# bcgsc/RNA-Bloom

Measured on AMD Instinct MI355X. Metric: k-mers/sec hashed+inserted into Bloom dBG (k=25, 50M 150bp reads), higher is better.
Workload: dtype u64

## Files before the change

### rna-bloom_amd/csrc/rb_capi.hip

```cpp
#include <math.h>
#include <stdarg.h>
#include <stdlib.h>
#include <string.h>
#include <time.h>

#include <algorithm>
#include <new>
#include <vector>

#include <functional>
#include <string>
#include <thread>

#include <fcntl.h>
#include <unistd.h>
#include <zlib.h>

#include "rb_pipeline.hpp"

using namespace rb;

namespace {

__global__ void k_popcount_bits(const uint32_t *__restrict__ w, size_t n_words, unsigned long long *out) {
// ... 594 lines not shown
            std::thread prep;
            int prep_rc = RB_OK;
            std::string prep_err;
            if (!last) {
                const size_t carry = len - cur.consumed;
                memcpy(buf[1 - w], buf[w] + cur.consumed, carry);
                prep = std::thread([&, carry] {
                    prep_rc = guarded([&] { nxt = make(1 - w, carry, &nlen); });
                    if (prep_rc != RB_OK) prep_err = rb_last_error();
                });
            }
            const int add_rc = guarded([&] { if (cur.b && cur.b->n_reads) add_range(g, cur.b, 0, cur.b->n_reads, flags, stats); });
            if (prep.joinable()) prep.join();
            if (add_rc != RB_OK) { if (nxt.b) rb_batch_destroy(nxt.b); throw HipError{add_rc}; }
            if (prep_rc != RB_OK) { set_error("%s", prep_err.c_str()); throw HipError{prep_rc}; }
            if (last) break;
            w = 1 - w; len = nlen; cur = nxt;
        }
        if (n_records) *n_records = recs;
    });
    if (st && !own_stream.s && rc != RB_OK) (void)hipStreamSynchronize(st);
    return rc;
}
}

extern "C" {
int rb_graph_add_fastq_file(rb_graph *g, const char *path, int min_base_qual, unsigned flags, rb_add_stats *stats, int64_t *n_records) {
    return add_text_file(g, path, false, min_base_qual, flags, stats, n_records);
}
int rb_graph_add_fasta_file(rb_graph *g, const char *path, unsigned flags, rb_add_stats *stats, int64_t *n_records) {
    return add_text_file(g, path, true, 0, flags, stats, n_records);
}

int rb_graph_apply(rb_graph *g, int op, const uint64_t *h0, size_t n) {
    return guarded([&] {
        RB_REQUIRE(g && (h0 || n == 0), "rb_graph_apply: null argument");
        WriteLock wl(g->rw);
        RB_REQUIRE(op >= RB_OP_ADD && op <= RB_OP_ADD_FRAG_PAIR, "rb_graph_apply: unknown op %d", op);
        RB_REQUIRE(!g->shard, "rb_graph_apply: not available on a shard handle");
        RB_HIP(hipSetDevice(g->p.device));
        hipStream_t s = g->stream;
        if (op == RB_OP_ADD_DBG_ONLY || op == RB_OP_ADD_READ_PAIR || op == RB_OP_ADD_FRAG_PAIR) {
            BitFilter *f = op == RB_OP_ADD_DBG_ONLY ? &g->dbg : op == RB_OP_ADD_READ_PAIR ? &g->rpk : &g->fpk;
            if (!f->bits) { set_error("rb_graph_apply: filter not initialised"); throw HipError{RB_ERR_STATE}; }
            if (n) {
                uint64_t *d = upload_h0(g, g->qbuf0, h0, n);
                hipLaunchKernelGGL(k_bits_add, dim3(blocks_for((int64_t)n)), dim3(TPB), 0, s, f->bits, f->mod, f->num_hash,
                                   kmul_of(g->k), d, n);
                RB_HIP(hipGetLastError());
            }
            RB_HIP(hipStreamSynchronize(s));
            return;
        }
        const int mode = op == RB_OP_ADD ? M_ADD : op == RB_OP_ADD_IF_ABSENT ? M_ADD_IF_ABSENT
                       : op == RB_OP_ADD_COUNT_IF_PRESENT ? M_COUNT_IF_PRESENT : M_COUNT_ONLY;
        size_t done = 0;
        const size_t chunk = (size_t)g->max_batch_kmers;
        while (done < n) {
            size_t m = std::min(chunk, n - done);
            g->keys0.reserve(m * 8); g->vals0.reserve(m * 4);
            RB_HIP(hipMemcpyAsync(g->keys0.p, h0 + done, m * 8, hipMemcpyHostToDevice, s));
            hipLaunchKernelGGL(k_iota, dim3(blocks_for((int64_t)m)), dim3(TPB), 0, s, g->vals0.as<uint32_t>(), m);
            run_pipeline(g, m, mode, g->ordinal, 0, nullptr);
            g->ordinal += m;
            done += m;
        }
        RB_HIP(hipStreamSynchronize(s));
    });
}

}
namespace {
__global__ void k_debug_probe(uint32_t *words, uint64_t n_words, uint32_t per_thread, int mode, uint64_t salt, unsigned long long *sink) {
    const uint64_t t = (uint64_t)blockIdx.x * blockDim.x + threadIdx.x;
    uint64_t x = (t + salt) * 0x9E3779B97F4A7C15ull + 0x632BE59BD9B4E019ull;
    uint32_t acc = 0;
    for (uint32_t i = 0; i < per_thread; ++i) {
        x ^= x >> 30; x *= 0xBF58476D1CE4E5B9ull; x ^= x >> 27; x *= 0x94D049BB133111EBull; x ^= x >> 31;
        uint32_t *w = &words[(uint64_t)(((unsigned __int128)x * n_words) >> 64)];
        acc |= mode ? atomicXor(w, 0x80808080u) : atomicOr(w, 0u);
    }
    if (acc == 0x12345678u) atomicAdd(sink, 1ull);
}
}
extern "C" {
int rb_debug_probe_cbf(rb_graph *g, int mode, float *ms_out) {
    return guarded([&] {
        RB_REQUIRE(g && g->cbf && ms_out, "rb_debug_probe_cbf: bad argument");
        rb::WriteLock wl(g->rw);
        RB_HIP(hipSetDevice(g->p.device));
        hipStream_t s = g->stream;
        g->devctr.reserve(DEVCTR_BYTES);
        rb::Event e0, e1;
        RB_HIP(hipEventCreate(&e0.e)); RB_HIP(hipEventCreate(&e1.e));
        RB_HIP(hipStreamSynchronize(s));
        RB_HIP(hipEventRecord(e0, s));
        for (int pass = 0; pass < 2; ++pass)
            hipLaunchKernelGGL(k_debug_probe, dim3(65536), dim3(256), 0, s, reinterpret_cast<uint32_t *>(g->cbf), (uint64_t)(g->cbf_alloc / 4), 16u, mode, 0ull, g->devctr.as<unsigned long long>());
        RB_HIP(hipEventRecord(e1, s));
        RB_HIP(hipEventSynchronize(e1));
        RB_HIP(hipEventElapsedTime(ms_out, e0, e1));
    });
}

int rb_debug_scan_u32(int device, const uint32_t *in, size_t n, uint32_t *out, int misalign) {
    DevBuf a, b, t;
    return guarded([&] {
        RB_REQUIRE((in && out) || n == 0, "rb_debug_scan_u32: null array");
        RB_REQUIRE(misalign >= 0 && misalign < 16, "rb_debug_scan_u32: misalign in 0..15");
        RB_HIP(hipSetDevice(device));
        a.reserve((n + 8) * 4); b.reserve((n + 8) * 4); t.reserve(scan_temp_bytes(n));
        uint32_t *di = a.as<uint32_t>() + (misalign & 3), *dout = b.as<uint32_t>() + ((misalign >> 2) & 3);
        if (n) RB_HIP(hipMemcpy(di, in, n * 4, hipMemcpyHostToDevice));
        exclusive_scan_u32(t.p, t.cap, di, dout, n, nullptr);
        RB_HIP(hipGetLastError());
        RB_HIP(hipDeviceSynchronize());
        if (n) RB_HIP(hipMemcpy(out, dout, n * 4, hipMemcpyDeviceToHost));
    });
}
int rb_debug_sort_pairs(int device, uint64_t *keys, void *vals, int vals64, size_t n, int lo_begin, int lo_end, int hi_begin, int hi_end) {
    DevBuf k0, k1, v0, v1, t;
    return guarded([&] {
        RB_REQUIRE(keys || n == 0, "rb_debug_sort_pairs: null keys");
        RB_REQUIRE(!(vals64 && hi_begin >= 0), "rb_debug_sort_pairs: two ranges with 32-bit values only");
        RB_HIP(hipSetDevice(device));
        if (n == 0) return;
        const size_t vb = vals64 ? 8 : 4;
        k0.reserve(n * 8); k1.reserve(n * 8);
        if (vals) { v0.reserve(n * vb); v1.reserve(n * vb); RB_HIP(hipMemcpy(v0.p, vals, n * vb, hipMemcpyHostToDevice)); }
        RB_HIP(hipMemcpy(k0.p, keys, n * 8, hipMemcpyHostToDevice));
        t.reserve(vals64 ? sort_pairs32_temp_bytes(n) : sort_pairs_temp_bytes(n));
        if (vals64) sort_pairs_u64_u64(t.p, t.cap, k0.as<uint64_t>(), k1.as<uint64_t>(), v0.as<uint64_t>(), v1.as<uint64_t>(), n, lo_begin, lo_end, nullptr);
        else if (hi_begin >= 0) sort_pairs_u64_u32_2r(t.p, t.cap, k0.as<uint64_t>(), k1.as<uint64_t>(), v0.as<uint32_t>(), v1.as<uint32_t>(), n, lo_begin, lo_end, hi_begin, hi_end, nullptr);
        else if (vals) sort_pairs_u64_u32(t.p, t.cap, k0.as<uint64_t>(), k1.as<uint64_t>(), v0.as<uint32_t>(), v1.as<uint32_t>(), n, lo_begin, lo_end, nullptr);
        else sort_keys_u64(t.p, t.cap, k0.as<uint64_t>(), k1.as<uint64_t>(), n, lo_begin, lo_end, nullptr);
        RB_HIP(hipGetLastError());
        RB_HIP(hipDeviceSynchronize());
        RB_HIP(hipMemcpy(keys, k1.p, n * 8, hipMemcpyDeviceToHost));
        if (vals) RB_HIP(hipMemcpy(vals, v1.p, n * vb, hipMemcpyDeviceToHost));
    });
}
int rb_debug_group(int device, const uint64_t *keys, const uint32_t *vals, size_t n, int group_bits, int bucket_target, unsigned flags,
                   uint64_t seed, uint64_t ordinal0, uint32_t pos_bits, uint64_t idx_size, uint64_t idx_lo, uint64_t idx_span,
                   uint32_t *vals_out, uint8_t *tz_out, uint64_t *uniq, uint32_t *counts, uint32_t *starts, uint32_t *brun, uint32_t *bnr, int64_t *info) {
    DevBuf k0, v0, k1, v1, vo, tz, un, cn, st, br, bn, t, ctr;
    return guarded([&] {
        RB_REQUIRE(keys && vals && vals_out && tz_out && uniq && counts && starts && info, "rb_debug_group: null array");
        RB_REQUIRE(n > 0 && n < ((size_t)1 << 28), "rb_debug_group: record count out of range");
        RB_REQUIRE((brun == nullptr) == (bnr == nullptr), "rb_debug_group: brun and bnr go together");
        RB_REQUIRE(pos_bits < 32 && (idx_span == 0 || idx_size > 0), "rb_debug_group: bad pos_bits / index range");
        RB_HIP(hipSetDevice(device));
        const int gflags = (int)flags;
        const GrIdx idx = idx_span ? GrIdx{make_mod(idx_size), idx_lo, idx_span} : GrIdx{Mod{1, 0, 0}, 0, 0};
        uint32_t plan[7];
        group_debug_plan(n, group_bits, bucket_target, gflags, idx, plan);
        const size_t nbk = (size_t)1 << plan[0];
        k0.reserve(n * 8); v0.reserve(n * 4); k1.reserve(n * 8); v1.reserve(n * 4);
        vo.reserve(n * 4); tz.reserve(n + 16); un.reserve(n * 8); cn.reserve((n + 1) * 4); st.reserve((n + 1) * 4);
        t.reserve(group_temp_bytes(n, group_bits, bucket_target, gflags));
        ctr.reserve(64);
        RB_HIP(hipMemcpy(k0.p, keys, n * 8, hipMemcpyHostToDevice));
        RB_HIP(hipMemcpy(v0.p, vals, n * 4, hipMemcpyHostToDevice));
        RB_HIP(hipMemset(vo.p, 0, n * 4)); RB_HIP(hipMemset(tz.p, 0, n)); RB_HIP(hipMemset(un.p, 0, n * 8));
        RB_HIP(hipMemset(cn.p, 0, n * 4)); RB_HIP(hipMemset(st.p, 0, n * 4)); RB_HIP(hipMemset(ctr.p, 0, 64));
        GroupExport ex;
        if (brun) {
            br.reserve(nbk * 4 + 16); bn.reserve(nbk * 4 + 16);
            RB_HIP(hipMemset(br.p, 0, nbk * 4)); RB_HIP(hipMemset(bn.p, 0, nbk * 4));
            ex = GroupExport{br.as<uint32_t>(), bn.as<uint32_t>(), ctr.as<uint32_t>() + 1};
        }
        group_records_device(k0.as<uint64_t>(), v0.as<uint32_t>(), k1.as<uint64_t>(), v1.as<uint32_t>(), n, group_bits, seed, ordinal0, pos_bits,
                             t.p, t.cap, vo.as<uint32_t>(), tz.as<uint8_t>(), un.as<uint64_t>(), cn.as<uint32_t>(), st.as<uint32_t>(), ctr.as<uint32_t>(),
                             nullptr, nullptr, bucket_target, gflags, idx, ex);
        RB_HIP(hipDeviceSynchronize());
        uint32_t c[2] = {0, 0}, live = (uint32_t)n, n_big = 0, largest = 0;
        uint64_t big_rec = 0;
        RB_HIP(hipMemcpy(c, ctr.p, 8, hipMemcpyDeviceToHost));
        if (gflags & GR_FLAG_DEAD) RB_HIP(hipMemcpy(&live, group_live_count(t.p, n, group_bits, bucket_target, gflags), 4, hipMemcpyDeviceToHost));
        group_debug_big(t.p, n, group_bits, bucket_target, &n_big, &big_rec, &largest, gflags);
        RB_REQUIRE(c[0] <= n && live <= n, "rb_debug_group: the stage reports %u runs and %u live records of %zu", c[0], live, n);
        RB_HIP(hipMemcpy(vals_out, vo.p, n * 4, hipMemcpyDeviceToHost));
        RB_HIP(hipMemcpy(tz_out, tz.p, n, hipMemcpyDeviceToHost));
        RB_HIP(hipMemcpy(uniq, un.p, n * 8, hipMemcpyDeviceToHost));
        RB_HIP(hipMemcpy(counts, cn.p, n * 4, hipMemcpyDeviceToHost));
        RB_HIP(hipMemcpy(starts, st.p, n * 4, hipMemcpyDeviceToHost));
        if (brun) {
            RB_HIP(hipMemcpy(brun, br.p, nbk * 4, hipMemcpyDeviceToHost));
            RB_HIP(hipMemcpy(bnr, bn.p, nbk * 4, hipMemcpyDeviceToHost));
        }
        for (int i = 0; i < 7; ++i) info[i] = (int64_t)plan[i];
        info[7] = (int64_t)c[0]; info[8] = brun ? (int64_t)c[1] : -1; info[9] = (int64_t)live;
        info[10] = (int64_t)n_big; info[11] = (int64_t)largest;
    });
}
int rb_debug_select(int device, const uint32_t *status, size_t n, uint32_t mask_a, uint32_t mask_b, uint32_t *out_a, uint32_t *out_b, uint32_t *counts) {
    DevBuf s, a, b, t, ctr;
    return guarded([&] {
        RB_REQUIRE(counts && (n == 0 || (status && out_a && (out_b || mask_b == 0u))), "rb_debug_select: null array");
        RB_REQUIRE(n < ((size_t)1 << 31), "rb_debug_select: too many items");
        RB_HIP(hipSetDevice(device));
        s.reserve(n * 4 + 16); a.reserve(n * 4 + 16); b.reserve(n * 4 + 16); ctr.reserve(64);
        t.reserve(mask_b ? select2_temp_bytes(n) : select_temp_bytes(n));
        if (n) RB_HIP(hipMemcpy(s.p, status, n * 4, hipMemcpyHostToDevice));
        RB_HIP(hipMemset(ctr.p, 0xFF, 64));
        if (mask_b) select_flagged2(t.p, t.cap, s.as<uint32_t>(), n, mask_a, a.as<uint32_t>(), mask_b, b.as<uint32_t>(), ctr.as<uint32_t>(), nullptr);
        else select_flagged(t.p, t.cap, s.as<uint32_t>(), mask_a, n, a.as<uint32_t>(), ctr.as<uint32_t>(), nullptr);
        RB_HIP(hipGetLastError());
        RB_HIP(hipDeviceSynchronize());
        uint32_t c[2] = {0, 0};
        RB_HIP(hipMemcpy(c, ctr.p, 8, hipMemcpyDeviceToHost));
        if (!mask_b) c[1] = 0;
        RB_REQUIRE(c[0] <= n && c[1] <= n, "rb_debug_select: the selection reports %u and %u of %zu items", c[0], c[1], n);
        if (c[0]) RB_HIP(hipMemcpy(out_a, a.p, (size_t)c[0] * 4, hipMemcpyDeviceToHost));
        if (c[1]) RB_HIP(hipMemcpy(out_b, b.p, (size_t)c[1] * 4, hipMemcpyDeviceToHost));
        counts[0] = c[0]; counts[1] = c[1];
    });
}
}
namespace {
bool debug_prefilter_on(const rb_graph *g) {
    const bool wide_off = getenv("RB_WIDE_PREFILTER") && atoi(getenv("RB_WIDE_PREFILTER")) == 0;
    return g->npf_log2 && (g->k <= 31 || (g->k <= 64 && !wide_off));
}
bool debug_prefilter_uses_mpf(const rb_graph *g, const rb_batch *b, int64_t nw) {
    return g->mpf_log2b && !getenv("RB_NO_MPF") && (uint32_t)g->k >= g->mpf_m &&
           (g->k <= RB_MPF_MAX_K ? (uint32_t)g->k - g->mpf_m + 1u <= RB_MPF_MAX_RING : filter_wide_mpf_ok(b, nw, g->k));
}
bool debug_prefilter_saves_state(const rb_graph *g, const rb_batch *b, int64_t nw, bool use_mpf) {
    return g->k > RB_MPF_MAX_K ? (use_mpf && filter_saves_state_wide(b, nw, g->k)) : filter_saves_state(b, nw, g->k);
}
}
extern "C" {
int rb_debug_cache_export(rb_graph *g, int which, uint64_t *out, size_t cap_words, uint32_t *log2_out, uint32_t *m_out) {
    return guarded([&] {
        RB_REQUIRE(g && log2_out && m_out, "rb_debug_cache_export: null argument");
        RB_REQUIRE(which == 0 || which == 1, "rb_debug_cache_export: which must be 0 (minimizer-bucketed) or 1 (hash-bucketed)");
        rb::WriteLock wl(g->rw);
        RB_REQUIRE(which == 0 ? g->mpf_log2b != 0u : g->npf_log2 != 0u, "rb_debug_cache_export: this handle has no %s prefilter cache (k = %d)",
                   which == 0 ? "minimizer-bucketed" : "hash-bucketed", g->k);
        const size_t words = which == 0 ? (size_t)16 << g->mpf_log2b : (size_t)1 << g->npf_log2;
        *log2_out = which == 0 ? g->mpf_log2b : g->npf_log2;
        *m_out = which == 0 ? g->mpf_m : 0u;
        if (!out) return;
        RB_REQUIRE(cap_words >= words, "rb_debug_cache_export: the table has %zu words, the array has room for %zu", words, cap_words);
        RB_HIP(hipSetDevice(g->p.device));
        for (hipStream_t st : {(hipStream_t)g->stream, (hipStream_t)g->stream2}) RB_HIP(hipStreamSynchronize(st));
        RB_HIP(hipMemcpy(out, which == 0 ? g->mpf.p : g->npf.p, words * 8, hipMemcpyDeviceToHost));
    });
}
int rb_debug_prefilter(rb_graph *g, const rb_batch *b, int64_t first_word, int64_t n_words, uint64_t ordinal0, uint32_t pos_bits,
                       uint32_t *cnt_out, uint32_t *mask_out) {
    DevBuf cnt, mask, tot, ws;
    return guarded([&] {
        RB_REQUIRE(g && b && cnt_out && mask_out, "rb_debug_prefilter: null argument");
        rb::WriteLock wl(g->rw);
        RB_REQUIRE(!g->shard, "rb_debug_prefilter: not available on a shard handle");
        RB_REQUIRE(b->device == g->p.device, "batch lives on device %d, graph on %d", b->device, g->p.device);
        RB_REQUIRE(debug_prefilter_on(g), "rb_debug_prefilter: an insert into this handle runs no prefilter (k = %d)", g->k);
        RB_REQUIRE(pos_bits >= 1u && pos_bits < 32u, "rb_debug_prefilter: pos_bits in 1..31");
        const auto &wo = b->h_woff;
        RB_REQUIRE(!wo.empty() && first_word >= 0 && n_words > 0 && first_word + n_words <= b->n_words, "rb_debug_prefilter: bad word range");
        const int64_t r0 = std::lower_bound(wo.begin(), wo.end(), (uint32_t)first_word) - wo.begin();
        const int64_t r1 = std::lower_bound(wo.begin(), wo.end(), (uint32_t)(first_word + n_words)) - wo.begin();
        RB_REQUIRE(r0 < (int64_t)wo.size() && wo[(size_t)r0] == (uint32_t)first_word && r1 < (int64_t)wo.size() && wo[(size_t)r1] == (uint32_t)(first_word + n_words),
                   "rb_debug_prefilter: the word range does not start and end at read boundaries");
        RB_HIP(hipSetDevice(g->p.device));
        hipStream_t s = g->stream;
        const bool use_mpf = debug_prefilter_uses_mpf(g, b, n_words);
        const Npf npf{reinterpret_cast<unsigned long long *>(g->npf.p), g->npf_log2};
        const Mpf mpf{use_mpf ? reinterpret_cast<unsigned long long *>(g->mpf.p) : nullptr, g->mpf_log2b, g->mpf_m};
        const size_t nb = (size_t)n_words * 4;
        cnt.reserve(nb + 4); mask.reserve(nb + 4); tot.reserve(2048);
        RB_HIP(hipMemsetAsync(cnt.p, 0xEE, nb, s)); RB_HIP(hipMemsetAsync(mask.p, 0xEE, nb, s)); RB_HIP(hipMemsetAsync(tot.p, 0, 2048, s));
        void *wstate = nullptr;
        if (debug_prefilter_saves_state(g, b, n_words, use_mpf)) { ws.reserve(((size_t)n_words + 1) * 16); wstate = ws.p; }
        launch_filter_windows(b, first_word, n_words, g->k, g->stranded ? 0 : 1, (uint32_t)r0, pos_bits, g->p.rng_seed, ordinal0, npf,
                              cnt.as<uint32_t>(), mask.as<uint32_t>(), tot.as<uint32_t>(), s, OwnRange{Mod{1, 0, 0}, 0, 0}, mpf, wstate);
        RB_HIP(hipGetLastError());
        RB_HIP(hipStreamSynchronize(s));
        RB_HIP(hipMemcpy(cnt_out, cnt.p, nb, hipMemcpyDeviceToHost));
        RB_HIP(hipMemcpy(mask_out, mask.p, nb, hipMemcpyDeviceToHost));
    });
}
int rb_filter_size(rb_graph *g, int which, int64_t *size, int64_t *nbytes, int *num_hash) {
    if (!g) { set_error("null graph"); return RB_ERR_INVALID; }
    if (which == RB_CBF) {
        if (!g->cbf) { set_error("rb_filter_size: filter %d not initialised", which); return RB_ERR_STATE; }
        if (size) *size = g->cbf_size;
        if (nbytes) *nbytes = g->cbf_hi - g->cbf_lo;
        if (num_hash) *num_hash = g->cbf_h;
        return RB_OK;
    }
    BitFilter *f = bit_filter(g, which);
    if (!f) { set_error("rb_filter_size: unknown filter %d", which); return RB_ERR_INVALID; }
    if (!f->bits) { set_error("rb_filter_size: filter %d not initialised", which); return RB_ERR_STATE; }
    if (size) *size = f->size;
    if (nbytes) *nbytes = f->nbytes;
    if (num_hash) *num_hash = f->num_hash;
    return RB_OK;
}

static int filter_reduce(rb_graph *g, int which, bool fold, unsigned long long *out) {
    return guarded([&] {
        RB_REQUIRE(g && out, "rb_filter_popcount / rb_filter_fold: null argument");
        QueryLease q(g);
        RB_HIP(hipStreamSynchronize(g->stream));
        q.c->b0.reserve(64);
// ... 182 lines not shown
```

### rna-bloom_amd/csrc/rb_graph.hip

```cpp
#include <math.h>
#include <stdarg.h>
#include <stdlib.h>
#include <string.h>
#include <time.h>

#include <algorithm>
#include <new>
#include <vector>

#include <functional>
#include <string>
#include <thread>

#include <fcntl.h>
#include <unistd.h>
#include <zlib.h>

#include "rb_pipeline.hpp"

using namespace rb;

namespace rb {
static thread_local char g_err[768] = "";
const char *last_error_text() { return g_err; }
// ... 921 lines not shown
                if (j && (e & 31u) == 0u) { cR = word_c(e >> 5); vR = word_v(e >> 5); }
                if (j && (j & 31u) == 0u) { cL = word_c(j >> 5); vL = word_v(j >> 5); }
                const uint32_t codeR = (uint32_t)cR & 3u, okR = vR & 1u, codeL = (uint32_t)cL & 3u, okL = vL & 1u;
                cR >>= 2; vR >>= 1; cL >>= 2; vL >>= 1;
                {
                    const uint32_t in5 = okR ? codeR + 1u : 0u;
                    const uint32_t out5 = ((uint32_t)(hvR >> sh_v) & 1u) ? ((uint32_t)((far ? hcR2 : hcR) >> sh_c) & 3u) + 1u : 0u;
                    const uint32_t tt = out5 * 5u + in5;
                    fR = rotl(fR, 1) ^ s_tf[tt]; rR = rotr(rR, 1) ^ s_tr[tt];
                    hcR2 = (hcR2 << 2) | (hcR >> 62); hcR = (hcR << 2) | codeR; hvR = (hvR << 1) | okR;
                }
                {
                    const uint32_t in5 = okL ? codeL + 1u : 0u;
                    const uint32_t out5 = ((uint32_t)(hvL >> sh_v) & 1u) ? ((uint32_t)((far ? hcL2 : hcL) >> sh_c) & 3u) + 1u : 0u;
                    const uint32_t tt = out5 * 5u + in5;
                    fL = rotl(fL, 1) ^ s_tf[tt]; rL = rotr(rL, 1) ^ s_tr[tt];
                    if (VAR == 1) {
                        mF = ((mF << 2) | codeL) & mmask;
                        mR = (mR >> 2) | ((3u - codeL) << mtop);
                        uint32_t x = (mF < mR ? mF : mR) * 0x9E3779B1u;
                        x ^= x >> 15;
                        xnew = x >> 4;
                        if ((x & seen.amask) == 0u && j + 1u >= um) { akey = xnew; apos1 = j + 2u - um; }
                    }
                    hcL2 = (hcL2 << 2) | (hcL >> 62); hcL = (hcL << 2) | codeL; hvL = (hvL << 1) | okL;
                }
                lb = okR ? lb : e + 1u;
                if (j + 1u >= uk) {
                    const uint32_t p = j + 1u - uk;
                    bool ok = lb <= p;
                    if (ok && present) {
                        const uint64_t hl = (MODE == 0) ? fL : (MODE == 2) ? rL : smin(fL, rL);
                        const uint64_t hr = (MODE == 0) ? fR : (MODE == 2) ? rR : smin(fR, rR);
                        ok = bits_lookup(present, present_mod, present_h, kmul, hl) && bits_lookup(present, present_mod, present_h, kmul, hr);
                    }
                    if (ok) {
                        uint64_t P;
                        if (MODE == 0) P = combine(fL, fR);
                        else if (MODE == 2) P = combine(rR, rL);
                        else P = smin(combine(fL, fR), combine(rR, rL));
                        if (VAR == 2) {
                            if ((p >> 5) != oword) { oword = p >> 5; obase = chunk_off[wrel + (int64_t)oword]; ocnt = 0; }
                            for (int h = 0; h < num_hash; ++h)
                                out_idx[((size_t)obase + ocnt) * (size_t)num_hash + h] = index_of(multi_hash(P, (uint32_t)h, kmul), mod);
                            ++ocnt;
                        } else if (VAR == 1) {
                            const uint32_t bk = (apos1 > p ? akey : xnew) & seen.mask;
                            if (bk != curb) {
                                curb = bk; ++dbg_fetch;
                                const uint4 *src = reinterpret_cast<const uint4 *>(seen.tab + ((size_t)bk << 4));
                                uint4 v[8];
#pragma unroll
                                for (int q = 0; q < 8; ++q) v[q] = src[q];
#pragma unroll
                                for (int q = 0; q < 8; ++q) {
                                    s_img[(2 * q) * 64 + threadIdx.x] = (unsigned long long)v[q].x | ((unsigned long long)v[q].y << 32);
                                    s_img[(2 * q + 1) * 64 + threadIdx.x] = (unsigned long long)v[q].z | ((unsigned long long)v[q].w << 32);
                                }
                            }
                            const uint32_t sa = (uint32_t)P & 15u, sb0 = ((uint32_t)P >> 4) & 15u, sb = sb0 == sa ? (sa ^ 1u) : sb0;
                            const unsigned long long ea = s_img[sa * 64u + threadIdx.x], eb = s_img[sb * 64u + threadIdx.x];
                            if (P == 0ull || (ea != P && eb != P)) {
                                ++dbg_miss;
                                for (int h = 0; h < num_hash; ++h) bit_set(bits, index_of(multi_hash(P, (uint32_t)h, kmul), mod));
                                if (P != 0ull) {
                                    const uint32_t sl = ea == 0ull ? sa : (eb == 0ull ? sb : sa);
                                    s_img[sl * 64u + threadIdx.x] = P;
                                    seen.tab[((size_t)bk << 4) + sl] = P;
                                }
                            }
                        } else {
                            for (int h = 0; h < num_hash; ++h) bit_set(bits, index_of(multi_hash(P, (uint32_t)h, kmul), mod));
                        }
                        ++cnt;
                    }
                }
            }
            if (VAR == 1 && seen.dbg) { atomicAdd(seen.dbg, (unsigned long long)dbg_miss); atomicAdd(seen.dbg + 1, (unsigned long long)dbg_fetch); }
        }
    }
    if (n_pairs) {
        unsigned long long c = cnt;
        for (int o = 32; o > 0; o >>= 1) c += __shfl_down(c, o, 64);
        if (threadIdx.x == 0 && c) atomicAdd(n_pairs, c);
    }
}

}

void rb::launch_pairs_reads(rb_graph *g, const rb_batch *b, int64_t w0, int64_t nw, int mode_hash, const BitFilter &f, int dist,
                               uint32_t min_len, bool if_present, const uint32_t *chunk_off, uint64_t *out_idx, unsigned long long *pc,
                               hipStream_t st) {
    RB_REQUIRE(g->k <= 64 && b->max_len <= 1024u, "paired k-mers: k <= 64 and reads of at most 1024 bases only on this path");
    const auto &wo = b->h_woff;
    const int64_t r0 = std::lower_bound(wo.begin(), wo.end(), (uint32_t)w0) - wo.begin();
    const int64_t r1 = std::lower_bound(wo.begin(), wo.end(), (uint32_t)(w0 + nw)) - wo.begin();
    RB_REQUIRE(r0 < (int64_t)wo.size() && wo[(size_t)r0] == (uint32_t)w0 && r1 < (int64_t)wo.size() && wo[(size_t)r1] == (uint32_t)(w0 + nw),
               "launch_pairs: word range does not start and end at read boundaries");
    if (r1 <= r0) return;
    dim3 gr(blocks_for(r1 - r0, 64)), th(64);
    const uint32_t *present = if_present ? g->dbg.bits : nullptr;
    const bool use_seen = f.seen && !out_idx && !present;
    static const uint32_t anchor_bits = getenv("RB_PAIR_SEEN_ANCHOR") ? (uint32_t)std::max(0, std::min(4, atoi(getenv("RB_PAIR_SEEN_ANCHOR")))) : 2u;
    const PairSeen seen{use_seen ? f.seen : nullptr, use_seen ? (1u << f.seen_log2b) - 1u : 0u, (1u << anchor_bits) - 1u,
                        (use_seen && pc == g->pairs_ctr.as<unsigned long long>() && getenv("RB_DEBUG")) ? pc + 1 : nullptr};
#define RB_LAUNCH_PR3(M, NW, V)                                                                                          \
    hipLaunchKernelGGL((k_pairs_reads<M, NW, V>), gr, th, 0, st, b->codes, b->valid, b->woff, b->len, r0, r1 - r0, w0, g->k, \
                       dist, f.bits, f.mod, f.num_hash, kmul_of(g->k), pc, chunk_off, out_idx, min_len, present, g->dbg.mod, g->dbg.num_hash, seen)
#define RB_LAUNCH_PR(M, NW) do { if (out_idx) RB_LAUNCH_PR3(M, NW, 2); else if (use_seen) RB_LAUNCH_PR3(M, NW, 1); else RB_LAUNCH_PR3(M, NW, 0); } while (0)
    if (b->max_len <= 384u) { if (mode_hash == 0) RB_LAUNCH_PR(0, 12); else if (mode_hash == 2) RB_LAUNCH_PR(2, 12); else RB_LAUNCH_PR(1, 12); }
    else { if (mode_hash == 0) RB_LAUNCH_PR(0, 32); else if (mode_hash == 2) RB_LAUNCH_PR(2, 32); else RB_LAUNCH_PR(1, 32); }
#undef RB_LAUNCH_PR
#undef RB_LAUNCH_PR3
}

void rb::launch_pairs(rb_graph *g, const rb_batch *b, int64_t w0, int64_t nw, int mode_hash, const uint32_t *chunk_off,
                      uint64_t *out_idx, unsigned long long *pc, hipStream_t st, const BitFilter *into) {
    if (!st) st = g->stream;
    if (nw <= 0) return;
    const BitFilter &rpk = into ? *into : g->rpk;
    const bool general = g->k > 64 || b->max_len > 384u || (getenv("RB_PAIRS_GENERAL") && atoi(getenv("RB_PAIRS_GENERAL")));
    if (!general) {
        launch_pairs_reads(g, b, w0, nw, mode_hash, rpk, g->read_d, 0u, false, chunk_off, out_idx, pc, st);
        return;
    }
    dim3 gr(blocks_for(nw)), th(TPB);
#ifdef RB_DIAG_PAIRS
    if (getenv("RB_PAIRS_VARIANT") && atoi(getenv("RB_PAIRS_VARIANT")) == 9 && mode_hash == 1) {
        hipLaunchKernelGGL(k_pairs_insert_runtime_branch, gr, th, 0, st, b->codes, b->valid, b->word_read, b->woff, b->len, w0, nw, g->k, g->read_d,
                           rpk.bits, rpk.mod, rpk.num_hash, kmul_of(g->k), pc, chunk_off, out_idx,
                           (b->wpr_uniform && nw % b->wpr_uniform == 0) ? b->wpr_uniform : 0u);
        return;
    }
#endif
#define RB_LAUNCH_PAIRS(M)                                                                                          \
    if (out_idx) RB_LAUNCH_PAIRS2(M, true); else RB_LAUNCH_PAIRS2(M, false)
#define RB_LAUNCH_PAIRS2(M, O)                                                                                      \
    hipLaunchKernelGGL((k_pairs_insert<M, O>), gr, th, 0, st, b->codes, b->valid, b->word_read, b->woff, b->len, w0, nw, \
                       g->k, g->read_d, rpk.bits, rpk.mod, rpk.num_hash, kmul_of(g->k), pc, chunk_off, out_idx, \
                       (b->wpr_uniform && nw % b->wpr_uniform == 0) ? b->wpr_uniform : 0u)
    if (mode_hash == 0) { RB_LAUNCH_PAIRS(0); } else if (mode_hash == 2) { RB_LAUNCH_PAIRS(2); } else { RB_LAUNCH_PAIRS(1); }
#undef RB_LAUNCH_PAIRS
#undef RB_LAUNCH_PAIRS2
}

static bool sweep_wanted(const rb_graph *g) {
    if (g->shard || !g->dbg.bits || g->dbg.lo != 0 || g->dbg.hi != g->dbg.size) return false;
    if (const char *e = getenv("RB_SWEEP")) return atoi(e) != 0;
    return g->dbg.nbytes >= ((int64_t)1 << 31);
}
void rb::group_enqueue(rb_graph *g, int slot, size_t N, uint64_t ordinal0, uint32_t pos_bits, hipStream_t st, DevBuf &temp,
                       DevBuf &ctrbuf, int flags) {
    rb_graph::GroupSlot &S = g->slots[slot];
    S.N = N; S.D = 0; S.flags = flags; S.live = (uint32_t)N;
    ctrbuf.reserve(DEVCTR_BYTES);
    uint32_t *ctr = ctrbuf.as<uint32_t>();
    RB_HIP(hipMemsetAsync(ctr, 0, DEVCTR_BYTES, st));
    if (N == 0) return;
    const int group_bits = 64 - g->sort_begin_bit;
    const int bucket_target = g->shard ? (getenv("RB_SHARD_GROUP_TARGET") ? atoi(getenv("RB_SHARD_GROUP_TARGET")) : 3072) : 0;
    S.bucket_target = bucket_target;
    temp.reserve(group_temp_bytes(N, group_bits, bucket_target, flags));
    S.keys1.reserve(N * 8); S.valsT.reserve(N * 4); S.vals1.reserve(N * 4); S.tz.reserve(N + 16);
    S.uniq.reserve(N * 8); S.counts.reserve((N + 1) * 4); S.starts.reserve((N + 1) * 4);
    GrIdx gidx{Mod{1, 0, 0}, 0, 0};
    bool want_idx = true;
    if (const char *e = getenv("RB_GROUP_IDX")) want_idx = atoi(e) != 0;
    if (want_idx) {
        if (g->cbf && g->cbf_size > 0) gidx = GrIdx{g->cbf_mod, (uint64_t)g->cbf_lo, (uint64_t)(g->cbf_hi - g->cbf_lo)};
        else if (g->dbg.bits && g->dbg.size > 0) gidx = GrIdx{g->dbg.mod, (uint64_t)g->dbg.lo, (uint64_t)(g->dbg.hi - g->dbg.lo)};
    }
    GroupExport ex;
    S.sweep_T = 0; S.n_main = 0;
    if (want_idx && sweep_wanted(g)) {
        const GrIdx didx{g->dbg.mod, 0, (uint64_t)g->dbg.size};
        const bool same = gidx.span == didx.span && gidx.lo == 0 && gidx.mod.d == didx.mod.d;
        if (!same) gidx = didx;
        S.sweep_T = group_index_buckets(N, group_bits, bucket_target, flags, gidx);
        if (S.sweep_T) {
            S.brun.reserve(((size_t)4 << S.sweep_T) + 16); S.bnr.reserve(((size_t)4 << S.sweep_T) + 16);
            ex = GroupExport{S.brun.as<uint32_t>(), S.bnr.as<uint32_t>(), ctr + 9};
        }
    }
    uint64_t *kin = g->group_in_keys ? g->group_in_keys : g->keys0.as<uint64_t>();
    uint32_t *vin = g->group_in_vals ? g->group_in_vals : g->vals0.as<uint32_t>();
    g->group_in_keys = nullptr; g->group_in_vals = nullptr;
    group_records_device(kin, vin, S.keys1.as<uint64_t>(), S.valsT.as<uint32_t>(), N, group_bits,
                         g->p.rng_seed, ordinal0, pos_bits, temp.p, temp.cap, S.vals1.as<uint32_t>(), S.tz.as<uint8_t>(), S.uniq.as<uint64_t>(),
                         S.counts.as<uint32_t>(), S.starts.as<uint32_t>(), ctr + 8, st, g, bucket_target, flags, gidx, ex);
}
uint32_t rb::group_finish(rb_graph *g, int slot, hipStream_t st, DevBuf &temp, DevBuf &ctrbuf, hipStream_t scan_stream) {
    rb_graph::GroupSlot &S = g->slots[slot];
    if (S.N == 0) { RB_HIP(hipStreamSynchronize(st)); return 0; }
    uint32_t D = 0;
    RB_HIP(hipMemcpyAsync(&D, ctrbuf.as<uint32_t>() + 8, 4, hipMemcpyDeviceToHost, st));
    if (S.sweep_T) RB_HIP(hipMemcpyAsync(&S.n_main, ctrbuf.as<uint32_t>() + 9, 4, hipMemcpyDeviceToHost, st));
    if (S.flags & GR_FLAG_DEAD)
        RB_HIP(hipMemcpyAsync(&S.live, group_live_count(temp.p, S.N, 64 - g->sort_begin_bit, S.bucket_target, S.flags), 4, hipMemcpyDeviceToHost, st));
    RB_HIP(hipStreamSynchronize(st));
    RB_REQUIRE(D < (1u << 30), "sub-batch has too many distinct k-mers (%u)", D);
    S.D = D;
    (void)scan_stream;
    if (getenv("RB_DEBUG") && temp.p) {
        uint32_t nb = 0, mx = 0; uint64_t rec = 0;
        group_debug_big(temp.p, S.N, 64 - g->sort_begin_bit, S.bucket_target, &nb, &rec, &mx, S.flags);
        fprintf(stderr, "[rb] grouping: N=%zu runs=%u; buckets that did not fit LDS: %u with %llu records, largest %u\n", S.N, D, nb, (unsigned long long)rec, mx);
    }
    return D;
}
uint32_t rb::group_records(rb_graph *g, size_t N, uint64_t ordinal0, uint32_t pos_bits, rb_add_stats *stats, uint32_t **ctr_out) {
    group_enqueue(g, g->cur, N, ordinal0, pos_bits, g->stream, g->temp, g->devctr);
    const uint32_t D = group_finish(g, g->cur, g->stream, g->temp, g->devctr, g->stream);
    if (ctr_out) *ctr_out = g->devctr.as<uint32_t>();
    if (stats) stats->distinct += D;
    return D;
}

namespace {

}
__global__ void __launch_bounds__(256) k_zero16(uint4 *__restrict__ p, size_t n16) {
    const uint4 z = make_uint4(0u, 0u, 0u, 0u);
    for (size_t i = (size_t)blockIdx.x * blockDim.x + threadIdx.x; i < n16; i += (size_t)gridDim.x * blockDim.x) p[i] = z;
}
void rb::fast_zero(void *p, size_t bytes, hipStream_t s) {
    if (!p || !bytes) return;
    if (bytes < ((size_t)64 << 20) || (reinterpret_cast<uintptr_t>(p) & 15u)) { RB_HIP(hipMemsetAsync(p, 0, bytes, s)); return; }
    const size_t n16 = bytes / 16;
    hipLaunchKernelGGL(k_zero16, dim3(256 * 16), dim3(256), 0, s, static_cast<uint4 *>(p), n16);
    RB_HIP(hipGetLastError());
    if (bytes & 15u) RB_HIP(hipMemsetAsync(static_cast<char *>(p) + n16 * 16, 0, bytes & 15u, s));
}

void rb::alloc_bits(BitFilter &f, int64_t bits, int num_hash, int64_t lo, int64_t hi) {
    f.size = bits;
    f.lo = lo; f.hi = hi;
    const int64_t local = hi - lo;
    f.nbytes = local / 8 + ((local % 8) ? 1 : 0);
    f.alloc = (((size_t)f.nbytes + 3) / 4 + 1) * 4;
    f.num_hash = num_hash;
    f.mod = make_mod((uint64_t)bits);
    RB_HIP(hipMalloc(&f.bits, f.alloc));
    RB_HIP(hipMemset(f.bits, 0, f.alloc));
    RB_HIP(hipDeviceSynchronize());
}
namespace {
__global__ void k_alloc_probe(uint32_t *words, uint64_t n_words, uint32_t per_thread, unsigned long long *sink) {
    const uint64_t t = (uint64_t)blockIdx.x * blockDim.x + threadIdx.x;
    uint64_t x = t * 0x9E3779B97F4A7C15ull + 0x632BE59BD9B4E019ull;
    uint32_t acc = 0;
    for (uint32_t i = 0; i < per_thread; ++i) {
        x ^= x >> 30; x *= 0xBF58476D1CE4E5B9ull; x ^= x >> 27; x *= 0x94D049BB133111EBull; x ^= x >> 31;
        acc |= atomicXor(&words[(uint64_t)(((unsigned __int128)x * n_words) >> 64)], 0x80808080u);
    }
    if (acc == 0x12345678u) atomicAdd(sink, 1ull);
}
}
void *rb::alloc_best_placed(size_t bytes, const char *what) {
    int tries = getenv("RB_ALLOC_TRIES") ? atoi(getenv("RB_ALLOC_TRIES")) : 8;
    tries = std::max(1, std::min(16, tries));
    if (bytes < ((size_t)1 << 30)) tries = 1;
    struct Held {
        void *best = nullptr, *cand = nullptr;
        unsigned long long *sink = nullptr;
        hipEvent_t e0 = nullptr, e1 = nullptr;
        std::vector<void *> losers;
        ~Held() {
            for (void *p : losers) (void)hipFree(p);
            if (best) (void)hipFree(best);
            if (cand) (void)hipFree(cand);
            if (sink) (void)hipFree(sink);
            if (e0) (void)hipEventDestroy(e0);
            if (e1) (void)hipEventDestroy(e1);
        }
    } H;
    float best_ms = 0;
    if (tries > 1) { RB_HIP(hipMalloc(&H.sink, 64)); RB_HIP(hipEventCreate(&H.e0)); RB_HIP(hipEventCreate(&H.e1)); }
    for (int t = 0; t < tries; ++t) {
        if (t) {
            size_t free_b = 0, total_b = 0;
            RB_HIP(hipMemGetInfo(&free_b, &total_b));
            if (free_b < bytes + total_b / 4) break;
        }
        if (hipMalloc(&H.cand, bytes) != hipSuccess) { H.cand = nullptr; (void)hipGetLastError(); if (t) break; RB_HIP(hipErrorOutOfMemory); }
        RB_HIP(hipMemset(H.cand, 0, bytes));
        float ms = 0;
        if (tries > 1) {
            RB_HIP(hipDeviceSynchronize());
            RB_HIP(hipEventRecord(H.e0, nullptr));
            for (int pass = 0; pass < 2; ++pass)
                hipLaunchKernelGGL(k_alloc_probe, dim3(16384), dim3(256), 0, nullptr, static_cast<uint32_t *>(H.cand), (uint64_t)(bytes / 4), 16u, H.sink);
            RB_HIP(hipEventRecord(H.e1, nullptr));
            RB_HIP(hipEventSynchronize(H.e1));
            RB_HIP(hipEventElapsedTime(&ms, H.e0, H.e1));
        }
        if (getenv("RB_ALLOC_DEBUG")) fprintf(stderr, "[rb] %s allocation %d: %.3f ms for 2 x 2^26 random XORs\n", what, t, ms);
        if (!H.best || ms < best_ms) { if (H.best) H.losers.push_back(H.best); H.best = H.cand; best_ms = ms; }
        else H.losers.push_back(H.cand);
        H.cand = nullptr;
    }
    RB_HIP(hipDeviceSynchronize());
    void *best = H.best;
    H.best = nullptr;
    return best;
}

void rb::free_bits(BitFilter &f) { if (f.bits) (void)hipFree(f.bits); if (f.seen) (void)hipFree(f.seen); f = BitFilter(); }
void rb::alloc_pair_seen(BitFilter &f) {
    if (!f.bits || f.seen) return;
    uint32_t lb = std::max(8u, std::min(24u, log2_ceil((uint64_t)std::max<int64_t>(f.size / 512, 1))));
    if (const char *e = getenv("RB_PAIR_SEEN")) { const int v = atoi(e); if (v <= 0) return; lb = (uint32_t)std::max(4, std::min(26, v)); }
    size_t fr = 0, tot = 0;
    if (hipMemGetInfo(&fr, &tot) == hipSuccess && ((size_t)128 << lb) > fr / 4) return;
    if (hipMalloc(&f.seen, (size_t)128 << lb) != hipSuccess) { (void)hipGetLastError(); f.seen = nullptr; return; }
    RB_HIP(hipMemset(f.seen, 0, (size_t)128 << lb));
    RB_HIP(hipDeviceSynchronize());
    f.seen_log2b = lb;
}
void rb::seen_reset(BitFilter &f, hipStream_t s) {
    if (f.seen) fast_zero(f.seen, (size_t)128 << f.seen_log2b, s);
}
namespace {


}
BitFilter *rb::bit_filter(rb_graph *g, int which) {
    switch (which) { case RB_DBGBF: return &g->dbg; case RB_RPKBF: return &g->rpk; case RB_FPKBF: return &g->fpk; default: return nullptr; }
}
namespace {

void run_core(rb_graph *g, size_t N, uint32_t D, int mode, uint64_t ordinal0, uint32_t pos_bits, rb_add_stats *stats,
              const std::function<void()> *after_resolve = nullptr);
}
void rb::run_pipeline(rb_graph *g, size_t N, int mode, uint64_t ordinal0, uint32_t pos_bits, rb_add_stats *stats) {
    if (N == 0) return;
    const uint32_t D = group_records(g, N, ordinal0, pos_bits, stats, nullptr);
    run_core(g, N, D, mode, ordinal0, pos_bits, stats);
}
namespace {
void run_core(rb_graph *g, size_t N, uint32_t D, int mode, uint64_t ordinal0, uint32_t pos_bits, rb_add_stats *stats,
              const std::function<void()> *after_resolve) {
    hipStream_t s = g->stream;
    if (N == 0 || D == 0) { if (after_resolve) (*after_resolve)(); return; }
    g->devctr.reserve(DEVCTR_BYTES);
    uint32_t *ctr = g->devctr.as<uint32_t>();
    RB_HIP(hipMemsetAsync(ctr, 0, DEVCTR_BYTES, s));
    FilterView fv = g->view(ordinal0, pos_bits);
    const uint64_t *uniq = g->uniq().as<uint64_t>();
    const uint32_t *counts = g->counts().as<uint32_t>(), *starts = g->starts().as<uint32_t>(), *vals = g->vals1().as<uint32_t>();
    g->status.reserve((size_t)D * 4); g->nops.reserve((size_t)D * 4); g->cvals.reserve((size_t)D * 8);
    g->heavy.reserve((size_t)D * 4); g->confk.reserve((size_t)D * 4);
    g->foreign.reserve((size_t)D * 8 * (size_t)g->cbf_h);
    uint32_t *status = g->status.as<uint32_t>(), *nops = g->nops.as<uint32_t>();
    const bool uses_dbg = (mode == M_ADD || mode == M_ADD_IF_ABSENT);
    uint32_t f_log2 = 1, c_log2 = 1, csf_log2 = 16;
    uint32_t *csf = nullptr;
    const bool full_table = getenv("RB_FIRST_SETTER_TABLE") && atoi(getenv("RB_FIRST_SETTER_TABLE"));
    const bool collide = uses_dbg && !full_table;
    Slot *ftab = nullptr;
    FtFilter ffl{nullptr, 0};
    if (uses_dbg && full_table) {
        g->prof_begin();
        f_log2 = log2_ceil(2ull * (uint64_t)D * (uint64_t)g->dbg.num_hash + 2);
        g->ftable.reserve(sizeof(Slot) << f_log2);
        RB_HIP(hipMemsetAsync(g->ftable.p, 0xFF, sizeof(Slot) << f_log2, s));
        ftab = g->ftable.as<Slot>();
        g->prof_end("table_clear");
    }
    g->prof_begin();
    const rb_graph::GroupSlot &GS = g->slots[g->cur];
    bool swept = false, swept_all = false;
    uint32_t *involved = nullptr, n_involved_max = 0;
    if (collide && !ftab && fv.dbg_h == 2 && fv.cbf_h == 2 && !getenv("RB_PROBE_GENERIC") && GS.sweep_T && !g->shard && sweep_wanted(g) &&
        ((uint64_t)g->dbg.size >> GS.sweep_T) < (1ull << 31)) {
        const char *e = getenv("RB_SWEEP");
        static const float present_max = getenv("RB_SWEEP_PRESENT") ? (float)atof(getenv("RB_SWEEP_PRESENT")) : 0.5f;
        swept = (e && atoi(e) == 1) || ((uint64_t)D * 64ull >= (uint64_t)g->dbg.nbytes && g->last_present_frac < present_max);
    }
    if (swept) {
        const GrIdx didx{g->dbg.mod, 0, (uint64_t)g->dbg.size};
        swept_all = GS.n_main >= D;
        const size_t st_pad = ((size_t)D + 15) & ~(size_t)15;
        g->sw_st.reserve(st_pad + D + 16);
        g->sw_temp.reserve(sweep_temp_bytes(D, GS.sweep_T));
        uint8_t *st0 = g->sw_st.as<uint8_t>(), *st1 = st0 + st_pad;
        uint64_t *ka = g->foreign.as<uint64_t>(), *kb = ka + D;
        sweep_bits_device(g->dbg.bits, didx, GS.sweep_T, fv.kmul, uniq, D, GS.n_main, GS.brun.as<uint32_t>(), GS.bnr.as<uint32_t>(), ka, g->nops.as<uint32_t>(), kb,
                          g->heavy.as<uint32_t>(), g->sw_temp.p, g->sw_temp.cap, st0, st1, s);
        const bool same_index = (int64_t)g->dbg.size == g->cbf_size && g->cbf_lo == 0 && g->dbg.mod.d == g->cbf_mod.d && g->dbg.mod.m_lo == g->cbf_mod.m_lo &&
                                g->dbg.mod.m_hi == g->cbf_mod.m_hi && fv.dbg_h == fv.cbf_h;
        const bool plain_ok = swept_all && same_index && !(getenv("RB_SWEEP_CLAIMS") && atoi(getenv("RB_SWEEP_CLAIMS")));
        constexpr int RUNS = 2;
        hipLaunchKernelGGL((k_probe_h2<RUNS, true>), dim3(blocks_for(((int64_t)D + RUNS - 1) / RUNS)), dim3(TPB), 0, s, fv, uniq, counts, D, mode, status,
                           g->cvals.as<uint64_t>(), g->foreign.as<uint64_t>(), ctr, (const uint8_t *)st0, (const uint8_t *)st1, swept_all ? 1u : 0u,
                           plain_ok ? 1u : 0u);
    } else if (!ftab && fv.dbg_h == 2 && fv.cbf_h == 2 && !getenv("RB_PROBE_GENERIC")) {
        constexpr int RUNS = 2;
        hipLaunchKernelGGL((k_probe_h2<RUNS, false>), dim3(blocks_for(((int64_t)D + RUNS - 1) / RUNS)), dim3(TPB), 0, s, fv, uniq, counts, D, mode, status,
                           g->cvals.as<uint64_t>(), g->foreign.as<uint64_t>(), ctr);
    } else
        hipLaunchKernelGGL(k_probe, dim3(blocks_for(D)), dim3(TPB), 0, s, fv, uniq, counts, starts, vals, D, mode,
                           ftab, f_log2, status, g->cvals.as<uint64_t>(), g->foreign.as<uint64_t>(), ctr);
    if (collide) {
        if (!swept) hipLaunchKernelGGL(k_set_bits, dim3(blocks_for(D)), dim3(TPB), 0, s, fv, uniq, D, status, ctr);
        uint32_t spread[16 * 32], n_collide = 0;
        RB_HIP(hipMemcpyAsync(spread, ctr + 16, sizeof spread, hipMemcpyDeviceToHost, s));
        RB_HIP(hipStreamSynchronize(s));
        for (int q = 0; q < 32; ++q) n_collide += spread[16 * q + 1];
        if (n_collide) {
            f_log2 = log2_ceil(4ull * (uint64_t)n_collide + 2);
            const size_t tab_bytes = sizeof(Slot) << f_log2;
            const uint32_t ff_log2 = std::max(16u, std::min(30u, log2_ceil(8ull * (uint64_t)n_collide)));
            const bool use_ff = getenv("RB_FT_FILTER") ? atoi(getenv("RB_FT_FILTER")) != 0 : tab_bytes > ((size_t)32 << 20);
            g->ftable.reserve(tab_bytes + (use_ff ? ((size_t)1 << (ff_log2 - 3)) : 0));
            RB_HIP(hipMemsetAsync(g->ftable.p, 0xFF, tab_bytes, s));
            ftab = g->ftable.as<Slot>();
            if (use_ff) {
                uint32_t *fb = reinterpret_cast<uint32_t *>(static_cast<char *>(g->ftable.p) + tab_bytes);
                RB_HIP(hipMemsetAsync(fb, 0, (size_t)1 << (ff_log2 - 3), s));
                ffl = FtFilter{fb, ff_log2};
            }
            if (swept_all) {
                involved = g->confk.as<uint32_t>(); n_involved_max = n_collide;
                g->temp.reserve(select_temp_bytes(D));
                select_flagged(g->temp.p, g->temp.cap, status, (3u << ST_COLLIDE_SHIFT) | (3u << ST_JOIN_SHIFT), D, involved, ctr + 12, s);
                hipLaunchKernelGGL(k_collide_insert, dim3(blocks_for(std::min(D, n_collide))), dim3(TPB), 0, s, fv, uniq, starts, vals, std::min(D, n_collide), status, ftab, f_log2,
                                   const_cast<uint32_t *>(ffl.bits), ffl.log2, (const uint32_t *)involved, (const uint32_t *)(ctr + 12));
            } else
            hipLaunchKernelGGL(k_collide_insert, dim3(blocks_for(D)), dim3(TPB), 0, s, fv, uniq, starts, vals, D, status, ftab, f_log2,
                               const_cast<uint32_t *>(ffl.bits), ffl.log2);
            if (!swept_all) hipLaunchKernelGGL(k_collide_fixup, dim3(blocks_for(D)), dim3(TPB), 0, s, fv, uniq, starts, vals, D, status, ftab, f_log2, ffl);
        }
    }
    if (mode == M_ADD) {
        if (swept_all) {
            if (involved) hipLaunchKernelGGL(k_late_claim, dim3(blocks_for(std::min(D, n_involved_max))), dim3(TPB), 0, s, fv, uniq, starts, vals, std::min(D, n_involved_max), ftab, f_log2,
                                             status, g->cvals.as<uint64_t>(), g->foreign.as<uint64_t>(), ctr, ffl, (const uint32_t *)involved, (const uint32_t *)(ctr + 12));
        } else
        hipLaunchKernelGGL(k_late_claim, dim3(blocks_for(D)), dim3(TPB), 0, s, fv, uniq, starts, vals, D, ftab, f_log2,
                           status, g->cvals.as<uint64_t>(), g->foreign.as<uint64_t>(), ctr, ffl);
    }
    uint32_t n_foreign = 0;
    {
        uint32_t spread[16 * 32];
        RB_HIP(hipMemcpyAsync(spread, ctr + 16, sizeof spread, hipMemcpyDeviceToHost, s));
        RB_HIP(hipStreamSynchronize(s));
        uint32_t n_present = 0;
        for (int q = 0; q < 32; ++q) { n_foreign += spread[16 * q]; n_present += spread[16 * q + 2]; }
        const bool counted = !(uses_dbg && full_table) && fv.dbg_h == 2 && fv.cbf_h == 2 && !getenv("RB_PROBE_GENERIC");
        g->last_present_frac = counted ? (float)n_present / (float)D : -1.0f;
    }
    if (getenv("RB_DEBUG") && swept) fprintf(stderr, "[rb] swept stage: %u runs (%u of oversized buckets), %u contested counters\n", D, D - std::min(D, GS.n_main), n_foreign);
    g->prof_end("probe_claim");
    if (n_foreign) {
        g->prof_begin();
        c_log2 = log2_ceil(2ull * (uint64_t)n_foreign + 2);
        csf_log2 = std::max(16u, std::min(25u, log2_ceil(8ull * (uint64_t)n_foreign)));
        const size_t tab_bytes = sizeof(Slot) << c_log2;
        g->ctable.reserve(tab_bytes + ((size_t)1 << (csf_log2 - 3)));
        csf = reinterpret_cast<uint32_t *>(static_cast<char *>(g->ctable.p) + tab_bytes);
        RB_HIP(hipMemsetAsync(g->ctable.p, 0xFF, tab_bytes, s));
        RB_HIP(hipMemsetAsync(csf, 0, (size_t)1 << (csf_log2 - 3), s));
        hipLaunchKernelGGL(k_cs_build, dim3(blocks_for(D)), dim3(TPB), 0, s, status, g->foreign.as<uint64_t>(), D, g->cbf_h,
                           g->ctable.as<Slot>(), c_log2, csf, csf_log2);
        g->prof_end("conflict_set");
    }
    g->prof_begin();
    hipLaunchKernelGGL(k_resolve_apply, dim3(blocks_for(D)), dim3(TPB), 0, s, fv, uniq, counts, starts, vals, D, mode, g->light_ops,
                       ftab, f_log2, ffl, (int)collide, g->ctable.as<Slot>(), c_log2, getenv("RB_NO_CS_FILTER") ? (uint32_t *)nullptr : csf, csf_log2, n_foreign, status, nops,
                       g->cvals.as<uint64_t>(), g->tz().as<uint8_t>(), getenv("RB_DEBUG") ? reinterpret_cast<float *>(ctr + 700) : (float *)nullptr);
    g->prof_end("resolve_apply");
    bool released = false;
    auto release = [&] { if (!released && after_resolve) (*after_resolve)(); released = true; };
    const bool old_rule = getenv("RB_ORDER_ALL_SHARED") != nullptr;
    if (!n_foreign || old_rule || getenv("RB_RELEASE_EARLY")) release();
    if (getenv("RB_DEBUG")) {
        float df[128];
        RB_HIP(hipMemcpyAsync(df, ctr + 700, sizeof df, hipMemcpyDeviceToHost, s));
        RB_HIP(hipStreamSynchronize(s));
        double dr = 0, tot = 0;
        for (int q = 0; q < 64; ++q) { dr += df[2 * q]; tot += df[2 * q + 1]; }
        unsigned long long hh[96];
        RB_HIP(hipMemcpyFromSymbol(hh, HIP_SYMBOL(g_dbg_hist), sizeof hh));
        double miss = 0;
        for (int s0 = 1; s0 < 8; ++s0) miss += (double)hh[s0 * 8] * (1.0 - 1.0 / (double)(1u << s0));
        fprintf(stderr, "[rb] ops a perfect cache would drop: %.1f%% of %.0f ops (N=%zu; %.1f%% if no occurrence had been filtered)\n",
                tot ? 100.0 * miss / tot : 0.0, tot, N, tot ? 100.0 * dr / tot : 0.0);
        for (int s0 = 1; s0 < 8; ++s0) {
            fprintf(stderr, "[rb]   true exponent %d: ops by cached exponent 0..7 (M):", s0);
            for (int sc = 0; sc < 8; ++sc) fprintf(stderr, " %.1f", hh[s0 * 8 + sc] / 1e6);
            fprintf(stderr, "\n");
        }
        fprintf(stderr, "[rb]   uncached ops by occupied slots of their bucket 0..16 (M):");
        for (int q = 0; q <= 16; ++q) fprintf(stderr, " %.1f", hh[64 + q] / 1e6);
        fprintf(stderr, "\n");
        memset(hh, 0, sizeof hh);
        RB_HIP(hipMemcpyToSymbol(HIP_SYMBOL(g_dbg_hist), hh, sizeof hh));
    }
    g->prof_begin();
    g->temp.reserve(select2_temp_bytes(D));
    select_flagged2(g->temp.p, g->temp.cap, status, D, RUN_HEAVY, g->heavy.as<uint32_t>(), RUN_CONFLICT, g->confk.as<uint32_t>(), ctr + 0, s);
    uint32_t hc[2] = {0, 0};
    RB_HIP(hipMemcpyAsync(hc, ctr, 8, hipMemcpyDeviceToHost, s));
    RB_HIP(hipStreamSynchronize(s));
    g->prof_end("compact_lists");
    if (hc[1] && !old_rule) {
        g->prof_begin();
        const uint32_t nc0 = hc[1];
        const size_t slots = (size_t)1 << c_log2;
        g->cwriters.reserve(slots * 8 + 64);
        const size_t cs_stride = ((size_t)nc0 + 1 + 3) / 4 * 4;
        const size_t hh = (size_t)fv.cbf_h;
        g->cshared.reserve(cs_stride * 4 * (5 + hh) + 64);
        RB_HIP(hipMemsetAsync(g->cwriters.p, 0, slots * 8 + 64, s));
        uint32_t *writers = g->cwriters.as<uint32_t>(), *cflag = writers + slots, *changed = cflag + slots;
        uint32_t *ordered = g->cshared.as<uint32_t>(), *heavy2 = ordered + cs_stride, *pos_o = heavy2 + cs_stride, *pos_h = pos_o + cs_stride,
                 *heavy2_list = pos_h + cs_stride, *cslot = heavy2_list + cs_stride;
        RB_HIP(hipMemsetAsync(ordered, 0, cs_stride * 4 * 2, s));
        const CsLookup L{g->ctable.as<Slot>(), c_log2, csf, csf_log2};
        const uint32_t *cand = g->confk.as<uint32_t>();
        hipLaunchKernelGGL(k_cs_writers, dim3(blocks_for(nc0)), dim3(TPB), 0, s, fv, uniq, nops, cand, nc0, g->cvals.as<uint64_t>(), L, writers, cslot);
        const int per_look = nc0 >= (1u << 20) ? 1 : 3;
        for (int round = 0;;) {
            int everything = 0;
            for (int q = 0; q < per_look; ++q, ++round) {
                everything = round >= 16 ? 1 : 0;
                hipLaunchKernelGGL(k_cs_order, dim3(blocks_for(nc0)), dim3(TPB), 0, s, (int)fv.cbf_h, nc0, cslot, writers, cflag, ordered, changed + (round & 7), everything);
                if (everything) { ++round; break; }
            }
            const int last = round - 1;
            uint32_t ch = 0;
            RB_HIP(hipMemcpyAsync(&ch, changed + (last & 7), 4, hipMemcpyDeviceToHost, s));
            RB_HIP(hipStreamSynchronize(s));
            if (!ch || everything) break;
            RB_HIP(hipMemsetAsync(changed, 0, 32, s));
        }
        hipLaunchKernelGGL(k_resolve_deferred, dim3(blocks_for(nc0)), dim3(TPB), 0, s, fv, uniq, counts, starts, vals, cand, nc0, ordered, mode, g->light_ops, cslot,
                           status, nops, g->cvals.as<uint64_t>(), g->tz().as<uint8_t>(), heavy2);
        g->prof_end("conflict_set");
        release();
// ... 312 lines not shown
```

### rna-bloom_amd/csrc/rb_group.hip

```cpp
#include <stdlib.h>

#include <algorithm>

#include "rb_pipeline.hpp"

namespace rb {

constexpr uint32_t GR_KEY_TOP = 60;
constexpr uint32_t GR_MAX_GROUP_BITS = 36;
constexpr uint32_t GR_TILE = 4096;
constexpr uint32_t GR_BUCKET_TARGET = 3072;
constexpr uint32_t GR_LOCAL_BITS = 8;
constexpr uint32_t GR_PART_MAX_BITS = 10;

constexpr uint64_t GR_DEAD_KEY = ~0ull;
constexpr uint32_t GR_DEAD_VAL = ~0u;
__device__ __forceinline__ uint32_t gr_digit(uint64_t key, uint32_t shift, uint32_t bits) {
    return (uint32_t)(key >> shift) & ((1u << bits) - 1u);
}
struct GrIdxDev { Mod mod; uint64_t lo, mul; uint32_t top, shift; };
__device__ __forceinline__ uint32_t gr_idx_digit(uint64_t key, const GrIdxDev &ix, uint32_t bits) {
    const uint64_t i = index_of(key, ix.mod) - ix.lo;
    const uint32_t d = min((uint32_t)min(__umul64hi(i, ix.mul), (uint64_t)0xFFFFFFFFull), ix.top);
    return (d >> ix.shift) & ((1u << bits) - 1u);
}
__device__ __forceinline__ uint32_t gr_lanes_below(uint64_t m) {
    return __builtin_amdgcn_mbcnt_hi((uint32_t)(m >> 32), __builtin_amdgcn_mbcnt_lo((uint32_t)m, 0u));
}

template <int ITEMS, typename CT>
__device__ __forceinline__ void gr_wave_rank(const uint32_t (&dig)[ITEMS], uint32_t (&rank)[ITEMS], CT *wc, uint32_t bits, uint32_t rows) {
    const uint32_t lane = threadIdx.x & 63u;
#pragma unroll
    for (int r = 0; r < ITEMS; ++r) {
        if ((uint32_t)r < rows) {
            const bool valid = dig[r] != ~0u;
            uint64_t m = __ballot(valid);
            for (uint32_t b = 0; b < bits; ++b) {
                const bool bit = (dig[r] >> b) & 1u;
                const uint64_t bal = __ballot(bit);
                m &= bit ? bal : ~bal;
            }
            uint32_t prior = 0;
            if (valid) prior = (uint32_t)wc[dig[r]];
            rank[r] = prior + gr_lanes_below(m);
            if (valid && (m >> lane) == 1ull) wc[dig[r]] = (CT)(prior + (uint32_t)__popcll(m));
            __builtin_amdgcn_wave_barrier();
        }
    }
}

template <int ITEMS, typename CT>
__device__ __forceinline__ void gr_wave_rank_lds(const uint32_t (&dig)[ITEMS], uint32_t (&rank)[ITEMS], CT *wc, unsigned long long *wm, uint32_t rows) {
    const uint32_t lane = threadIdx.x & 63u;
#pragma unroll
    for (int r = 0; r < ITEMS; ++r) {
        if ((uint32_t)r < rows) {
            const bool valid = dig[r] != ~0u;
            uint64_t m = 0;
            uint32_t prior = 0;
            if (valid) {
                __hip_atomic_fetch_or(&wm[dig[r]], 1ull << lane, __ATOMIC_RELAXED, __HIP_MEMORY_SCOPE_WORKGROUP);
                m = __hip_atomic_load(&wm[dig[r]], __ATOMIC_RELAXED, __HIP_MEMORY_SCOPE_WORKGROUP);
                prior = (uint32_t)wc[dig[r]];
            }
            rank[r] = prior + gr_lanes_below(m);
            if (valid && (m >> lane) == 1ull) {
                __hip_atomic_store(&wm[dig[r]], 0ull, __ATOMIC_RELAXED, __HIP_MEMORY_SCOPE_WORKGROUP);
                wc[dig[r]] = (CT)(prior + (uint32_t)__popcll(m));
            }
            __builtin_amdgcn_wave_barrier();
        }
    }
}

template <int ITEMS, typename CT>
__device__ __forceinline__ void gr_wave_rank_lds_wide(const uint32_t (&dig)[ITEMS], uint32_t (&rank)[ITEMS], CT *wc, unsigned long long *wm, uint32_t bits,
                                                      uint32_t rows) {
    const uint32_t lane = threadIdx.x & 63u;
#pragma unroll
    for (int r = 0; r < ITEMS; ++r) {
        if ((uint32_t)r < rows) {
            const bool valid = dig[r] != ~0u;
            uint64_t ml = 0;
            uint32_t prior = 0;
            if (valid) {
                __hip_atomic_fetch_or(&wm[dig[r] & 255u], 1ull << lane, __ATOMIC_RELAXED, __HIP_MEMORY_SCOPE_WORKGROUP);
                ml = __hip_atomic_load(&wm[dig[r] & 255u], __ATOMIC_RELAXED, __HIP_MEMORY_SCOPE_WORKGROUP);
                prior = (uint32_t)wc[dig[r]];
            }
            uint64_t m = ml;
            for (uint32_t b = 8; b < bits; ++b) {
                const bool bit = valid && ((dig[r] >> b) & 1u);
                const uint64_t bal = __ballot(bit);
                m &= bit ? bal : ~bal;
            }
            rank[r] = prior + gr_lanes_below(m);
            if (valid && (ml >> lane) == 1ull) __hip_atomic_store(&wm[dig[r] & 255u], 0ull, __ATOMIC_RELAXED, __HIP_MEMORY_SCOPE_WORKGROUP);
            if (valid && (m >> lane) == 1ull) wc[dig[r]] = (CT)(prior + (uint32_t)__popcll(m));
            __builtin_amdgcn_wave_barrier();
        }
    }
}

template <int TPB>
__device__ __forceinline__ uint32_t gr_block_excl_scan(uint32_t v, uint32_t *s_wsum) {
    const uint32_t lane = threadIdx.x & 63u, w = threadIdx.x >> 6;
    uint32_t inc = v;
#pragma unroll
    for (int o = 1; o < 64; o <<= 1) {
        const uint32_t t = __shfl_up(inc, o, 64);
        if ((int)lane >= o) inc += t;
    }
    if (lane == 63u) s_wsum[w] = inc;
    __syncthreads();
    uint32_t base = 0;
#pragma unroll
    for (int i = 0; i < TPB / 64; ++i) {
        const uint32_t t = s_wsum[i];
        if ((uint32_t)i < w) base += t;
    }
    __syncthreads();
    return base + inc - v;
}

template <int TPB, typename CT, typename DT>
__device__ __forceinline__ void gr_digit_offsets(CT *wcnt , DT *dstart , uint32_t nb, uint32_t *s_wsum) {
    constexpr int NW = TPB / 64;
    const uint32_t per = (nb + TPB - 1) / TPB;
    uint32_t tot[4] = {0, 0, 0, 0}, sum = 0;
    for (uint32_t q = 0; q < per; ++q) {
        const uint32_t d = threadIdx.x * per + q;
        if (d < nb) {
            uint32_t run = 0;
#pragma unroll
            for (int w = 0; w < NW; ++w) { const uint32_t t = (uint32_t)wcnt[(uint32_t)w * nb + d]; wcnt[(uint32_t)w * nb + d] = (CT)run; run += t; }
            tot[q] = run; sum += run;
        }
    }
    uint32_t base = gr_block_excl_scan<TPB>(sum, s_wsum);
    for (uint32_t q = 0; q < per; ++q) {
        const uint32_t d = threadIdx.x * per + q;
        if (d < nb) { dstart[d] = (DT)base; base += tot[q]; }
    }
}

__device__ __forceinline__ uint32_t gr_tile_of_block(uint32_t b, uint32_t grid_tiles, int xcd_map) {
    if (!xcd_map) return b;
    return (b & 7u) * (grid_tiles >> 3) + (b >> 3);
}
inline uint32_t gr_grid_for_tiles(uint32_t ntiles) { return ((ntiles + 7u) / 8u) * 8u; }

struct GrTile { uint32_t start, count, hist_base, hist_stride; };
struct GrTiling {
    const GrTile *desc;
    const uint32_t *ntiles_dev;
    uint32_t n, ntiles, grid_tiles;
    int xcd_map;
};
__device__ __forceinline__ bool gr_get_tile(const GrTiling &tl, GrTile &t) {
    const uint32_t i = gr_tile_of_block(blockIdx.x, tl.grid_tiles, tl.xcd_map);
    if (!tl.desc) {
        if (i >= tl.ntiles) return false;
        t.start = i * GR_TILE; t.count = min(GR_TILE, tl.n - t.start); t.hist_base = i; t.hist_stride = tl.ntiles;
        return true;
    }
    if (i >= *tl.ntiles_dev) return false;
    t = tl.desc[i];
    return true;
}

template <int TPB, bool DERIVE = false>
__global__ void __launch_bounds__(TPB) k_part_count(const uint64_t *__restrict__ keys, GrTiling tl, uint32_t shift, uint32_t bits,
                                                    uint32_t *__restrict__ hist, const uint32_t *__restrict__ dead_vals = nullptr,
                                                    GrIdxDev ix = GrIdxDev{Mod{1, 0, 0}, 0, 0, 0, 0}, uint64_t kmul = 0) {
    constexpr int ITEMS = GR_TILE / TPB;
    __shared__ uint32_t s_h[1u << GR_PART_MAX_BITS];
    GrTile t;
    if (!gr_get_tile(tl, t)) return;
    const uint32_t nb = 1u << bits;
    for (uint32_t d = threadIdx.x; d < nb; d += TPB) s_h[d] = 0;
    __syncthreads();
    uint64_t k[ITEMS];
#pragma unroll
    for (int i = 0; i < ITEMS; ++i) {
        const uint32_t j = (uint32_t)i * TPB + threadIdx.x;
        k[i] = j < t.count ? keys[t.start + j] : 0ull;
        if (DERIVE) k[i] = multi_hash(k[i], 1u, kmul);
    }
#pragma unroll
    for (int i = 0; i < ITEMS; ++i) {
        const uint32_t j = (uint32_t)i * TPB + threadIdx.x;
        if (j < t.count && !(dead_vals && k[i] == GR_DEAD_KEY && dead_vals[t.start + j] == GR_DEAD_VAL))
            atomicAdd(&s_h[ix.mul ? gr_idx_digit(k[i], ix, bits) : gr_digit(k[i], shift, bits)], 1u);
    }
    __syncthreads();
    for (uint32_t d = threadIdx.x; d < nb; d += TPB) hist[(size_t)t.hist_base + (size_t)d * t.hist_stride] = s_h[d];
}

template <int TPB, int MAXBITS, bool DERIVE = false>
__global__ void __launch_bounds__(TPB) k_part_scatter(const uint64_t *__restrict__ keys_in, const uint32_t *__restrict__ vals_in, GrTiling tl,
                                                      uint32_t shift, uint32_t bits, const uint32_t *__restrict__ goffs ,
                                                      uint64_t *__restrict__ keys_out, uint32_t *__restrict__ vals_out, uint32_t wide_lds,
                                                      uint32_t skip_dead = 0u, GrIdxDev ix = GrIdxDev{Mod{1, 0, 0}, 0, 0, 0, 0}, uint64_t kmul = 0) {
    constexpr uint32_t ITEMS = GR_TILE / TPB, NW = TPB / 64, SEG = 64 * ITEMS, MAXNB = 1u << MAXBITS;
    __shared__ uint64_t s_keys[GR_TILE];
    __shared__ uint32_t s_vals[GR_TILE];
    __shared__ uint32_t s_cnt[NW * MAXNB / 2 > MAXNB ? NW * MAXNB / 2 : MAXNB];
    __shared__ uint16_t s_dstart[MAXNB];
    __shared__ uint32_t s_wsum[NW];
    constexpr bool NARROW = MAXBITS <= 8;
    static_assert(sizeof(s_vals) >= NW * 256u * sizeof(unsigned long long), "the mask table must fit the staging array");
    unsigned long long *s_wmask = reinterpret_cast<unsigned long long *>(s_vals);
    uint16_t *s_wcnt = reinterpret_cast<uint16_t *>(s_cnt);
    GrTile t;
    if (!gr_get_tile(tl, t)) return;
    const uint32_t nb = 1u << bits;
    const uint32_t w = threadIdx.x >> 6, lane = threadIdx.x & 63u;
    for (uint32_t d = threadIdx.x; d < NW * nb; d += TPB) s_wcnt[d] = 0;
    for (uint32_t d = threadIdx.x; d < NW * (NARROW ? nb : 256u); d += TPB) s_wmask[d] = 0ull;
    uint64_t k[ITEMS];
    uint32_t v[ITEMS], dig[ITEMS], rank[ITEMS];
#pragma unroll
    for (uint32_t r = 0; r < ITEMS; ++r) {
        const uint32_t j = w * SEG + r * 64u + lane;
        bool ok = j < t.count;
        k[r] = ok ? keys_in[t.start + j] : 0ull;
        v[r] = (ok && vals_in) ? vals_in[t.start + j] : 0u;
        if (DERIVE) { k[r] = multi_hash(k[r], 1u, kmul); v[r] = t.start + j; }
        if (skip_dead && k[r] == GR_DEAD_KEY && v[r] == GR_DEAD_VAL) ok = false;
        dig[r] = ok ? (ix.mul ? gr_idx_digit(k[r], ix, bits) : gr_digit(k[r], shift, bits)) : ~0u;
    }
    const uint32_t rows = t.count > w * SEG ? min(ITEMS, (t.count - w * SEG + 63u) / 64u) : 0u;
    __syncthreads();
    if (NARROW) gr_wave_rank_lds<ITEMS>(dig, rank, s_wcnt + w * nb, s_wmask + w * nb, rows);
    else if (wide_lds) gr_wave_rank_lds_wide<ITEMS>(dig, rank, s_wcnt + w * nb, s_wmask + w * 256u, bits, rows);
    else gr_wave_rank<ITEMS>(dig, rank, s_wcnt + w * nb, bits, rows);
    __syncthreads();
    gr_digit_offsets<TPB>(s_wcnt, s_dstart, nb, s_wsum);
    __syncthreads();
#pragma unroll
    for (uint32_t r = 0; r < ITEMS; ++r)
        if (dig[r] != ~0u) {
            const uint32_t p = (uint32_t)s_dstart[dig[r]] + (uint32_t)s_wcnt[w * nb + dig[r]] + rank[r];
            s_keys[p] = k[r]; s_vals[p] = v[r];
        }
    __syncthreads();
    uint32_t live = 0;
#pragma unroll
    for (uint32_t i = 0; i < NW; ++i) live += s_wsum[i];
    for (uint32_t d = threadIdx.x; d < nb; d += TPB) s_cnt[d] = goffs[(size_t)t.hist_base + (size_t)d * t.hist_stride] - (uint32_t)s_dstart[d];
    __syncthreads();
    for (uint32_t j = threadIdx.x; j < live; j += TPB) {
        const uint64_t key = s_keys[j];
        const uint32_t g = s_cnt[ix.mul ? gr_idx_digit(key, ix, bits) : gr_digit(key, shift, bits)] + j;
        keys_out[g] = key;
        if (vals_out) vals_out[g] = s_vals[j];
    }
}

__global__ void __launch_bounds__(1024) k_seg_tiles(const uint32_t *__restrict__ goffs1, uint32_t ntiles1, uint32_t nb1, uint32_t n, uint32_t nb2,
                                                    GrTile *__restrict__ desc, uint32_t *__restrict__ seg_tile_base ,
                                                    uint32_t *__restrict__ seg_start , uint32_t *__restrict__ ntiles2_dev,
                                                    const uint32_t *__restrict__ n_dev = nullptr ) {
    __shared__ uint32_t s_wsum[16];
    const uint32_t b = threadIdx.x;
    if (n_dev) n = *n_dev;
    uint32_t s = 0, e = 0;
    if (b < nb1) { s = goffs1[(size_t)b * ntiles1]; e = b + 1u < nb1 ? goffs1[(size_t)(b + 1u) * ntiles1] : n; }
    const uint32_t nt = (e - s + GR_TILE - 1u) / GR_TILE;
    const uint32_t tb = gr_block_excl_scan<1024>(nt, s_wsum);
    if (b < nb1) {
        seg_tile_base[b] = tb; seg_start[b] = s;
        for (uint32_t i = 0; i < nt; ++i) {
            GrTile t; t.start = s + i * GR_TILE; t.count = min(GR_TILE, e - t.start); t.hist_base = tb * nb2 + i; t.hist_stride = nt;
            desc[tb + i] = t;
        }
        if (b == nb1 - 1u) { seg_tile_base[nb1] = tb + nt; seg_start[nb1] = n; *ntiles2_dev = tb + nt; }
    }
}
__global__ void k_bucket_bounds(const uint32_t *__restrict__ goffs, uint32_t ntiles1, const uint32_t *__restrict__ seg_tile_base,
                                const uint32_t *__restrict__ seg_start, uint32_t t_hi, uint32_t t_lo, uint32_t n, uint32_t *__restrict__ bstart,
                                const uint32_t *__restrict__ n_dev = nullptr) {
    const uint32_t p = blockIdx.x * blockDim.x + threadIdx.x, nbk = 1u << (t_hi + t_lo);
    if (n_dev) n = *n_dev;
    if (p > nbk) return;
    if (p == nbk) { bstart[p] = n; return; }
    if (t_hi == 0) { bstart[p] = 0; return; }
    if (t_lo == 0) { bstart[p] = goffs[(size_t)p * ntiles1]; return; }
    const uint32_t b = p >> t_lo, lo = p & ((1u << t_lo) - 1u);
    const uint32_t tb = seg_tile_base[b], nt = seg_tile_base[b + 1u] - tb;
    bstart[p] = nt ? goffs[((size_t)tb << t_lo) + (size_t)lo * nt] : seg_start[b];
}

__global__ void k_copy_u32(uint32_t *__restrict__ dst, const uint32_t *__restrict__ src) { if (threadIdx.x == 0 && blockIdx.x == 0) *dst = *src; }

#ifndef GR_ABL
#define GR_ABL 0
#endif
struct GroupRng { uint64_t seed, ordinal0; uint32_t pos_bits; };
constexpr unsigned long long GR_ST_AGG = 1ull << 62, GR_ST_PREFIX = 2ull << 62;

__device__ __forceinline__ uint32_t gr_look_back(const unsigned long long *status, uint32_t c) {
    const uint32_t lane = threadIdx.x & 63u;
    uint32_t sum = 0;
    int64_t p = (int64_t)c - 1;
    for (;;) {
        const int64_t mine = p - (int64_t)lane;
        unsigned long long st = GR_ST_PREFIX;
        if (mine >= 0) st = __hip_atomic_load(&status[mine], __ATOMIC_RELAXED, __HIP_MEMORY_SCOPE_AGENT);
        const uint64_t ready = __ballot((st >> 62) != 0ull), pref = __ballot((st >> 62) == 2ull);
        const uint32_t n_ready = ready == ~0ull ? 64u : (uint32_t)__builtin_ctzll(~ready);
        const uint32_t first_pref = pref ? (uint32_t)__builtin_ctzll(pref) : 64u;
        const uint32_t take = first_pref < n_ready ? first_pref + 1u : n_ready;
        uint32_t val = lane < take ? (uint32_t)(st & 0xFFFFFFFFull) : 0u;
#pragma unroll
        for (int o = 32; o > 0; o >>= 1) val += __shfl_xor(val, o, 64);
        sum += val;
        if (first_pref < n_ready) return sum;
        p -= (int64_t)take;
        if (take == 0) __builtin_amdgcn_s_sleep(2);
    }
}

template <int TPB, bool PREFETCH>
__global__ void __launch_bounds__(TPB, (TPB == 512 ? 4 : 2)) k_group_buckets(const uint64_t *__restrict__ keys_in, const uint32_t *__restrict__ vals_in,
                                                       const uint32_t *__restrict__ bstart, uint32_t nbuckets,
                                                       uint32_t shift_lo, uint32_t bits_lo, uint32_t shift_hi, uint32_t bits_hi,
                                                       GroupRng rng, uint32_t do_fix, uint32_t *__restrict__ ticket, unsigned long long *__restrict__ status,
                                                       uint32_t *__restrict__ big_list, uint32_t *__restrict__ n_big,
                                                       uint32_t *__restrict__ vals_out, uint8_t *__restrict__ tz_out,
                                                       uint64_t *__restrict__ uniq, uint32_t *__restrict__ counts, uint32_t *__restrict__ starts,
                                                       uint32_t *__restrict__ n_runs_out, uint32_t by_class,
                                                       uint32_t *__restrict__ brun , uint32_t *__restrict__ bnr ) {
    constexpr uint32_t ITEMS = GR_TILE / TPB, NW = TPB / 64, SEG = 64 * ITEMS, NB = 1u << GR_LOCAL_BITS;
    static_assert(ITEMS * NW == 64, "the segment scan below is one wavefront wide");
    __shared__ uint64_t s_keys[GR_TILE];
    __shared__ uint32_t s_vals[GR_TILE];
    __shared__ uint16_t s_wcnt[2][NW * NB];
    __shared__ unsigned long long s_wmask[NW * NB];
    __shared__ uint16_t s_dstart[NB];
    __shared__ uint32_t s_wsum[NW], s_seg[ITEMS * NW], s_misc[3], s_fixn, s_redo;
    __shared__ uint16_t s_fixlist[64];
    __shared__ uint32_t s_cls[16];
    const uint32_t w = threadIdx.x >> 6, lane = threadIdx.x & 63u;
    for (uint32_t d = threadIdx.x; d < NW * NB; d += TPB) { s_wmask[d] = 0ull; s_wcnt[0][d] = 0; s_wcnt[1][d] = 0; }
    uint32_t c = 0, b0 = 0, b1 = 0;
    uint64_t k[ITEMS];
    uint32_t v[ITEMS], dig[ITEMS], rank[ITEMS];
    auto load_bucket = [&](uint32_t cc, uint32_t &bb0, uint32_t &bb1, uint64_t (&kk)[ITEMS], uint32_t (&vv)[ITEMS]) {
        bb0 = bstart[cc]; bb1 = bstart[cc + 1u];
        const uint32_t n = bb1 - bb0 > GR_TILE ? 0u : bb1 - bb0;
#pragma unroll
        for (uint32_t r = 0; r < ITEMS; ++r) {
            const uint32_t j = w * SEG + r * 64u + lane;
            const bool ok = j < n;
            kk[r] = ok ? keys_in[bb0 + j] : 0ull;
            vv[r] = ok ? vals_in[bb0 + j] : 0u;
        }
    };
    if (PREFETCH) {
        if (threadIdx.x == 0) s_misc[0] = atomicAdd(ticket, 1u);
        __syncthreads();
        c = s_misc[0];
        if (c >= nbuckets) return;
        load_bucket(c, b0, b1, k, v);
    }
    for (;;) {
    __syncthreads();
    if (threadIdx.x == 0) { s_misc[PREFETCH ? 2 : 0] = atomicAdd(ticket, 1u); s_fixn = 0; s_redo = 0; }
    __syncthreads();
    if (!PREFETCH) {
        c = s_misc[0];
        if (c >= nbuckets) return;
        load_bucket(c, b0, b1, k, v);
    }
    const uint32_t c_next = PREFETCH ? s_misc[2] : 0u;
    const bool big = b1 - b0 > GR_TILE;
    const uint32_t cn = big ? 0u : b1 - b0;
    const uint32_t rows = cn > w * SEG ? min(ITEMS, (cn - w * SEG + 63u) / 64u) : 0u;
    if (big && threadIdx.x == 0) big_list[atomicAdd(n_big, 1u)] = c;
    bool in_lds = false;
    auto sort_pass = [&](uint32_t shift, uint32_t bits, uint16_t *wcnt) {
        if (bits == 0 || cn == 0) return;
        const uint32_t nb = 1u << bits;
        if (in_lds) {
#pragma unroll
            for (uint32_t r = 0; r < ITEMS; ++r) {
                const uint32_t j = w * SEG + r * 64u + lane;
                if (j < cn) { k[r] = s_keys[j]; v[r] = s_vals[j]; }
            }
        }
#pragma unroll
        for (uint32_t r = 0; r < ITEMS; ++r) {
            const uint32_t j = w * SEG + r * 64u + lane;
            dig[r] = j < cn ? gr_digit(k[r], shift, bits) : ~0u;
        }
        gr_wave_rank_lds<ITEMS>(dig, rank, wcnt + w * nb, s_wmask + w * NB, rows);
        __syncthreads();
        gr_digit_offsets<TPB>(wcnt, s_dstart, nb, s_wsum);
        __syncthreads();
#pragma unroll
        for (uint32_t r = 0; r < ITEMS; ++r)
            if (dig[r] != ~0u) {
                const uint32_t p = (uint32_t)s_dstart[dig[r]] + (uint32_t)wcnt[w * nb + dig[r]] + rank[r];
                s_keys[p] = k[r]; s_vals[p] = v[r];
            }
        __syncthreads();
        for (uint32_t d = threadIdx.x; d < NW * nb; d += TPB) wcnt[d] = 0;
        in_lds = true;
    };
    auto fix_groups = [&](uint32_t gshift, uint32_t gbits) {
#pragma unroll
        for (uint32_t i = 0; i < ITEMS; ++i) {
            const uint32_t j = i * TPB + threadIdx.x;
            if (j == 0u || j >= cn) continue;
            const uint64_t k1 = s_keys[j], k0 = s_keys[j - 1u];
            if (k1 != k0 && gr_digit(k0, gshift, gbits) == gr_digit(k1, gshift, gbits)) {
                const uint32_t slot = atomicAdd(&s_fixn, 1u);
                if (slot < 64u) s_fixlist[slot] = (uint16_t)j;
            }
        }
        __syncthreads();
        const uint32_t nfix = min(s_fixn, 64u);
        if (s_fixn > 64u && threadIdx.x == 0) s_redo = 1u;
        for (uint32_t m0 = 0; m0 < nfix; m0 += NW) {
            const uint32_t m = m0 + w;
            uint64_t key = 0;
            uint32_t val = 0, dst = ~0u;
            if (m < nfix) {
                const uint32_t j = s_fixlist[m];
                const int pos = (int)j - 32 + (int)lane;
                const bool valid = pos >= 0 && pos < (int)cn;
                key = valid ? s_keys[pos] : 0ull;
                val = valid ? s_vals[pos] : 0u;
                const uint64_t kj = __shfl(key, 32, 64), k0 = __shfl(key, 31, 64);
                const unsigned long long same = __ballot(valid && gr_digit(key, gshift, gbits) == gr_digit(kj, gshift, gbits));
                const uint32_t nl = ~(uint32_t)same, nr = ~(uint32_t)(same >> 32);
                const uint32_t lrun = nl ? (uint32_t)__builtin_clz(nl) : 32u;
                const uint32_t rrun = nr ? (uint32_t)__builtin_ctz(nr) : 32u;
                const uint32_t a0 = 32u - lrun, e0 = 32u + rrun;
                const unsigned long long left = ((1ull << 32) - 1ull) & ~((1ull << a0) - 1ull);
                const unsigned long long eq0 = __ballot(key == k0);
                if (lrun + rrun > 32u) {
                    if (lane == 0) s_redo = 1u;
                } else if ((eq0 & left) == left) {
                    uint32_t rk = 0;
                    for (uint32_t q = a0; q < e0; ++q) {
                        const uint64_t kq = ((uint64_t)(uint32_t)__builtin_amdgcn_readlane((int)(uint32_t)(key >> 32), (int)q) << 32) |
                                            (uint32_t)__builtin_amdgcn_readlane((int)(uint32_t)key, (int)q);
                        rk += (kq < key || (kq == key && q < lane)) ? 1u : 0u;
                    }
                    if (lane >= a0 && lane < e0) dst = (uint32_t)((int)j - 32 + (int)a0) + rk;
                }
            }
            __syncthreads();
            if (dst != ~0u) { s_keys[dst] = key; s_vals[dst] = val; }
            __syncthreads();
        }
    };
    if (!(GR_ABL & 16)) sort_pass(shift_lo, bits_lo, s_wcnt[0]);
    if (!(GR_ABL & 20)) sort_pass(shift_hi, bits_hi, s_wcnt[1]);
    if (!in_lds) {
#pragma unroll
        for (uint32_t r = 0; r < ITEMS; ++r) {
            const uint32_t j = w * SEG + r * 64u + lane;
            if (j < cn) { s_keys[j] = k[r]; s_vals[j] = v[r]; }
        }
        __syncthreads();
    }
    if (do_fix && cn && !(GR_ABL & 2)) {
        fix_groups(shift_lo, bits_lo + bits_hi);
        if (do_fix > 1u && s_redo) {
            __syncthreads();
            if (threadIdx.x == 0) { s_fixn = 0; s_redo = 0; }
            sort_pass(shift_lo - GR_LOCAL_BITS, GR_LOCAL_BITS, s_wcnt[0]);
            sort_pass(shift_lo, bits_lo, s_wcnt[1]);
            sort_pass(shift_hi, bits_hi, s_wcnt[0]);
            fix_groups(shift_lo - GR_LOCAL_BITS, bits_lo + bits_hi + GR_LOCAL_BITS);
        }
    }
    uint32_t nb0 = 0, nb1 = 0;
    if (PREFETCH && c_next < nbuckets) load_bucket(c_next, nb0, nb1, k, v);
    unsigned long long hb[ITEMS];
    uint32_t occ[ITEMS];
    bool head[ITEMS];
#pragma unroll
    for (uint32_t i = 0; i < ITEMS; ++i) {
        const uint32_t j = i * TPB + threadIdx.x;
        head[i] = false; occ[i] = 0;
        if (j < cn) {
            const uint64_t key = s_keys[j];
            head[i] = j == 0u || s_keys[j - 1u] != key;
            occ[i] = s_vals[j];
        }
        hb[i] = __ballot(head[i]);
        if (lane == 0) s_seg[i * NW + w] = (uint32_t)__popcll(hb[i]);
    }
    __syncthreads();
    if (w == 0) {
        const uint32_t mine = s_seg[lane];
        uint32_t inc = mine;
#pragma unroll
        for (int o = 1; o < 64; o <<= 1) { const uint32_t t = __shfl_up(inc, o, 64); if ((int)lane >= o) inc += t; }
        s_seg[lane] = inc - mine;
        if (lane == 63u) {
            s_misc[1] = inc;
            if (status) __hip_atomic_store(&status[c], (c == 0 ? GR_ST_PREFIX : GR_ST_AGG) | (unsigned long long)inc, __ATOMIC_RELAXED, __HIP_MEMORY_SCOPE_AGENT);
            else s_misc[0] = atomicAdd(n_runs_out, inc);
        }
    }
    __syncthreads();
    const uint32_t nruns = s_misc[1];
    uint16_t *hpos = reinterpret_cast<uint16_t *>(s_vals);
#pragma unroll
    for (uint32_t i = 0; i < ITEMS; ++i)
        if (head[i]) hpos[s_seg[i * NW + w] + gr_lanes_below(hb[i])] = (uint16_t)(i * TPB + threadIdx.x);
    if (w == 0 && status) {
        uint32_t rb_ = 0;
        if (c != 0 && !(GR_ABL & 1)) rb_ = gr_look_back(status, c);
        if (lane == 0) {
            s_misc[0] = rb_;
            if (c != 0) __hip_atomic_store(&status[c], GR_ST_PREFIX | (unsigned long long)(rb_ + nruns), __ATOMIC_RELAXED, __HIP_MEMORY_SCOPE_AGENT);
            if (c == nbuckets - 1u) *n_runs_out = rb_ + nruns;
        }
    }
    const uint32_t pmask = (1u << rng.pos_bits) - 1u;
#pragma unroll
    for (uint32_t i = 0; i < ITEMS; ++i) {
        const uint32_t j = i * TPB + threadIdx.x;
        if (j < cn && !(GR_ABL & 8)) {
            vals_out[b0 + j] = occ[i];
            const uint32_t rr = rng31(rng.seed, rng.ordinal0 + (uint64_t)(occ[i] >> rng.pos_bits), occ[i] & pmask) | 0x8000u;
            tz_out[b0 + j] = (uint8_t)(__ffs((int)rr) - 1);
        }
    }
    __syncthreads();
    const uint32_t run_base = s_misc[0];
    if (brun && threadIdx.x == 0) { brun[c] = run_base; bnr[c] = nruns; }
    if (by_class && nruns > 64u && nruns != cn) {
        if (threadIdx.x < 16u) s_cls[threadIdx.x] = 0u;
        __syncthreads();
        for (uint32_t i = threadIdx.x; i < nruns; i += TPB) {
            const uint32_t j = hpos[i], e = i + 1u < nruns ? (uint32_t)hpos[i + 1u] : cn;
            atomicAdd(&s_cls[min(7u, 32u - (uint32_t)__clz((int)(e - j - 1u)))], 1u);
        }
        __syncthreads();
        if (threadIdx.x == 0) { uint32_t run = 0; for (int q = 7; q >= 0; --q) { const uint32_t t = s_cls[q]; s_cls[q] = run; run += t; } }
        __syncthreads();
        for (uint32_t i = threadIdx.x; i < nruns; i += TPB) {
            const uint32_t j = hpos[i], e = i + 1u < nruns ? (uint32_t)hpos[i + 1u] : cn;
            const uint32_t q = min(7u, 32u - (uint32_t)__clz((int)(e - j - 1u)));
            const uint32_t slot = run_base + s_cls[q] + atomicAdd(&s_cls[8u + q], 1u);
            uniq[slot] = s_keys[j];
            starts[slot] = b0 + j;
            counts[slot] = e - j;
        }
    } else
    for (uint32_t i = threadIdx.x; i < nruns; i += TPB) {
        const uint32_t j = hpos[i], e = i + 1u < nruns ? (uint32_t)hpos[i + 1u] : cn;
        uniq[run_base + i] = s_keys[j];
        starts[run_base + i] = b0 + j;
        counts[run_base + i] = e - j;
    }
    if (PREFETCH) {
        if (c_next >= nbuckets) return;
        c = c_next; b0 = nb0; b1 = nb1;
    }
    }
}

template <int TPB>
__global__ void __launch_bounds__(TPB) k_group_big(uint64_t *keys_a, uint32_t *vals_a, uint64_t *keys_b, uint32_t *vals_b,
                                                   const uint32_t *__restrict__ bstart, const uint32_t *__restrict__ big_list,
                                                   const uint32_t *__restrict__ n_big_dev,
                                                   uint32_t shift_lo, uint32_t bits_lo, uint32_t shift_hi, uint32_t bits_hi, GroupRng rng,
                                                   uint32_t *__restrict__ vals_out, uint8_t *__restrict__ tz_out,
                                                   uint64_t *__restrict__ uniq, uint32_t *__restrict__ counts, uint32_t *__restrict__ starts,
                                                   uint32_t *__restrict__ run_cursor) {
    constexpr uint32_t ITEMS = GR_TILE / TPB, NW = TPB / 64, SEG = 64 * ITEMS, NB = 1u << GR_LOCAL_BITS;
    __shared__ uint64_t s_keys[GR_TILE];
    __shared__ uint16_t s_hpos[GR_TILE];
    __shared__ uint16_t s_wcnt[NW * NB];
    __shared__ unsigned long long s_wmask[NW * NB];
    __shared__ uint32_t s_hist[NB], s_dbase[NB], s_tot[NB];
    __shared__ uint32_t s_wsum[NW], s_seg[ITEMS * NW], s_misc[4];
    __shared__ uint64_t s_carry_key;
    const uint32_t w = threadIdx.x >> 6, lane = threadIdx.x & 63u;
    for (uint32_t d = threadIdx.x; d < NW * NB; d += TPB) s_wmask[d] = 0ull;
    const uint32_t n_big = *n_big_dev;
    const uint32_t pmask = (1u << rng.pos_bits) - 1u;
    for (uint32_t bi = blockIdx.x; bi < n_big; bi += gridDim.x) {
        const uint32_t c = big_list[bi], b0 = bstart[c], b1 = bstart[c + 1u];
        uint64_t *ksrc = keys_a, *kdst = keys_b;
        uint32_t *vsrc = vals_a, *vdst = vals_b;
        for (int pass = 0; pass < 2; ++pass) {
            const uint32_t shift = pass ? shift_hi : shift_lo, bits = pass ? bits_hi : bits_lo;
            if (bits == 0) continue;
            const uint32_t nb = 1u << bits;
            __syncthreads();
            for (uint32_t d = threadIdx.x; d < nb; d += TPB) s_hist[d] = 0;
            __syncthreads();
            for (uint32_t x = b0 + threadIdx.x; x < b1; x += TPB) atomicAdd(&s_hist[gr_digit(ksrc[x], shift, bits)], 1u);
            __syncthreads();
            {
                const uint32_t per = (nb + TPB - 1) / TPB;
                uint32_t vsum = 0;
                if (threadIdx.x * per < nb) vsum = s_hist[threadIdx.x];
                const uint32_t ex = gr_block_excl_scan<TPB>(vsum, s_wsum);
                if (threadIdx.x < nb) s_dbase[threadIdx.x] = ex;
            }
            __syncthreads();
            for (uint32_t p0 = b0; p0 < b1; p0 += GR_TILE) {
                const uint32_t cn = min(GR_TILE, b1 - p0);
                const uint32_t rows = cn > w * SEG ? min(ITEMS, (cn - w * SEG + 63u) / 64u) : 0u;
                uint64_t k[ITEMS];
                uint32_t v[ITEMS], dig[ITEMS], rank[ITEMS];
#pragma unroll
                for (uint32_t r = 0; r < ITEMS; ++r) {
                    const uint32_t j = w * SEG + r * 64u + lane;
                    const bool ok = j < cn;
                    k[r] = ok ? ksrc[p0 + j] : 0ull;
                    v[r] = ok ? vsrc[p0 + j] : 0u;
                    dig[r] = ok ? gr_digit(k[r], shift, bits) : ~0u;
                }
                for (uint32_t d = threadIdx.x; d < NW * nb; d += TPB) s_wcnt[d] = 0;
                __syncthreads();
                gr_wave_rank_lds<ITEMS>(dig, rank, s_wcnt + w * nb, s_wmask + w * NB, rows);
                __syncthreads();
                if (threadIdx.x < nb) {
                    uint32_t run = 0;
#pragma unroll
                    for (uint32_t ww = 0; ww < NW; ++ww) { const uint32_t t = s_wcnt[ww * nb + threadIdx.x]; s_wcnt[ww * nb + threadIdx.x] = (uint16_t)run; run += t; }
                    s_tot[threadIdx.x] = run;
                }
                __syncthreads();
#pragma unroll
                for (uint32_t r = 0; r < ITEMS; ++r)
                    if (dig[r] != ~0u) {
                        const uint32_t g = b0 + s_dbase[dig[r]] + (uint32_t)s_wcnt[w * nb + dig[r]] + rank[r];
                        kdst[g] = k[r]; vdst[g] = v[r];
                    }
                __syncthreads();
                if (threadIdx.x < nb) s_dbase[threadIdx.x] += s_tot[threadIdx.x];
                __syncthreads();
            }
            { uint64_t *t = ksrc; ksrc = kdst; kdst = t; }
            { uint32_t *t = vsrc; vsrc = vdst; vdst = t; }
            __threadfence();
            __syncthreads();
        }
        uint32_t carry_start = b0;
        for (uint32_t p0 = b0; p0 < b1; p0 += GR_TILE) {
            const uint32_t cn = min(GR_TILE, b1 - p0);
            const bool first = p0 == b0;
            __syncthreads();
            for (uint32_t j = threadIdx.x; j < cn; j += TPB) s_keys[j] = ksrc[p0 + j];
            __syncthreads();
            unsigned long long hb[ITEMS];
            bool head[ITEMS];
            const uint64_t ckey = first ? 0ull : s_carry_key;
#pragma unroll
            for (uint32_t i = 0; i < ITEMS; ++i) {
                const uint32_t j = i * TPB + threadIdx.x;
                head[i] = false;
                if (j < cn) {
                    const uint64_t key = s_keys[j];
                    head[i] = j == 0u ? (first || key != ckey) : s_keys[j - 1u] != key;
                    const uint32_t occ = vsrc[p0 + j];
                    vals_out[p0 + j] = occ;
                    const uint32_t rr = rng31(rng.seed, rng.ordinal0 + (uint64_t)(occ >> rng.pos_bits), occ & pmask) | 0x8000u;
                    tz_out[p0 + j] = (uint8_t)(__ffs((int)rr) - 1);
                }
                hb[i] = __ballot(head[i]);
                if (lane == 0) s_seg[i * NW + w] = (uint32_t)__popcll(hb[i]);
            }
            __syncthreads();
            if (threadIdx.x == 0) {
                uint32_t run = 0;
                for (uint32_t q = 0; q < ITEMS * NW; ++q) { const uint32_t t = s_seg[q]; s_seg[q] = run; run += t; }
                s_misc[1] = run;
                const uint32_t closed = run - (first ? 1u : 0u);
                s_misc[0] = closed ? atomicAdd(run_cursor, closed) : 0u;
            }
            __syncthreads();
            const uint32_t nheads = s_misc[1], base = s_misc[0];
#pragma unroll
            for (uint32_t i = 0; i < ITEMS; ++i)
                if (head[i]) s_hpos[s_seg[i * NW + w] + gr_lanes_below(hb[i])] = (uint16_t)(i * TPB + threadIdx.x);
            __syncthreads();
            for (uint32_t i = threadIdx.x; i < nheads; i += TPB) {
                const uint32_t j = s_hpos[i];
                if (i == 0u) {
                    if (!first) { uniq[base] = ckey; starts[base] = carry_start; counts[base] = p0 + j - carry_start; }
                } else {
                    const uint32_t jp = s_hpos[i - 1u], slot = base + i - (first ? 1u : 0u);
                    uniq[slot] = s_keys[jp]; starts[slot] = p0 + jp; counts[slot] = j - jp;
                }
            }
            __syncthreads();
            if (nheads) {
                const uint32_t jl = s_hpos[nheads - 1u];
                carry_start = p0 + jl;
                if (threadIdx.x == 0) s_carry_key = s_keys[jl];
            }
        }
        __syncthreads();
        if (threadIdx.x == 0) {
            const uint32_t slot = atomicAdd(run_cursor, 1u);
            uniq[slot] = s_carry_key; starts[slot] = carry_start; counts[slot] = b1 - carry_start;
        }
        __syncthreads();
    }
}

struct GroupPlan {
    uint32_t n = 0, T = 0;
    uint32_t t_lo = 0, t_hi = 0;
    uint32_t shift_lo = 0, shift_hi = 0;
    uint32_t l_lo = 0, l_hi = 0, lshift_lo = 0, lshift_hi = 0;
    uint32_t ntiles = 0, ntiles2_max = 0, nbuckets = 1;
    bool dead = false;
    uint32_t tpb = 256;
    uint32_t fix_cap = 0;
    int xcd_map = 1;
    size_t hist_entries = 0;
    size_t off_status = 0, off_ticket = 0, off_bstart = 0, off_big = 0, off_hist = 0, off_goffs = 0, off_scan = 0, off_desc = 0, off_segtb = 0, off_segst = 0,
           scan_bytes = 0, total = 0;
};
static size_t gr_align(size_t x) { return (x + 255) / 256 * 256; }

static GroupPlan group_plan(size_t N, int group_bits, int bucket_target = 0, int flags = 0, int force_T = -1) {
    GroupPlan P;
    P.n = (uint32_t)N;
    P.dead = (flags & GR_FLAG_DEAD) != 0;
    const uint32_t gb = (uint32_t)std::max(1, std::min<int>(group_bits, (int)GR_MAX_GROUP_BITS));
    uint32_t T = 0;
    const size_t target = getenv("RB_GROUP_TARGET") ? (size_t)std::max(64, std::min(atoi(getenv("RB_GROUP_TARGET")), (int)GR_TILE))
                        : bucket_target > 0 ? (size_t)bucket_target : (size_t)GR_BUCKET_TARGET;
    while ((target << T) < N) ++T;
    if (const char *e = getenv("RB_GROUP_T")) T = (uint32_t)std::max(0, atoi(e));
    if (force_T >= 0) T = (uint32_t)force_T;
    T = std::min({T, gb, 2u * GR_PART_MAX_BITS});
    if (P.dead && T == 0) T = 1;
    P.T = T;
    if (T <= GR_PART_MAX_BITS) { P.t_hi = T; P.t_lo = 0; }
    else { P.t_hi = (T + 1u) / 2u; P.t_lo = T - P.t_hi; }
    P.shift_hi = GR_KEY_TOP - P.t_hi;
    P.shift_lo = GR_KEY_TOP - T;
    const uint32_t L = std::min(gb - T, 2u * GR_LOCAL_BITS);
    P.l_hi = (L + 1u) / 2u;
    P.l_lo = L - P.l_hi;
    P.lshift_hi = GR_KEY_TOP - T - P.l_hi;
    P.lshift_lo = GR_KEY_TOP - T - L;
    P.tpb = getenv("RB_GROUP_TPB") ? (uint32_t)atoi(getenv("RB_GROUP_TPB")) : 512u;
    if (P.tpb != 256u) P.tpb = 512u;
    P.xcd_map = getenv("RB_GROUP_XCD") ? atoi(getenv("RB_GROUP_XCD")) : 1;
    P.fix_cap = L == 2u * GR_LOCAL_BITS ? (bucket_target > 0 ? 2u : 1u) : 0u;
    if (const char *e = getenv("RB_GROUP_FIX")) P.fix_cap = (uint32_t)std::max(0, std::min(atoi(e), 2));
    P.ntiles = (uint32_t)((N + GR_TILE - 1) / GR_TILE);
    P.ntiles2_max = P.t_lo ? P.ntiles + (1u << P.t_hi) : 0;
    P.nbuckets = 1u << T;
    if (T) P.hist_entries = std::max((size_t)P.ntiles << P.t_hi, (size_t)P.ntiles2_max << P.t_lo) + 2;
    size_t o = 0;
    P.off_status = o; o += gr_align((size_t)P.nbuckets * 8);
    P.off_ticket = o; o += 256;
    P.off_bstart = o; o += gr_align(((size_t)P.nbuckets + 1) * 4);
    P.off_big = o; o += gr_align((size_t)P.nbuckets * 4);
    if (T) {
        P.off_hist = o; o += gr_align(P.hist_entries * 4);
        P.off_goffs = o; o += gr_align(P.hist_entries * 4);
        P.scan_bytes = gr_align(scan_temp_bytes(P.hist_entries));
        P.off_scan = o; o += P.scan_bytes;
        if (P.t_lo) {
            P.off_desc = o; o += gr_align((size_t)P.ntiles2_max * sizeof(GrTile));
            P.off_segtb = o; o += gr_align(((size_t)(1u << P.t_hi) + 1) * 4);
            P.off_segst = o; o += gr_align(((size_t)(1u << P.t_hi) + 1) * 4);
        }
    }
    P.total = o;
    return P;
}

void group_debug_big(const void *temp, size_t N, int group_bits, int bucket_target, uint32_t *n_big_out, uint64_t *records_out, uint32_t *largest_out, int flags) {
    const GroupPlan P = group_plan(N, group_bits, bucket_target, flags);
    const char *tp = static_cast<const char *>(temp);
    uint32_t tick[4] = {0, 0, 0, 0};
    RB_HIP(hipMemcpy(tick, tp + P.off_ticket, 16, hipMemcpyDeviceToHost));
    const uint32_t nb = std::min(tick[2], P.nbuckets);
    std::vector<uint32_t> big(nb), bs((size_t)P.nbuckets + 1);
    if (nb) RB_HIP(hipMemcpy(big.data(), tp + P.off_big, (size_t)nb * 4, hipMemcpyDeviceToHost));
    RB_HIP(hipMemcpy(bs.data(), tp + P.off_bstart, ((size_t)P.nbuckets + 1) * 4, hipMemcpyDeviceToHost));
    uint64_t rec = 0; uint32_t mx = 0;
    for (uint32_t i = 0; i < nb; ++i) { const uint32_t c = bs[big[i] + 1] - bs[big[i]]; rec += c; mx = std::max(mx, c); }
    *n_big_out = nb; *records_out = rec; *largest_out = mx;
}
size_t group_temp_bytes(size_t N, int group_bits, int bucket_target, int flags) { return group_plan(N, group_bits, bucket_target, flags).total; }
const uint32_t *group_live_count(const void *temp, size_t N, int group_bits, int bucket_target, int flags) {
    const GroupPlan P = group_plan(N, group_bits, bucket_target, flags);
    return reinterpret_cast<const uint32_t *>(static_cast<const char *>(temp) + P.off_ticket) + 3;
}

template <int TPB>
static void part_pass(const GrTiling &tl, size_t entries, uint32_t shift, uint32_t bits, const uint64_t *kin, const uint32_t *vin, uint64_t *kout,
                      uint32_t *vout, uint32_t *hist, uint32_t *goffs, void *scan_tmp, size_t scan_bytes, hipStream_t st, rb_graph *prof,
                      uint32_t *n_live_dev = nullptr ,
                      GrIdxDev ix = GrIdxDev{Mod{1, 0, 0}, 0, 0, 0, 0}, uint64_t derive_kmul = 0 ) {
    const dim3 grid(tl.grid_tiles), blk(TPB);
    if (prof) prof->prof_begin(st);
    if (n_live_dev) RB_HIP(hipMemsetAsync(hist + entries, 0, 4, st));
    if (derive_kmul) hipLaunchKernelGGL((k_part_count<TPB, true>), grid, blk, 0, st, kin, tl, shift, bits, hist, (const uint32_t *)nullptr, ix, derive_kmul);
    else hipLaunchKernelGGL(k_part_count<TPB>, grid, blk, 0, st, kin, tl, shift, bits, hist, n_live_dev ? vin : (const uint32_t *)nullptr, ix);
    if (prof) { prof->prof_end("group_part_count", st); prof->prof_begin(st); }
    exclusive_scan_u32(scan_tmp, scan_bytes, hist, goffs, entries + (n_live_dev ? 1 : 0), st);
    if (n_live_dev) hipLaunchKernelGGL(k_copy_u32, dim3(1), dim3(64), 0, st, n_live_dev, goffs + entries);
    if (prof) { prof->prof_end("group_scan", st); prof->prof_begin(st); }
    const uint32_t wide = !(getenv("RB_GROUP_WIDE_LDS") && atoi(getenv("RB_GROUP_WIDE_LDS")) == 0);
    if (derive_kmul) {
        if (bits <= 8u) hipLaunchKernelGGL((k_part_scatter<TPB, 8, true>), grid, blk, 0, st, kin, (const uint32_t *)nullptr, tl, shift, bits, goffs, kout, vout, wide, 0u, ix, derive_kmul);
        else hipLaunchKernelGGL((k_part_scatter<TPB, GR_PART_MAX_BITS, true>), grid, blk, 0, st, kin, (const uint32_t *)nullptr, tl, shift, bits, goffs, kout, vout, wide, 0u, ix, derive_kmul);
    } else if (bits <= 8u) hipLaunchKernelGGL((k_part_scatter<TPB, 8>), grid, blk, 0, st, kin, vin, tl, shift, bits, goffs, kout, vout, wide, n_live_dev ? 1u : 0u, ix);
    else hipLaunchKernelGGL((k_part_scatter<TPB, GR_PART_MAX_BITS>), grid, blk, 0, st, kin, vin, tl, shift, bits, goffs, kout, vout, wide, n_live_dev ? 1u : 0u, ix);
    if (prof) prof->prof_end("group_part_scatter", st);
}

namespace {
struct LsdPlan {
    uint32_t ntiles = 0, n_pass = 0, shift[16], bits[16];
    size_t entries = 0, off_hist = 0, off_goffs = 0, off_scan = 0, scan_bytes = 0, off_idx = 0, total = 0;
};
LsdPlan lsd_plan(size_t n, const int (*ranges)[2], int n_ranges, bool idx_vals) {
    LsdPlan P;
    P.ntiles = (uint32_t)((n + GR_TILE - 1) / GR_TILE);
    uint32_t maxbits = 0;
    for (int r = 0; r < n_ranges; ++r) {
        const uint32_t B = (uint32_t)std::max(0, ranges[r][1] - ranges[r][0]);
        const uint32_t maxb = n <= ((size_t)1 << 20) ? 8u : GR_PART_MAX_BITS;
        const uint32_t np = (B + maxb - 1) / maxb;
        uint32_t lo = (uint32_t)ranges[r][0], left = B;
        for (uint32_t q = 0; q < np; ++q) {
            const uint32_t b = (left + (np - q) - 1) / (np - q);
            P.shift[P.n_pass] = lo; P.bits[P.n_pass] = b; ++P.n_pass;
            lo += b; left -= b;
            maxbits = std::max(maxbits, b);
        }
    }
    P.entries = ((size_t)P.ntiles << maxbits) + 2;
    size_t o = 0;
    P.off_hist = o; o += gr_align(P.entries * 4);
    P.off_goffs = o; o += gr_align(P.entries * 4);
    P.scan_bytes = gr_align(scan_temp_bytes(P.entries));
    P.off_scan = o; o += P.scan_bytes;
    if (idx_vals) { P.off_idx = o; o += 2 * gr_align(n * 4); }
    P.total = o;
    return P;
}
void lsd_sort(const LsdPlan &P, char *tp, uint64_t *k_in, uint64_t *k_out, uint32_t *v_in, uint32_t *v_out, size_t n, hipStream_t st) {
    uint32_t *hist = reinterpret_cast<uint32_t *>(tp + P.off_hist), *goffs = reinterpret_cast<uint32_t *>(tp + P.off_goffs);
    const GrTiling tl{nullptr, nullptr, (uint32_t)n, P.ntiles, gr_grid_for_tiles(P.ntiles), 1};
    uint64_t *ka = k_in, *kb = k_out;
    uint32_t *va = v_in, *vb = v_out;
    for (uint32_t q = 0; q < P.n_pass; ++q) {
        part_pass<512>(tl, (size_t)P.ntiles << P.bits[q], P.shift[q], P.bits[q], ka, va, kb, vb, hist, goffs, tp + P.off_scan, P.scan_bytes, st, nullptr);
        std::swap(ka, kb); std::swap(va, vb);
    }
    if ((P.n_pass & 1u) == 0) {
        RB_HIP(hipMemcpyAsync(k_out, k_in, n * 8, hipMemcpyDeviceToDevice, st));
        if (v_in && v_out) RB_HIP(hipMemcpyAsync(v_out, v_in, n * 4, hipMemcpyDeviceToDevice, st));
    }
}
__global__ void k_lsd_iota(uint32_t *__restrict__ v, size_t n) {
    const size_t i = (size_t)blockIdx.x * blockDim.x + threadIdx.x;
    if (i < n) v[i] = (uint32_t)i;
}
__global__ void k_lsd_gather64(const uint32_t *__restrict__ idx, const uint64_t *__restrict__ src, uint64_t *__restrict__ dst, size_t n) {
    const size_t i = (size_t)blockIdx.x * blockDim.x + threadIdx.x;
    if (i < n) dst[i] = src[idx[i]];
}
}

size_t sort_pairs_temp_bytes(size_t n) { const int r[1][2] = {{0, 64}}; return lsd_plan(n, r, 1, false).total; }
size_t sort_keys_temp_bytes(size_t n) { return sort_pairs_temp_bytes(n); }
size_t sort_pairs32_temp_bytes(size_t n) { const int r[1][2] = {{0, 64}}; return lsd_plan(n, r, 1, true).total; }
void sort_pairs_u64_u32(void *temp, size_t temp_bytes, uint64_t *keys_in, uint64_t *keys_out, uint32_t *vals_in, uint32_t *vals_out, size_t n,
                        int begin_bit, int end_bit, hipStream_t s) {
    if (n == 0) return;
    RB_REQUIRE(n < (1ull << 32) - 2 * GR_TILE, "sort_pairs_u64_u32: too many records");
    const int r[1][2] = {{begin_bit, end_bit}};
    const LsdPlan P = lsd_plan(n, r, 1, false);
    RB_REQUIRE(temp_bytes >= P.total, "sort_pairs_u64_u32: temp too small");
    lsd_sort(P, static_cast<char *>(temp), keys_in, keys_out, vals_in, vals_out, n, s);
}
void sort_pairs_u64_u32_2r(void *temp, size_t temp_bytes, uint64_t *keys_in, uint64_t *keys_out, uint32_t *vals_in, uint32_t *vals_out, size_t n,
                           int lo_begin, int lo_end, int hi_begin, int hi_end, hipStream_t s) {
    if (n == 0) return;
    RB_REQUIRE(n < (1ull << 32) - 2 * GR_TILE, "sort_pairs_u64_u32_2r: too many records");
    const int r[2][2] = {{lo_begin, lo_end}, {hi_begin, hi_end}};
    const LsdPlan P = lsd_plan(n, r, 2, false);
    RB_REQUIRE(temp_bytes >= P.total, "sort_pairs_u64_u32_2r: temp too small");
    lsd_sort(P, static_cast<char *>(temp), keys_in, keys_out, vals_in, vals_out, n, s);
}
void sort_keys_u64(void *temp, size_t temp_bytes, uint64_t *keys_in, uint64_t *keys_out, size_t n, int begin_bit, int end_bit, hipStream_t s) {
    sort_pairs_u64_u32(temp, temp_bytes, keys_in, keys_out, nullptr, nullptr, n, begin_bit, end_bit, s);
}
void sort_pairs_u64_u64(void *temp, size_t temp_bytes, uint64_t *keys_in, uint64_t *keys_out, uint64_t *vals_in, uint64_t *vals_out, size_t n,
                        int begin_bit, int end_bit, hipStream_t s) {
    if (n == 0) return;
    RB_REQUIRE(n < (1ull << 32) - 2 * GR_TILE, "sort_pairs_u64_u64: too many records");
    const int r[1][2] = {{begin_bit, end_bit}};
    const LsdPlan P = lsd_plan(n, r, 1, true);
    RB_REQUIRE(temp_bytes >= P.total, "sort_pairs_u64_u64: temp too small");
    char *tp = static_cast<char *>(temp);
    uint32_t *i0 = reinterpret_cast<uint32_t *>(tp + P.off_idx), *i1 = reinterpret_cast<uint32_t *>(tp + P.off_idx + gr_align(n * 4));
    hipLaunchKernelGGL(k_lsd_iota, dim3((unsigned)((n + 255) / 256)), dim3(256), 0, s, i0, n);
    lsd_sort(P, tp, keys_in, keys_out, i0, i1, n, s);
    hipLaunchKernelGGL(k_lsd_gather64, dim3((unsigned)((n + 255) / 256)), dim3(256), 0, s, i1, vals_in, vals_out, n);
}

static GrIdxDev gr_idx_dev(const GroupPlan &P, const GrIdx &idx) {
    if (idx.span > (1ull << P.T))
        return GrIdxDev{idx.mod, idx.lo, (uint64_t)((((unsigned __int128)1 << 64) << P.T) / idx.span), (1u << P.T) - 1u, P.t_lo};
    return GrIdxDev{Mod{1, 0, 0}, 0, 0, 0, 0};
}
template <int TPB>
static uint32_t *partition_records(const GroupPlan &P, uint64_t *keys0, uint32_t *vals0, uint64_t *keys_tmp, uint32_t *vals_tmp, char *tp, hipStream_t st,
                                   rb_graph *prof, GrIdx idx, const uint64_t **kin_out, const uint32_t **vin_out,
                                   const uint64_t *derive_src = nullptr, uint64_t derive_kmul = 0 ) {
    unsigned long long *status = reinterpret_cast<unsigned long long *>(tp + P.off_status);
    uint32_t *ticket = reinterpret_cast<uint32_t *>(tp + P.off_ticket);
    uint32_t *bstart = reinterpret_cast<uint32_t *>(tp + P.off_bstart);
    RB_HIP(hipMemsetAsync(status, 0, P.off_bstart, st));
    const uint64_t *kin = derive_src ? derive_src : keys0;
    const uint32_t *vin = derive_src ? nullptr : vals0;
    if (P.T) {
        uint32_t *hist = reinterpret_cast<uint32_t *>(tp + P.off_hist), *goffs = reinterpret_cast<uint32_t *>(tp + P.off_goffs);
        void *scan_tmp = tp + P.off_scan;
        GrTiling t1{nullptr, nullptr, P.n, P.ntiles, gr_grid_for_tiles(P.ntiles), P.xcd_map};
        uint32_t *n_live = P.dead ? ticket + 3 : nullptr;
        GrIdxDev ix = gr_idx_dev(P, idx);
        part_pass<TPB>(t1, (size_t)P.ntiles << P.t_hi, P.shift_hi, P.t_hi, kin, vin, keys_tmp, vals_tmp, hist, goffs, scan_tmp, P.scan_bytes, st, prof, n_live, ix, derive_src ? derive_kmul : 0);
        kin = keys_tmp; vin = vals_tmp;
        uint32_t *segtb = nullptr, *segst = nullptr;
        if (P.t_lo) {
            GrTile *desc = reinterpret_cast<GrTile *>(tp + P.off_desc);
            segtb = reinterpret_cast<uint32_t *>(tp + P.off_segtb); segst = reinterpret_cast<uint32_t *>(tp + P.off_segst);
            uint32_t *nt2 = ticket + 1;
            hipLaunchKernelGGL(k_seg_tiles, dim3(1), dim3(1024), 0, st, goffs, P.ntiles, 1u << P.t_hi, P.n, 1u << P.t_lo, desc, segtb, segst, nt2, (const uint32_t *)n_live);
            RB_HIP(hipMemsetAsync(hist, 0, ((size_t)P.ntiles2_max << P.t_lo) * 4, st));
            GrTiling t2{desc, nt2, P.n, P.ntiles2_max, gr_grid_for_tiles(P.ntiles2_max), P.xcd_map};
            ix.shift = 0;
            part_pass<TPB>(t2, (size_t)P.ntiles2_max << P.t_lo, P.shift_lo, P.t_lo, kin, vin, keys0, vals0, hist, goffs, scan_tmp, P.scan_bytes, st, prof, nullptr, ix);
            kin = keys0; vin = vals0;
        }
        hipLaunchKernelGGL(k_bucket_bounds, dim3((P.nbuckets + 256u) / 256u), dim3(256), 0, st, goffs, P.ntiles, segtb, segst, P.t_hi, P.t_lo, P.n, bstart, (const uint32_t *)n_live);
    } else
        hipLaunchKernelGGL(k_bucket_bounds, dim3(1), dim3(64), 0, st, (const uint32_t *)nullptr, 0u, (const uint32_t *)nullptr, (const uint32_t *)nullptr, 0u, 0u, P.n, bstart);
    *kin_out = kin; *vin_out = vin;
    return bstart;
}

template <int TPB>
static void group_records_impl(const GroupPlan &P, uint64_t *keys0, uint32_t *vals0, uint64_t *keys_tmp, uint32_t *vals_tmp, GroupRng rng, char *tp,
                               uint32_t *vals_out, uint8_t *tz_out, uint64_t *uniq, uint32_t *counts, uint32_t *starts, uint32_t *n_runs_dev,
                               hipStream_t st, rb_graph *prof, GrIdx idx, GroupExport ex) {
    unsigned long long *status = reinterpret_cast<unsigned long long *>(tp + P.off_status);
    uint32_t *ticket = reinterpret_cast<uint32_t *>(tp + P.off_ticket);
    const uint64_t *kin = nullptr;
    const uint32_t *vin = nullptr;
    uint32_t *bstart = partition_records<TPB>(P, keys0, vals0, keys_tmp, vals_tmp, tp, st, prof, idx, &kin, &vin);
    uint32_t *big_list = reinterpret_cast<uint32_t *>(tp + P.off_big), *n_big = ticket + 2;
    if (prof) prof->prof_begin(st);
    const uint32_t bucket_grid = std::min(P.nbuckets, (uint32_t)(getenv("RB_GROUP_GRID") ? atoi(getenv("RB_GROUP_GRID")) : 768));
    const bool ordered = getenv("RB_GROUP_ORDERED") && atoi(getenv("RB_GROUP_ORDERED")) != 0;
    if (!ordered) RB_HIP(hipMemsetAsync(n_runs_dev, 0, 4, st));
    const bool prefetch = !(getenv("RB_GROUP_PREFETCH") && atoi(getenv("RB_GROUP_PREFETCH")) == 0);
    const uint32_t by_class = getenv("RB_GROUP_CLASSES") ? (uint32_t)(atoi(getenv("RB_GROUP_CLASSES")) != 0) : 1u;
    if (ordered || !prefetch)
        hipLaunchKernelGGL((k_group_buckets<TPB, false>), dim3(bucket_grid), dim3(TPB), 0, st, kin, vin, bstart, P.nbuckets, P.lshift_lo, P.l_lo, P.lshift_hi, P.l_hi,
                           rng, P.fix_cap, ticket, ordered ? status : nullptr, big_list, n_big, vals_out, tz_out, uniq, counts, starts, n_runs_dev, 0u, ex.brun, ex.bnr);
    else
        hipLaunchKernelGGL((k_group_buckets<TPB, true>), dim3(bucket_grid), dim3(TPB), 0, st, kin, vin, bstart, P.nbuckets, P.lshift_lo, P.l_lo, P.lshift_hi, P.l_hi,
                           rng, P.fix_cap, ticket, nullptr, big_list, n_big, vals_out, tz_out, uniq, counts, starts, n_runs_dev, by_class, ex.brun, ex.bnr);
    if (ex.n_main) hipLaunchKernelGGL(k_copy_u32, dim3(1), dim3(64), 0, st, ex.n_main, n_runs_dev);
    if (prof) { prof->prof_end("group_buckets", st); prof->prof_begin(st); }
    uint64_t *ka = const_cast<uint64_t *>(kin), *kb = kin == keys0 ? keys_tmp : keys0;
    uint32_t *va = const_cast<uint32_t *>(vin), *vb = vin == vals0 ? vals_tmp : vals0;
    hipLaunchKernelGGL(k_group_big<512>, dim3(std::min(P.nbuckets, 2048u)), dim3(512), 0, st, ka, va, kb, vb, bstart, big_list, n_big,
                       P.lshift_lo, P.l_lo, P.lshift_hi, P.l_hi, rng, vals_out, tz_out, uniq, counts, starts, n_runs_dev);
    if (prof) prof->prof_end("group_big_buckets", st);
    RB_HIP(hipGetLastError());
}

void group_records_device(uint64_t *keys0, uint32_t *vals0, uint64_t *keys_tmp, uint32_t *vals_tmp, size_t N, int group_bits,
                          uint64_t seed, uint64_t ordinal0, uint32_t pos_bits, void *temp, size_t temp_bytes,
                          uint32_t *vals_out, uint8_t *tz_out, uint64_t *uniq, uint32_t *counts, uint32_t *starts, uint32_t *n_runs_dev,
                          hipStream_t st, rb_graph *prof, int bucket_target, int flags, GrIdx idx, GroupExport ex) {
    RB_REQUIRE(N > 0 && N < (1ull << 32) - 2 * GR_TILE, "group_records_device: bad record count");
    const GroupPlan P = group_plan(N, group_bits, bucket_target, flags);
    RB_REQUIRE(temp_bytes >= P.total, "group_records_device: temp too small");
    const GroupRng rng{seed, ordinal0, pos_bits};
    if (P.tpb == 512u) group_records_impl<512>(P, keys0, vals0, keys_tmp, vals_tmp, rng, static_cast<char *>(temp), vals_out, tz_out, uniq, counts, starts, n_runs_dev, st, prof, idx, ex);
    else group_records_impl<256>(P, keys0, vals0, keys_tmp, vals_tmp, rng, static_cast<char *>(temp), vals_out, tz_out, uniq, counts, starts, n_runs_dev, st, prof, idx, ex);
}
uint32_t group_index_buckets(size_t N, int group_bits, int bucket_target, int flags, GrIdx idx) {
    const GroupPlan P = group_plan(N, group_bits, bucket_target, flags);
    return (P.T && idx.span > (1ull << P.T)) ? P.T : 0u;
}
void group_debug_plan(size_t N, int group_bits, int bucket_target, int flags, GrIdx idx, uint32_t out[7]) {
    const GroupPlan P = group_plan(N, group_bits, bucket_target, flags);
    out[0] = P.T; out[1] = P.t_hi; out[2] = P.t_lo; out[3] = P.l_hi; out[4] = P.l_lo; out[5] = P.fix_cap;
    out[6] = (P.T && gr_idx_dev(P, idx).mul != 0) ? 1u : 0u;
}

constexpr uint32_t SW_WORDS = 16384;
constexpr uint32_t SW_MARKS = 1024;
__device__ __forceinline__ uint32_t sw_digit(uint64_t x, const GrIdxDev &ix) {
    return min((uint32_t)min(__umul64hi(x, ix.mul), (uint64_t)0xFFFFFFFFull), ix.top);
}
__device__ __forceinline__ uint64_t sw_first(uint32_t c, const GrIdxDev &ix, uint64_t span, uint32_t T) {
    if (c == 0u) return 0ull;
    if (c > ix.top) return span;
    uint64_t e = ((uint64_t)c * span) >> T;
    while (e > 0ull && sw_digit(e - 1ull, ix) >= c) --e;
    while (e < span && sw_digit(e, ix) < c) ++e;
    return e;
}
template <int TPB>
__global__ void __launch_bounds__(TPB, 4) k_sweep_bits(uint32_t *words, GrIdxDev ix, uint64_t span, uint32_t T, const uint64_t *__restrict__ uniq,
                                                    const uint32_t *__restrict__ brun, const uint32_t *__restrict__ bnr,
                                                    const uint64_t *__restrict__ k1, const uint32_t *__restrict__ v1, const uint32_t *__restrict__ bstart1,
                                                    uint8_t *st0, uint8_t *st1, uint32_t SWW ) {
    extern __shared__ __attribute__((aligned(16))) uint32_t sw_lds[];
    uint32_t *s_w = sw_lds, *s_c = sw_lds + SWW, *s_t = sw_lds + SWW + SW_MARKS;
    __shared__ uint32_t s_any;
    const uint32_t c = blockIdx.x;
    const uint32_t r0 = brun[c], nr = bnr[c], p0 = bstart1[c], p1 = bstart1[c + 1u];
    if (nr == 0u && p0 == p1) return;
    const uint64_t x_lo = sw_first(c, ix, span, T), x_hi = sw_first(c + 1u, ix, span, T);
    const uint64_t w_lo = (x_lo >> 5) & ~3ull, w_hi = (x_hi + 31ull) >> 5;
    const uint64_t in_lo = (x_lo + 31ull) >> 5, in_hi = x_hi >> 5;
    constexpr uint32_t KEEP = GR_TILE / TPB;
    constexpr uint32_t NONE = ~0u;
    static_assert(KEEP <= 16, "one mask bit per remembered probe");
    const uint64_t bit0 = w_lo << 5;
    uint32_t i0[KEEP], i1[KEEP];
    {
        uint64_t h[KEEP];
#pragma unroll
        for (uint32_t it = 0; it < KEEP; ++it) { const uint32_t r = it * TPB + threadIdx.x; h[it] = r < nr ? uniq[r0 + r] : 0ull; }
#pragma unroll
        for (uint32_t it = 0; it < KEEP; ++it) { const uint32_t r = it * TPB + threadIdx.x; i0[it] = r < nr ? (uint32_t)(index_of(h[it], ix.mod) - ix.lo - bit0) : NONE; }
#pragma unroll
        for (uint32_t it = 0; it < KEEP; ++it) { const uint32_t j = p0 + it * TPB + threadIdx.x; h[it] = j < p1 ? k1[j] : 0ull; }
#pragma unroll
        for (uint32_t it = 0; it < KEEP; ++it) { const uint32_t j = p0 + it * TPB + threadIdx.x; i1[it] = j < p1 ? (uint32_t)(index_of(h[it], ix.mod) - ix.lo - bit0) : NONE; }
    }
    for (uint64_t wb = w_lo; wb < w_hi; wb += SWW) {
        const uint32_t cnt = (uint32_t)min((uint64_t)SWW, w_hi - wb);
        const uint32_t wrel = (uint32_t)(wb - w_lo);
        for (uint32_t i = threadIdx.x * 4u; i < cnt; i += TPB * 4u) {
            if (i + 4u <= cnt) *reinterpret_cast<uint4 *>(s_w + i) = *reinterpret_cast<const uint4 *>(words + wb + i);
            else for (uint32_t q = i; q < cnt; ++q) s_w[q] = words[wb + q];
        }
        for (uint32_t i = threadIdx.x; i < 2u * SW_MARKS; i += TPB) s_c[i] = 0u;
        if (threadIdx.x == 0) s_any = 0u;
        __syncthreads();
        auto probe = [&](uint32_t rel) -> int {
            const uint32_t w = (rel >> 5) - wrel;
            if (rel == NONE || w >= cnt) return -1;
            const uint32_t m = 1u << (rel & 31u);
            if (!(atomicOr(&s_w[w], m) & m)) return 0;
            if (__hip_atomic_load(&words[w_lo + (rel >> 5)], __ATOMIC_RELAXED, __HIP_MEMORY_SCOPE_AGENT) & m) {
                if (atomicOr(&s_t[w & (SW_MARKS - 1u)], m) & m) { atomicOr(&s_c[w & (SW_MARKS - 1u)], m); s_any = 1u; return 4; }
                return 1;
            }
            atomicOr(&s_c[w & (SW_MARKS - 1u)], m); s_any = 1u;
            return 2;
        };
        uint32_t setmask = 0, premask = 0;
#pragma unroll
        for (uint32_t it = 0; it < KEEP; ++it) {
            const int s = probe(i0[it]);
            if (s >= 0) st0[r0 + it * TPB + threadIdx.x] = (uint8_t)s;
            if (s == 0) setmask |= 1u << it;
            if (s == 1) premask |= 1u << it;
        }
#pragma unroll
        for (uint32_t it = 0; it < KEEP; ++it) {
            const int s = probe(i1[it]);
            if (s > 0) st1[v1[p0 + it * TPB + threadIdx.x]] = (uint8_t)s;
            if (s == 0) setmask |= 1u << (16u + it);
            if (s == 1) premask |= 1u << (16u + it);
        }
        for (uint32_t j = p0 + KEEP * TPB + threadIdx.x; j < p1; j += TPB) {
            const int s = probe((uint32_t)(index_of(k1[j], ix.mod) - ix.lo - bit0));
            if (s > 0) st1[v1[j]] = (uint8_t)s;
        }
        __syncthreads();
        if (s_any) {
            auto marked = [&](uint32_t rel) { return ((s_c[((rel >> 5) - wrel) & (SW_MARKS - 1u)] >> (rel & 31u)) & 1u) != 0u; };
#pragma unroll
            for (uint32_t it = 0; it < KEEP; ++it) {
                if (((setmask >> it) & 1u) && marked(i0[it])) st0[r0 + it * TPB + threadIdx.x] = 3;
                if (((premask >> it) & 1u) && marked(i0[it])) st0[r0 + it * TPB + threadIdx.x] = 4;
                if (((setmask >> (16u + it)) & 1u) && marked(i1[it])) st1[v1[p0 + it * TPB + threadIdx.x]] = 3;
                if (((premask >> (16u + it)) & 1u) && marked(i1[it])) st1[v1[p0 + it * TPB + threadIdx.x]] = 4;
            }
            for (uint32_t j = p0 + KEEP * TPB + threadIdx.x; j < p1; j += TPB) {
                const uint32_t rel = (uint32_t)(index_of(k1[j], ix.mod) - ix.lo - bit0);
                if ((rel >> 5) - wrel < cnt && marked(rel)) {
                    const uint32_t d = v1[j];
                    if (st1[d] == 0) st1[d] = 3; else if (st1[d] == 1) st1[d] = 4;
                }
            }
        }
        for (uint32_t i = threadIdx.x * 4u; i < cnt; i += TPB * 4u) {
            const uint64_t gw = wb + i;
            if (gw >= in_lo && gw + 4ull <= in_hi) *reinterpret_cast<uint4 *>(words + gw) = *reinterpret_cast<const uint4 *>(s_w + i);
            else
                for (uint32_t q = 0; q < 4u && i + q < cnt; ++q) {
                    const uint64_t g = gw + q;
                    if (g >= in_lo && g < in_hi) words[g] = s_w[i + q];
                    else if ((g << 5) < x_hi && ((g + 1ull) << 5) > x_lo) atomicOr(&words[g], s_w[i + q]);
                }
        }
        __syncthreads();
    }
}
__global__ void k_sw_big_pre(const uint32_t *__restrict__ words, Mod mod, uint64_t lo, const uint64_t *__restrict__ uniq, uint32_t d0, uint32_t D, uint8_t *__restrict__ st0) {
    const uint32_t d = d0 + blockIdx.x * blockDim.x + threadIdx.x;
    if (d >= D) return;
    const uint64_t i0 = index_of(uniq[d], mod) - lo;
    st0[d] = (words[i0 >> 5] >> (uint32_t)(i0 & 31ull)) & 1u;
}
__global__ void k_sw_big_set(uint32_t *__restrict__ words, Mod mod, uint64_t lo, const uint64_t *__restrict__ uniq, uint32_t d0, uint32_t D, uint8_t *__restrict__ st0) {
    const uint32_t d = d0 + blockIdx.x * blockDim.x + threadIdx.x;
    if (d >= D || st0[d]) return;
    const uint64_t i0 = index_of(uniq[d], mod) - lo;
    const uint32_t m = 1u << (uint32_t)(i0 & 31ull);
    if (atomicOr(&words[i0 >> 5], m) & m) st0[d] = 2;
}
size_t sweep_temp_bytes(size_t D, uint32_t T) { return group_plan(D, 64, 0, 0, (int)T).total; }
void sweep_bits_device(uint32_t *words, GrIdx idx, uint32_t T, uint64_t kmul, const uint64_t *uniq, uint32_t D, uint32_t n_main, const uint32_t *brun,
                       const uint32_t *bnr, uint64_t *keys_a, uint32_t *vals_a, uint64_t *keys_b, uint32_t *vals_b, void *temp, size_t temp_bytes,
                       uint8_t *st0, uint8_t *st1, hipStream_t st) {
    RB_REQUIRE(D > 0 && T > 0 && idx.span > (1ull << T) && (idx.span >> T) < (1ull << 31), "sweep_bits_device: nothing to sweep by / ranges of 2^31 bits and more");
    const GroupPlan P = group_plan(D, 64, 0, 0, (int)T);
    RB_REQUIRE(P.T == T && temp_bytes >= P.total, "sweep_bits_device: plan / temp mismatch");
    RB_HIP(hipMemsetAsync(st1, 0, D, st));
    RB_REQUIRE(kmul != 0, "sweep_bits_device: kmul");
    const uint64_t *k1 = nullptr;
    const uint32_t *v1 = nullptr;
    const uint32_t *bstart1 = P.tpb == 512u ? partition_records<512>(P, keys_a, vals_a, keys_b, vals_b, static_cast<char *>(temp), st, nullptr, idx, &k1, &v1, uniq, kmul)
                                            : partition_records<256>(P, keys_a, vals_a, keys_b, vals_b, static_cast<char *>(temp), st, nullptr, idx, &k1, &v1, uniq, kmul);
    GrIdxDev ix = gr_idx_dev(P, idx);
    const uint32_t n_big = D - std::min(n_main, D);
    if (n_big) hipLaunchKernelGGL(k_sw_big_pre, dim3((n_big + 255u) / 256u), dim3(256), 0, st, (const uint32_t *)words, idx.mod, idx.lo, uniq, n_main, D, st0);
    const uint64_t range_words = (idx.span >> T) / 32 + 16;
    const uint32_t sww = (uint32_t)std::min<uint64_t>(SW_WORDS, (range_words + 1023) / 1024 * 1024);
    RB_HIP(hipFuncSetAttribute(reinterpret_cast<const void *>(k_sweep_bits<512>), hipFuncAttributeMaxDynamicSharedMemorySize, (int)((SW_WORDS + 2 * SW_MARKS) * 4)));
    hipLaunchKernelGGL(k_sweep_bits<512>, dim3(P.nbuckets), dim3(512), (sww + 2 * SW_MARKS) * 4, st, words, ix, idx.span, T, uniq, brun, bnr, k1, v1, bstart1, st0, st1, sww);
    if (n_big) hipLaunchKernelGGL(k_sw_big_set, dim3((n_big + 255u) / 256u), dim3(256), 0, st, words, idx.mod, idx.lo, uniq, n_main, D, st0);
    RB_HIP(hipGetLastError());
}

}
```

### rna-bloom_amd/csrc/rb_internal.hpp

```cpp
#pragma once
#include <hip/hip_runtime.h>
#include <stdint.h>
#include <stdio.h>
#include <stdlib.h>

#include <algorithm>
#include <memory>
#include <mutex>
#include <string>
#include <unordered_map>
#include <utility>
#include <vector>

#include "../../include/rb_capi.h"
#include "rb_device.hpp"

namespace rb {

struct HostPin {
    void *p = nullptr;
    static bool pinned_already(const void *ptr) {
        hipPointerAttribute_t a;
        const bool yes = hipPointerGetAttributes(&a, ptr) == hipSuccess && a.type == hipMemoryTypeHost;
        (void)hipGetLastError();
// ... 100 lines not shown
    const uint32_t *end() const { return data() + size(); }
    void assign(size_t n, uint32_t v) { ext = nullptr; own.assign(n, v); }
    void resize(size_t n) { ext = nullptr; own.resize(n); }
    HostWoff &operator=(const std::vector<uint32_t> &v) { ext = nullptr; own = v; return *this; }
    void borrow(uint32_t *p, size_t n) { own.clear(); ext = p; ext_n = n; }
};

struct SlabPin {
    static constexpr uintptr_t SLAB = (uintptr_t)256 << 20;
    uintptr_t hi = 0, done = 0;
    bool on = false;
    std::vector<void *> pins;
    void begin(const void *p, size_t bytes) {
        on = false;
        if (!p || bytes <= ((size_t)16 << 20) || getenv("RB_NO_PIN")) return;
        hipPointerAttribute_t a;
        const bool pinned = hipPointerGetAttributes(&a, p) == hipSuccess && a.type == hipMemoryTypeHost;
        (void)hipGetLastError();
        if (pinned) return;
        done = reinterpret_cast<uintptr_t>(p); hi = done + bytes; on = true;
    }
    void pin_to(const void *upto) {
        const uintptr_t need = std::min(reinterpret_cast<uintptr_t>(upto), hi);
        while (on && done < need) {
            const uintptr_t a = done, e = std::min(hi, (a & ~(SLAB - 1)) + SLAB);
            if (hipHostRegister(reinterpret_cast<void *>(a), (size_t)(e - a), hipHostRegisterDefault) == hipSuccess) pins.push_back(reinterpret_cast<void *>(a));
            else { (void)hipGetLastError(); on = false; }
            done = e;
        }
    }
    void end() { for (void *q : pins) (void)hipHostUnregister(q); pins.clear(); on = false; }
    ~SlabPin() { end(); }
    static hipError_t copy(void *dst, const char *src, size_t n, hipStream_t st) {
        for (size_t o = 0; o < n;) {
            const uintptr_t at = reinterpret_cast<uintptr_t>(src + o);
            const size_t m = std::min<size_t>(n - o, (size_t)(((at & ~(SLAB - 1)) + SLAB) - at));
            const hipError_t e = hipMemcpyAsync(static_cast<char *>(dst) + o, src + o, m, hipMemcpyHostToDevice, st);
            if (e != hipSuccess) return e;
            o += m;
        }
        return hipSuccess;
    }
};

struct DevPool {
    std::mutex m;
    std::vector<std::pair<void *, size_t>> free_;
    std::unordered_map<void *, size_t> out;
    size_t held = 0, limit = (size_t)12 << 30;
    void *get(size_t bytes) {
        bytes = std::max<size_t>((bytes + ((size_t)2 << 20) - 1) & ~(((size_t)2 << 20) - 1), (size_t)2 << 20);
        {
            std::lock_guard<std::mutex> lk(m);
            size_t best = free_.size();
            for (size_t i = 0; i < free_.size(); ++i)
                if (free_[i].second >= bytes && free_[i].second <= 2 * bytes && (best == free_.size() || free_[i].second < free_[best].second)) best = i;
            if (best != free_.size()) {
                void *p = free_[best].first; const size_t cap = free_[best].second;
                free_.erase(free_.begin() + (std::ptrdiff_t)best);
                held -= cap; out[p] = cap;
                return p;
            }
        }
        void *p = nullptr;
        hipError_t e = hipMalloc(&p, bytes);
        if (e != hipSuccess) { clear(); e = hipMalloc(&p, bytes); }
        if (e != hipSuccess) { (void)hipGetLastError(); rb::set_error("hipMalloc of %zu bytes failed: %s", bytes, hipGetErrorString(e)); throw rb::HipError{RB_ERR_NOMEM}; }
        std::lock_guard<std::mutex> lk(m);
        out[p] = bytes;
        return p;
    }
    void put(void *p) {
        if (!p) return;
        size_t cap = 0;
        {
            std::lock_guard<std::mutex> lk(m);
            auto it = out.find(p);
            if (it != out.end()) { cap = it->second; out.erase(it); }
            if (cap && held + cap <= limit) { free_.push_back({p, cap}); held += cap; return; }
        }
        (void)hipFree(p);
    }
    void clear() {
        std::vector<std::pair<void *, size_t>> f;
        { std::lock_guard<std::mutex> lk(m); f.swap(free_); held = 0; }
        for (auto &b : f) (void)hipFree(b.first);
    }
    ~DevPool() { clear(); }
};

struct IngestHost {
    uint32_t *woff = nullptr, *len = nullptr;
    int64_t *rel = nullptr;
    size_t cap = 0;
    void reserve(size_t n) {
        if (n <= cap) return;
        release();
        const size_t want = n + (n >> 2) + 1024;
        void *p = nullptr;
        if (hipHostMalloc(&p, want * 16, hipHostMallocDefault) != hipSuccess) { (void)hipGetLastError(); rb::set_error("hipHostMalloc of %zu bytes failed", want * 16); throw rb::HipError{RB_ERR_NOMEM}; }
        rel = static_cast<int64_t *>(p); woff = reinterpret_cast<uint32_t *>(rel + want); len = woff + want;
        cap = want;
    }
    void release() { if (rel) (void)hipHostFree(rel); rel = nullptr; woff = len = nullptr; cap = 0; }
    ~IngestHost() { release(); }
};

struct rb_batch {
    int device = 0;
    DevPool *pool = nullptr;
    int64_t n_reads = 0, n_bases = 0, n_words = 0;
    uint32_t max_len = 0;
    uint32_t wpr_uniform = 0;
    uint64_t *codes = nullptr;
    uint32_t *valid = nullptr;
    uint32_t *rnz = nullptr;
    uint32_t *word_read = nullptr;
    uint32_t *woff = nullptr;
    uint32_t *len = nullptr;
    size_t device_bytes = 0;
    HostWoff h_woff;
};
namespace rb {
struct BatchDestroy { void operator()(rb_batch *p) const { (void)rb_batch_destroy(p); } };
using BatchPtr = std::unique_ptr<rb_batch, BatchDestroy>;
}

namespace rb {

size_t sort_pairs_temp_bytes(size_t n);
void sort_pairs_u64_u32(void *temp, size_t temp_bytes, uint64_t *keys_in, uint64_t *keys_out,
                        uint32_t *vals_in, uint32_t *vals_out, size_t n, int begin_bit, int end_bit,
                        hipStream_t s);
void sort_pairs_u64_u32_2r(void *temp, size_t temp_bytes, uint64_t *keys_in, uint64_t *keys_out, uint32_t *vals_in, uint32_t *vals_out, size_t n,
                           int lo_begin, int lo_end, int hi_begin, int hi_end, hipStream_t s);
size_t sort_pairs32_temp_bytes(size_t n);
void sort_pairs_u64_u64(void *temp, size_t temp_bytes, uint64_t *keys_in, uint64_t *keys_out,
                        uint64_t *vals_in, uint64_t *vals_out, size_t n, int begin_bit, int end_bit,
                        hipStream_t s);
size_t sort_keys_temp_bytes(size_t n);
void sort_keys_u64(void *temp, size_t temp_bytes, uint64_t *keys_in, uint64_t *keys_out, size_t n, int begin_bit,
                   int end_bit, hipStream_t s);
size_t scan_temp_bytes(size_t n);
void exclusive_scan_u32(void *temp, size_t temp_bytes, const uint32_t *in, uint32_t *out, size_t n,
                        hipStream_t s);
size_t select_temp_bytes(size_t n);
void select_flagged(void *temp, size_t temp_bytes, const uint32_t *status, uint32_t mask, size_t n, uint32_t *out,
                    uint32_t *count_dev, hipStream_t s);
size_t select2_temp_bytes(size_t n);
void select_flagged2(void *temp, size_t temp_bytes, const uint32_t *status, size_t n, uint32_t mask_a, uint32_t *out_a,
                     uint32_t mask_b, uint32_t *out_b, uint32_t *count_dev, hipStream_t s);

constexpr int GR_FLAG_DEAD = 1;
struct GrIdx {
    Mod mod;
    uint64_t lo = 0, span = 0;
};
struct GroupExport { uint32_t *brun = nullptr, *bnr = nullptr, *n_main = nullptr; };
void group_debug_big(const void *temp, size_t N, int group_bits, int bucket_target, uint32_t *n_big_out, uint64_t *records_out, uint32_t *largest_out, int flags = 0);
size_t group_temp_bytes(size_t N, int group_bits, int bucket_target = 0, int flags = 0);
const uint32_t *group_live_count(const void *temp, size_t N, int group_bits, int bucket_target, int flags);
void group_records_device(uint64_t *keys0, uint32_t *vals0, uint64_t *keys_tmp, uint32_t *vals_tmp, size_t N, int group_bits,
                          uint64_t seed, uint64_t ordinal0, uint32_t pos_bits, void *temp, size_t temp_bytes,
                          uint32_t *vals_out, uint8_t *tz_out, uint64_t *uniq, uint32_t *counts, uint32_t *starts, uint32_t *n_runs_dev,
                          hipStream_t st, struct rb_graph *prof = nullptr ,
                          int bucket_target = 0 , int flags = 0 ,
                          GrIdx idx = GrIdx{Mod{1, 0, 0}, 0, 0} ,
                          GroupExport ex = GroupExport{});
uint32_t group_index_buckets(size_t N, int group_bits, int bucket_target, int flags, GrIdx idx);
void group_debug_plan(size_t N, int group_bits, int bucket_target, int flags, GrIdx idx, uint32_t out[7]);
size_t sweep_temp_bytes(size_t D, uint32_t T);
void sweep_bits_device(uint32_t *words, GrIdx idx, uint32_t T, uint64_t kmul, const uint64_t *uniq, uint32_t D, uint32_t n_main, const uint32_t *brun,
                       const uint32_t *bnr, uint64_t *keys_a, uint32_t *vals_a, uint64_t *keys_b, uint32_t *vals_b, void *temp, size_t temp_bytes,
                       uint8_t *st0, uint8_t *st1, hipStream_t st);

}
```

### rna-bloom_amd/csrc/rb_pipeline.hpp

```cpp
#pragma once
#include <string.h>

#include <algorithm>
#include <condition_variable>
#include <mutex>
#include <new>
#include <shared_mutex>
#include <functional>
#include <memory>
#include <string>
#include <thread>
#include <vector>

#include "rb_internal.hpp"
#include "rb_kernels.hpp"

namespace rb {

constexpr int TPB = 256;
constexpr size_t DEVCTR_BYTES = 4096;
inline unsigned blocks_for(int64_t n, int tpb = TPB) { return (unsigned)((n + tpb - 1) / tpb); }

struct BitFilter {
    uint32_t *bits = nullptr;
// ... 145 lines not shown
    atomicAnd(w, ~(CLAIM << (8u * (uint32_t)(idx & 3u))));
}

constexpr uint32_t ST_CLAIMED = 1u << 9, ST_FOREIGN = 1u << 10;
constexpr uint32_t ST_LATE = 1u << 11, ST_LATE_FOUND = 1u << 16;
constexpr uint32_t RUN_CONFLICT = 1u << 17, RUN_RELEASE = 1u << 18, RUN_WRITES = 1u << 19, RUN_HEAVY = 1u << 20;


template <typename F> int guarded(F &&f) {
    try { f(); return RB_OK; }
    catch (const HipError &e) { return e.code; }
    catch (const std::bad_alloc &) { set_error("host allocation failed"); return RB_ERR_NOMEM; }
}
void alloc_bits(BitFilter &f, int64_t bits, int num_hash, int64_t lo, int64_t hi);
void free_bits(BitFilter &f);
const char *last_error_text();
BitFilter *bit_filter(rb_graph *g, int which);
uint64_t *upload_h0(rb_graph *g, DevBuf &buf, const uint64_t *h0, size_t n, hipStream_t st = nullptr);
void fast_zero(void *p, size_t bytes, hipStream_t s);
void add_reads_streamed(rb_graph *g, const char *seq, const char *qual, const int64_t *offsets, int64_t n_reads, int min_base_qual, int64_t piece_bases,
                        unsigned flags, rb_add_stats *stats);
void add_range(rb_graph *g, const rb_batch *b, int64_t first, int64_t n, unsigned flags, rb_add_stats *stats);
void run_pipeline(rb_graph *g, size_t N, int mode, uint64_t ordinal0, uint32_t pos_bits, rb_add_stats *stats);
void launch_pairs_reads(rb_graph *g, const rb_batch *b, int64_t w0, int64_t nw, int mode_hash, const BitFilter &f, int dist,
                        uint32_t min_len, bool if_present, const uint32_t *chunk_off, uint64_t *out_idx, unsigned long long *pc, hipStream_t st);
__global__ void k_bits_add(uint32_t *bits, Mod mod, int num_hash, uint64_t kmul, const uint64_t *__restrict__ h0, size_t n);
void alloc_pair_seen(BitFilter &f);
void seen_reset(BitFilter &f, hipStream_t s);
static __global__ void __launch_bounds__(64) k_cbf_heavy(FilterView fv, const uint64_t *__restrict__ uniq,
                            const uint32_t *__restrict__ counts, const uint32_t *__restrict__ starts,
                            const uint32_t *__restrict__ vals, const uint32_t *__restrict__ status,
                            const uint32_t *__restrict__ nops, const uint64_t *__restrict__ cvals,
                            const uint8_t *__restrict__ tz, const uint32_t *__restrict__ heavy_list,
                            const uint32_t *__restrict__ counters, uint64_t *__restrict__ cfinal,
                            uint8_t *__restrict__ cache_upd = nullptr ) {
    const uint32_t n_heavy = counters[0];
    const uint32_t lane = threadIdx.x;
    for (uint32_t hi = blockIdx.x; hi < n_heavy; hi += gridDim.x) {
        const uint32_t d = heavy_list[hi];
        const uint64_t h0 = uniq[d];
        const uint32_t ops = nops[d];
        const uint32_t st = status[d];
        const uint64_t cv = cvals[d];
        uint64_t idx[RB_MAX_HASH];
        uint32_t c[RB_MAX_HASH];
        for (int j = 0; j < fv.cbf_h; ++j) {
            idx[j] = index_of(multi_hash(h0, (uint32_t)j, fv.kmul), fv.cbf_mod);
            c[j] = (uint32_t)(cv >> (8 * j)) & 0xFFu;
        }
        const uint32_t base = starts[d] + counts[d] - ops;
        const uint32_t krest = (st >> 14) & 3u;
        uint32_t done = 0;
        {
            uint32_t mn = c[0];
            for (int j = 1; j < fv.cbf_h; ++j) mn = c[j] < mn ? c[j] : mn;
            const uint32_t k0 = (st >> 12) & 3u;
            const bool gate = !((k0 == K_INC_IF_POS && mn == 0u) || (k0 == K_INC_IF_ZERO && mn != 0u));
            if (gate && mn < 127u && (mn < 16u || tz[base] >= (mn >> 3) - 1u))
                for (int j = 0; j < fv.cbf_h; ++j) if (c[j] == mn) c[j] = mn + 1u;
            done = 1;
        }
        while (done < ops) {
            uint32_t mn = c[0];
            for (int j = 1; j < fv.cbf_h; ++j) mn = c[j] < mn ? c[j] : mn;
            if (mn >= 127u) break;
            if (krest == K_INC_IF_POS && mn == 0u) break;
            if (krest == K_INC_IF_ZERO && mn != 0u) break;
            if (mn < 16u) {
                cbf_step(c, fv.cbf_h, krest, 0u);
                ++done;
                continue;
            }
            const uint32_t shift = (mn >> 3) - 1u;
            const uint32_t pos = base + done, end = base + ops;
            const uint32_t a0 = pos & ~7u;
            const uint32_t mine = a0 + 8u * lane;
            uint32_t hit = 0xFFFFFFFFu;
            if (mine < end) {
                uint64_t w = *reinterpret_cast<const uint64_t *>(tz + mine);
                uint64_t m = (w + (uint64_t)(0x80u - shift) * 0x0101010101010101ull) & 0x8080808080808080ull;
                if (mine < pos) m &= ~0ull << (8u * (pos - mine));
                if (m) { uint32_t q = mine + ((uint32_t)__ffsll((long long)m) - 1u) / 8u; if (q < end) hit = q; }
            }
            const unsigned long long win = __ballot(hit != 0xFFFFFFFFu);
            if (!win) { done = (a0 + 512u) - base; continue; }
            const uint32_t first_lane = (uint32_t)__ffsll((long long)win) - 1u;
            const uint32_t q = __shfl(hit, (int)first_lane, 64);
            cbf_step(c, fv.cbf_h, krest, 0u);
            done = q - base + 1u;
        }
        if (lane == 0) {
            if (cfinal) {
                uint64_t out = 0;
                for (int j = 0; j < fv.cbf_h; ++j) out |= (uint64_t)c[j] << (8 * j);
                cfinal[d] = out;
            } else
                for (int j = 0; j < fv.cbf_h; ++j) {
                    if (c[j] == ((uint32_t)(cv >> (8 * j)) & 0xFFu)) cbf_release(fv.cbf, idx[j]);
                    else fv.cbf[idx[j]] = (uint8_t)c[j];
                }
            if (cache_on(fv) && (st & ST_ALLPRE)) {
                uint32_t mn = c[0];
                for (int j = 1; j < fv.cbf_h; ++j) mn = c[j] < mn ? c[j] : mn;
                if (mn >= 16u) { if (cache_store(fv, h0, vals[starts[d]], cache_exp(mn)) && cache_upd) cache_upd[d] = (uint8_t)cache_exp(mn); }
            }
        }
    }
}

inline uint32_t log2_ceil(uint64_t x) { uint32_t l = 0; while ((1ull << l) < x) ++l; return l; }

}

struct ShardState;
struct rb_trav;
using rb::BitFilter; using rb::FilterView; using rb::Mod; using rb::DevBuf; using rb::kmul_of;
struct rb_query_ctx {
    rb::Stream st;
    rb::DevBuf b0, b1, b2, b3;
};
struct rb_graph {
    ~rb_graph();
    std::shared_mutex rw;
    std::mutex qm;
    std::condition_variable qcv;
    std::vector<std::unique_ptr<rb_query_ctx>> qfree;
    int qmade = 0;
    static constexpr int kMaxQueryCtx = 32;
    int shard_rank = 0, shard_count = 1;
    ShardState *shard = nullptr;
    rb_trav *trav = nullptr;
    rb_graph_params p{};
    int k = 0, H = 0;
    bool stranded = false;
    BitFilter dbg, rpk, fpk;
    uint8_t *cbf = nullptr;
    int64_t cbf_size = 0;
    int64_t cbf_lo = 0, cbf_hi = 0;
    size_t cbf_alloc = 0;
    Mod cbf_mod{1, 0, 0};
    int cbf_h = 0;
    int read_d = -1, frag_d = -1;
    uint64_t ordinal = 0;
    int64_t max_batch_kmers = 0;
    int sort_begin_bit = 28;
    uint32_t light_ops = 96;
    uint32_t small_ops = 32;
    rb::Stream stream;
    rb::Stream stream2;
    rb::Stream stream3;
    rb::Stream pk_stream;
    rb::Event ev0, ev1, ev2, ev3;
    DevPool ingest_pool;
    struct GroupSlot { DevBuf keys1, valsT, vals1, tz, uniq, counts, starts, brun, bnr ; uint32_t sweep_T = 0, n_main = 0; size_t N = 0; uint32_t D = 0; int flags = 0; uint32_t live = 0; int bucket_target = 0;  };
    GroupSlot slots[2];
    int cur = 0;
    DevBuf &keys1() { return slots[cur].keys1; }
    DevBuf &vals1() { return slots[cur].vals1; }
    DevBuf &tz() { return slots[cur].tz; }
    DevBuf &uniq() { return slots[cur].uniq; }
    DevBuf &counts() { return slots[cur].counts; }
    DevBuf &starts() { return slots[cur].starts; }
    DevBuf temp2, devctr2, pairs_ctr;
    DevBuf sw_st, sw_temp;
    int pf_streak = 0, pf_skip_left = 0;
    float last_present_frac = 0.0f;
    DevBuf npf, chunk_mask, npf_tot, wstate;
    uint32_t npf_log2 = 0;
    DevBuf mpf;
    uint32_t mpf_log2b = 0, mpf_m = 0;
    const uint64_t *seq_codes = nullptr;
    const uint32_t *seq_woff = nullptr;
    uint32_t seq_wpr = 0;
    uint32_t seq_first = 0;
    uint64_t *group_in_keys = nullptr;
    uint32_t *group_in_vals = nullptr;
    uint32_t occ_bits = 32;
    bool use_mpf = false;
    DevBuf chunk_cnt, chunk_off, keys0, vals0, status, nops, temp,
        ftable, ctable, heavy, confk, conf_sizes, conf_off, opk0, opk1, opv0, opv1, label, kk0, kk1, biglist, cvals, foreign, devctr, qbuf0, qbuf1, qbuf2, qbuf3,
        comm_keep, comm_dreply, comm_creply,
        cwriters, cshared;
    bool prof_on = false;
    struct ProfEntry { const char *name; double ms; int64_t launches; };
    std::vector<ProfEntry> prof;
    struct ProfPending { const char *name; hipEvent_t e0, e1; };
    std::vector<ProfPending> prof_pending;
    std::vector<rb::Event> prof_made;
    std::vector<hipEvent_t> prof_pool;
    hipEvent_t prof_open[3] = {nullptr, nullptr, nullptr};
    std::function<void(int64_t w_end, hipStream_t st)> await_words;
    struct PackedIngest {
        DevBuf codes, valid, word_read, woff, len, wc, temp, stats;
        rb::HostBuf<uint32_t> h_woff, h_stats;
        size_t h_woff_cap = 0;
        std::vector<rb::Event> ev;
        rb::Event ev_woff;
        std::vector<int64_t> wend;
        const void *src = nullptr;
        int64_t n_reads = 0, n_words = 0;
        bool inflight = false;
        std::vector<void *> pins;
        DevBuf off, stage_seq[2], stage_qual[2];
        std::vector<int64_t> rend;
        std::thread feeder;
        std::mutex fm;
        std::condition_variable fcv;
        size_t enqueued = 0;
        bool cancel = false;
        int feeder_rc = 0;
        std::string feeder_err;
        ~PackedIngest() {
            if (feeder.joinable()) {
                { std::lock_guard<std::mutex> lk(fm); cancel = true; }
                fcv.notify_all();
                feeder.join();
            }
            for (void *p : pins) (void)hipHostUnregister(p);
        }
    } pk[2];
    IngestHost ingest_host[2];
    std::mutex pk_mutex;
    int pk_busy = -1;
    hipEvent_t prof_event() {
        if (!prof_pool.empty()) { hipEvent_t e = prof_pool.back(); prof_pool.pop_back(); return e; }
        prof_made.emplace_back();
        RB_HIP(hipEventCreate(&prof_made.back().e));
        return prof_made.back();
    }

    FilterView view(uint64_t ordinal0, uint32_t pos_bits, bool need_all = true) const {
        if (need_all) RB_REQUIRE(dbg.bits && cbf, "this call needs dbgbf and cbf, and one of them has been destroyed");
        FilterView fv;
        fv.dbg = dbg.bits; fv.dbg_mod = dbg.mod; fv.dbg_h = dbg.num_hash;
        fv.cbf = cbf; fv.cbf_mod = cbf_mod; fv.cbf_h = cbf_h;
        fv.kmul = kmul_of(k); fv.seed = p.rng_seed; fv.ordinal0 = ordinal0; fv.pos_bits = pos_bits;
        fv.npf.tab = npf_log2 ? reinterpret_cast<unsigned long long *>(npf.p) : nullptr;
        fv.npf.log2n = npf_log2;
        fv.mpf.tab = (use_mpf && mpf_log2b) ? reinterpret_cast<unsigned long long *>(mpf.p) : nullptr;
        fv.mpf.log2b = mpf_log2b; fv.mpf.m = mpf_m;
        fv.seq_codes = seq_codes; fv.seq_woff = seq_woff; fv.seq_wpr = seq_wpr; fv.seq_first = seq_first; fv.k = k;
        return fv;
    }
    void prof_begin(hipStream_t st = nullptr) {
        if (!prof_on) return;
        const int w = (st && st == stream2) ? 1 : (st && st == stream3) ? 2 : 0;
        prof_open[w] = prof_event();
        RB_HIP(hipEventRecord(prof_open[w], w == 1 ? stream2 : w == 2 ? stream3 : stream));
    }
    void prof_end(const char *name, hipStream_t st = nullptr) {
        if (!prof_on) return;
        const int w = (st && st == stream2) ? 1 : (st && st == stream3) ? 2 : 0;
        if (!prof_open[w]) return;
        hipEvent_t e1 = prof_event();
        RB_HIP(hipEventRecord(e1, w == 1 ? stream2 : w == 2 ? stream3 : stream));
        prof_pending.push_back({name, prof_open[w], e1});
        prof_open[w] = nullptr;
    }
    void prof_add(const char *name, double ms, int64_t launches) {
        for (auto &e : prof) if (!strcmp(e.name, name)) { e.ms += ms; e.launches += launches; return; }
        prof.push_back({name, ms, launches});
    }
    void prof_collect() {
        for (auto &pp : prof_pending) {
            float ms = 0;
            if (hipEventElapsedTime(&ms, pp.e0, pp.e1) == hipSuccess) prof_add(pp.name, ms, 1);
            prof_pool.push_back(pp.e0); prof_pool.push_back(pp.e1);
        }
        prof_pending.clear();
    }
};


namespace rb {
struct QueryLease {
    rb_graph *g;
    std::unique_ptr<rb_query_ctx> c;
    std::shared_lock<std::shared_mutex> lk;
    explicit QueryLease(rb_graph *g_) : g(g_), lk(g_->rw) {
        RB_HIP(hipSetDevice(g->p.device));
        std::unique_lock<std::mutex> q(g->qm);
        for (;;) {
            if (!g->qfree.empty()) { c = std::move(g->qfree.back()); g->qfree.pop_back(); return; }
            if (g->qmade < rb_graph::kMaxQueryCtx) {
                ++g->qmade;
                q.unlock();
                c.reset(new rb_query_ctx());
                hipError_t e = hipStreamCreateWithFlags(&c->st.s, hipStreamNonBlocking);
                if (e != hipSuccess) { c.reset(); q.lock(); --g->qmade; q.unlock(); RB_HIP(e); }
                return;
            }
            g->qcv.wait(q);
        }
    }
    ~QueryLease() {
        if (!c) return;
        { std::lock_guard<std::mutex> q(g->qm); g->qfree.push_back(std::move(c)); }
        g->qcv.notify_one();
    }
    QueryLease(const QueryLease &) = delete;
    QueryLease &operator=(const QueryLease &) = delete;
};
using WriteLock = std::unique_lock<std::shared_mutex>;
uint32_t group_records(rb_graph *g, size_t N, uint64_t ordinal0, uint32_t pos_bits, rb_add_stats *stats, uint32_t **ctr_out);
void group_enqueue(rb_graph *g, int slot, size_t N, uint64_t ordinal0, uint32_t pos_bits, hipStream_t st, DevBuf &temp, DevBuf &ctrbuf,
                   int flags = 0 );
uint32_t group_finish(rb_graph *g, int slot, hipStream_t st, DevBuf &temp, DevBuf &ctrbuf, hipStream_t scan_stream);
// ... 25 lines not shown
```

Before: 43.58 billion.

## Use non-power-of-two index-keyed bucket counts to fill grouping tiles evenly

Index-keyed grouping now picks a bucket count from a per-bucket record target instead of rounding up to a power of two. Buckets carry more records and fewer of them sit partly empty, which spreads the grouping and sweep kernels over fewer but fuller blocks. The in-bucket load layout is changed to split each bucket evenly across wavefronts, and bucket bounds are made wave-uniform with readfirstlane. The shard path keeps power-of-two buckets. The sweep kernel now derives bucket ranges by division instead of shifts, and a debug fill report is added.

```diff
diff --git a/rna-bloom_amd/csrc/rb_capi.hip b/rna-bloom_amd/csrc/rb_capi.hip
--- a/rna-bloom_amd/csrc/rb_capi.hip
+++ b/rna-bloom_amd/csrc/rb_capi.hip
@@ -770,7 +770,7 @@
         RB_HIP(hipSetDevice(device));
         const int gflags = (int)flags;
         const GrIdx idx = idx_span ? GrIdx{make_mod(idx_size), idx_lo, idx_span} : GrIdx{Mod{1, 0, 0}, 0, 0};
-        uint32_t plan[7];
+        uint32_t plan[8];
         group_debug_plan(n, group_bits, bucket_target, gflags, idx, plan);
         const size_t nbk = (size_t)1 << plan[0];
         k0.reserve(n * 8); v0.reserve(n * 4); k1.reserve(n * 8); v1.reserve(n * 4);
diff --git a/rna-bloom_amd/csrc/rb_graph.hip b/rna-bloom_amd/csrc/rb_graph.hip
--- a/rna-bloom_amd/csrc/rb_graph.hip
+++ b/rna-bloom_amd/csrc/rb_graph.hip
@@ -1097,6 +1097,7 @@
 void rb::group_enqueue(rb_graph *g, int slot, size_t N, uint64_t ordinal0, uint32_t pos_bits, hipStream_t st, DevBuf &temp,
                        DevBuf &ctrbuf, int flags) {
     rb_graph::GroupSlot &S = g->slots[slot];
+    if (g->shard) flags |= GR_FLAG_POW2;
     S.N = N; S.D = 0; S.flags = flags; S.live = (uint32_t)N;
     ctrbuf.reserve(DEVCTR_BYTES);
     uint32_t *ctr = ctrbuf.as<uint32_t>();
@@ -1116,17 +1117,18 @@
         else if (g->dbg.bits && g->dbg.size > 0) gidx = GrIdx{g->dbg.mod, (uint64_t)g->dbg.lo, (uint64_t)(g->dbg.hi - g->dbg.lo)};
     }
     GroupExport ex;
-    S.sweep_T = 0; S.n_main = 0;
+    S.sweep_T = 0; S.sweep_nbk = 0; S.n_main = 0;
     if (want_idx && sweep_wanted(g)) {
         const GrIdx didx{g->dbg.mod, 0, (uint64_t)g->dbg.size};
         const bool same = gidx.span == didx.span && gidx.lo == 0 && gidx.mod.d == didx.mod.d;
         if (!same) gidx = didx;
-        S.sweep_T = group_index_buckets(N, group_bits, bucket_target, flags, gidx);
+        S.sweep_T = group_index_buckets(N, group_bits, bucket_target, flags, gidx, &S.sweep_nbk);
         if (S.sweep_T) {
             S.brun.reserve(((size_t)4 << S.sweep_T) + 16); S.bnr.reserve(((size_t)4 << S.sweep_T) + 16);
             ex = GroupExport{S.brun.as<uint32_t>(), S.bnr.as<uint32_t>(), ctr + 9};
         }
     }
+    if (getenv("RB_DEBUG")) { uint32_t plan[8]; group_debug_plan(N, group_bits, bucket_target, flags, gidx, plan); S.nbk = plan[7]; }
     uint64_t *kin = g->group_in_keys ? g->group_in_keys : g->keys0.as<uint64_t>();
     uint32_t *vin = g->group_in_vals ? g->group_in_vals : g->vals0.as<uint32_t>();
     g->group_in_keys = nullptr; g->group_in_vals = nullptr;
@@ -1150,6 +1152,11 @@
         uint32_t nb = 0, mx = 0; uint64_t rec = 0;
         group_debug_big(temp.p, S.N, 64 - g->sort_begin_bit, S.bucket_target, &nb, &rec, &mx, S.flags);
         fprintf(stderr, "[rb] grouping: N=%zu runs=%u; buckets that did not fit LDS: %u with %llu records, largest %u\n", S.N, D, nb, (unsigned long long)rec, mx);
+        uint32_t used = 0, T = 0;
+        while ((1u << T) < S.nbk) ++T;
+        group_debug_fill(temp.p, S.N, 64 - g->sort_begin_bit, S.bucket_target, S.flags, S.nbk, &used, &mx);
+        fprintf(stderr, "[rb] group fill: N=%zu live=%u T=%u buckets=%u in_use=%u avg_fill=%.1f largest=%u\n", S.N, S.live, T, S.nbk, used,
+                used ? (double)S.live / used : 0.0, mx);
     }
     return D;
 }
@@ -1317,7 +1324,7 @@
     bool swept = false, swept_all = false;
     uint32_t *involved = nullptr, n_involved_max = 0;
     if (collide && !ftab && fv.dbg_h == 2 && fv.cbf_h == 2 && !getenv("RB_PROBE_GENERIC") && GS.sweep_T && !g->shard && sweep_wanted(g) &&
-        ((uint64_t)g->dbg.size >> GS.sweep_T) < (1ull << 31)) {
+        (uint64_t)g->dbg.size / GS.sweep_nbk < (1ull << 31)) {
         const char *e = getenv("RB_SWEEP");
         static const float present_max = getenv("RB_SWEEP_PRESENT") ? (float)atof(getenv("RB_SWEEP_PRESENT")) : 0.5f;
         swept = (e && atoi(e) == 1) || ((uint64_t)D * 64ull >= (uint64_t)g->dbg.nbytes && g->last_present_frac < present_max);
@@ -1327,10 +1334,10 @@
         swept_all = GS.n_main >= D;
         const size_t st_pad = ((size_t)D + 15) & ~(size_t)15;
         g->sw_st.reserve(st_pad + D + 16);
-        g->sw_temp.reserve(sweep_temp_bytes(D, GS.sweep_T));
+        g->sw_temp.reserve(sweep_temp_bytes(D, GS.sweep_T, GS.sweep_nbk));
         uint8_t *st0 = g->sw_st.as<uint8_t>(), *st1 = st0 + st_pad;
         uint64_t *ka = g->foreign.as<uint64_t>(), *kb = ka + D;
-        sweep_bits_device(g->dbg.bits, didx, GS.sweep_T, fv.kmul, uniq, D, GS.n_main, GS.brun.as<uint32_t>(), GS.bnr.as<uint32_t>(), ka, g->nops.as<uint32_t>(), kb,
+        sweep_bits_device(g->dbg.bits, didx, GS.sweep_T, GS.sweep_nbk, fv.kmul, uniq, D, GS.n_main, GS.brun.as<uint32_t>(), GS.bnr.as<uint32_t>(), ka, g->nops.as<uint32_t>(), kb,
                           g->heavy.as<uint32_t>(), g->sw_temp.p, g->sw_temp.cap, st0, st1, s);
         const bool same_index = (int64_t)g->dbg.size == g->cbf_size && g->cbf_lo == 0 && g->dbg.mod.d == g->cbf_mod.d && g->dbg.mod.m_lo == g->cbf_mod.m_lo &&
                                 g->dbg.mod.m_hi == g->cbf_mod.m_hi && fv.dbg_h == fv.cbf_h;
diff --git a/rna-bloom_amd/csrc/rb_group.hip b/rna-bloom_amd/csrc/rb_group.hip
--- a/rna-bloom_amd/csrc/rb_group.hip
+++ b/rna-bloom_amd/csrc/rb_group.hip
@@ -10,6 +10,7 @@
 constexpr uint32_t GR_MAX_GROUP_BITS = 36;
 constexpr uint32_t GR_TILE = 4096;
 constexpr uint32_t GR_BUCKET_TARGET = 3072;
+constexpr uint32_t GR_INDEX_TARGET = 2304;
 constexpr uint32_t GR_LOCAL_BITS = 8;
 constexpr uint32_t GR_PART_MAX_BITS = 10;
 
@@ -280,9 +281,9 @@
     }
 }
 __global__ void k_bucket_bounds(const uint32_t *__restrict__ goffs, uint32_t ntiles1, const uint32_t *__restrict__ seg_tile_base,
-                                const uint32_t *__restrict__ seg_start, uint32_t t_hi, uint32_t t_lo, uint32_t n, uint32_t *__restrict__ bstart,
+                                const uint32_t *__restrict__ seg_start, uint32_t t_hi, uint32_t t_lo, uint32_t nbk, uint32_t n, uint32_t *__restrict__ bstart,
                                 const uint32_t *__restrict__ n_dev = nullptr) {
-    const uint32_t p = blockIdx.x * blockDim.x + threadIdx.x, nbk = 1u << (t_hi + t_lo);
+    const uint32_t p = blockIdx.x * blockDim.x + threadIdx.x;
     if (n_dev) n = *n_dev;
     if (p > nbk) return;
     if (p == nbk) { bstart[p] = n; return; }
@@ -333,7 +334,7 @@
                                                        uint64_t *__restrict__ uniq, uint32_t *__restrict__ counts, uint32_t *__restrict__ starts,
                                                        uint32_t *__restrict__ n_runs_out, uint32_t by_class,
                                                        uint32_t *__restrict__ brun , uint32_t *__restrict__ bnr ) {
-    constexpr uint32_t ITEMS = GR_TILE / TPB, NW = TPB / 64, SEG = 64 * ITEMS, NB = 1u << GR_LOCAL_BITS;
+    constexpr uint32_t ITEMS = GR_TILE / TPB, NW = TPB / 64, NB = 1u << GR_LOCAL_BITS;
     static_assert(ITEMS * NW == 64, "the segment scan below is one wavefront wide");
     __shared__ uint64_t s_keys[GR_TILE];
     __shared__ uint32_t s_vals[GR_TILE];
@@ -343,18 +344,20 @@
     __shared__ uint32_t s_wsum[NW], s_seg[ITEMS * NW], s_misc[3], s_fixn, s_redo;
     __shared__ uint16_t s_fixlist[64];
     __shared__ uint32_t s_cls[16];
-    const uint32_t w = threadIdx.x >> 6, lane = threadIdx.x & 63u;
+    const uint32_t w = (uint32_t)__builtin_amdgcn_readfirstlane((int)(threadIdx.x >> 6)), lane = threadIdx.x & 63u;
     for (uint32_t d = threadIdx.x; d < NW * NB; d += TPB) { s_wmask[d] = 0ull; s_wcnt[0][d] = 0; s_wcnt[1][d] = 0; }
     uint32_t c = 0, b0 = 0, b1 = 0;
     uint64_t k[ITEMS];
     uint32_t v[ITEMS], dig[ITEMS], rank[ITEMS];
+    auto seg_of = [](uint32_t n) { return ((n + 64u * NW - 1u) / (64u * NW)) * 64u; };
     auto load_bucket = [&](uint32_t cc, uint32_t &bb0, uint32_t &bb1, uint64_t (&kk)[ITEMS], uint32_t (&vv)[ITEMS]) {
-        bb0 = bstart[cc]; bb1 = bstart[cc + 1u];
+        bb0 = (uint32_t)__builtin_amdgcn_readfirstlane((int)bstart[cc]); bb1 = (uint32_t)__builtin_amdgcn_readfirstlane((int)bstart[cc + 1u]);
         const uint32_t n = bb1 - bb0 > GR_TILE ? 0u : bb1 - bb0;
+        const uint32_t sg = seg_of(n);
 #pragma unroll
         for (uint32_t r = 0; r < ITEMS; ++r) {
-            const uint32_t j = w * SEG + r * 64u + lane;
-            const bool ok = j < n;
+            const uint32_t j = w * sg + r * 64u + lane;
+            const bool ok = r * 64u < sg && j < n;
             kk[r] = ok ? keys_in[bb0 + j] : 0ull;
             vv[r] = ok ? vals_in[bb0 + j] : 0u;
         }
@@ -378,7 +381,8 @@
     const uint32_t c_next = PREFETCH ? s_misc[2] : 0u;
     const bool big = b1 - b0 > GR_TILE;
     const uint32_t cn = big ? 0u : b1 - b0;
-    const uint32_t rows = cn > w * SEG ? min(ITEMS, (cn - w * SEG + 63u) / 64u) : 0u;
+    const uint32_t seg = seg_of(cn);
+    const uint32_t rows = cn > w * seg ? min(seg / 64u, (cn - w * seg + 63u) / 64u) : 0u;
     if (big && threadIdx.x == 0) big_list[atomicAdd(n_big, 1u)] = c;
     bool in_lds = false;
     auto sort_pass = [&](uint32_t shift, uint32_t bits, uint16_t *wcnt) {
@@ -387,14 +391,14 @@
         if (in_lds) {
 #pragma unroll
             for (uint32_t r = 0; r < ITEMS; ++r) {
-                const uint32_t j = w * SEG + r * 64u + lane;
-                if (j < cn) { k[r] = s_keys[j]; v[r] = s_vals[j]; }
+                const uint32_t j = w * seg + r * 64u + lane;
+                if (r < rows && j < cn) { k[r] = s_keys[j]; v[r] = s_vals[j]; }
             }
         }
 #pragma unroll
         for (uint32_t r = 0; r < ITEMS; ++r) {
-            const uint32_t j = w * SEG + r * 64u + lane;
-            dig[r] = j < cn ? gr_digit(k[r], shift, bits) : ~0u;
+            const uint32_t j = w * seg + r * 64u + lane;
+            dig[r] = (r < rows && j < cn) ? gr_digit(k[r], shift, bits) : ~0u;
         }
         gr_wave_rank_lds<ITEMS>(dig, rank, wcnt + w * nb, s_wmask + w * NB, rows);
         __syncthreads();
@@ -464,8 +468,8 @@
     if (!in_lds) {
 #pragma unroll
         for (uint32_t r = 0; r < ITEMS; ++r) {
-            const uint32_t j = w * SEG + r * 64u + lane;
-            if (j < cn) { s_keys[j] = k[r]; s_vals[j] = v[r]; }
+            const uint32_t j = w * seg + r * 64u + lane;
+            if (r < rows && j < cn) { s_keys[j] = k[r]; s_vals[j] = v[r]; }
         }
         __syncthreads();
     }
@@ -720,6 +724,7 @@
     uint32_t shift_lo = 0, shift_hi = 0;
     uint32_t l_lo = 0, l_hi = 0, lshift_lo = 0, lshift_hi = 0;
     uint32_t ntiles = 0, ntiles2_max = 0, nbuckets = 1;
+    uint32_t nbk = 1;
     bool dead = false;
     uint32_t tpb = 256;
     uint32_t fix_cap = 0;
@@ -730,7 +735,7 @@
 };
 static size_t gr_align(size_t x) { return (x + 255) / 256 * 256; }
 
-static GroupPlan group_plan(size_t N, int group_bits, int bucket_target = 0, int flags = 0, int force_T = -1) {
+static GroupPlan group_plan(size_t N, int group_bits, int bucket_target = 0, int flags = 0, int force_T = -1, uint32_t force_nbk = 0) {
     GroupPlan P;
     P.n = (uint32_t)N;
     P.dead = (flags & GR_FLAG_DEAD) != 0;
@@ -739,11 +744,17 @@
     const size_t target = getenv("RB_GROUP_TARGET") ? (size_t)std::max(64, std::min(atoi(getenv("RB_GROUP_TARGET")), (int)GR_TILE))
                         : bucket_target > 0 ? (size_t)bucket_target : (size_t)GR_BUCKET_TARGET;
     while ((target << T) < N) ++T;
-    if (const char *e = getenv("RB_GROUP_T")) T = (uint32_t)std::max(0, atoi(e));
-    if (force_T >= 0) T = (uint32_t)force_T;
+    const size_t count_target = (getenv("RB_GROUP_TARGET") || bucket_target > 0) ? target : (size_t)GR_INDEX_TARGET;
+    uint32_t nbk = (uint32_t)std::min<size_t>((size_t)1 << T, (N + count_target - 1) / count_target);
+    if (flags & GR_FLAG_POW2) nbk = 0;
+    if (const char *e = getenv("RB_GROUP_POW2")) { if (atoi(e) != 0) nbk = 0; }
+    if (const char *e = getenv("RB_GROUP_T")) { T = (uint32_t)std::max(0, atoi(e)); nbk = 0; }
+    if (force_T >= 0) { T = (uint32_t)force_T; nbk = force_nbk; }
+    const uint32_t T_asked = T;
     T = std::min({T, gb, 2u * GR_PART_MAX_BITS});
     if (P.dead && T == 0) T = 1;
     P.T = T;
+    P.nbk = (nbk && T == T_asked && nbk <= (1u << T) && nbk > (T ? 1u << (T - 1u) : 0u)) ? nbk : 1u << T;
     if (T <= GR_PART_MAX_BITS) { P.t_hi = T; P.t_lo = 0; }
     else { P.t_hi = (T + 1u) / 2u; P.t_lo = T - P.t_hi; }
     P.shift_hi = GR_KEY_TOP - P.t_hi;
@@ -795,6 +806,15 @@
     for (uint32_t i = 0; i < nb; ++i) { const uint32_t c = bs[big[i] + 1] - bs[big[i]]; rec += c; mx = std::max(mx, c); }
     *n_big_out = nb; *records_out = rec; *largest_out = mx;
 }
+void group_debug_fill(const void *temp, size_t N, int group_bits, int bucket_target, int flags, uint32_t nbk, uint32_t *in_use_out, uint32_t *largest_out) {
+    const GroupPlan P = group_plan(N, group_bits, bucket_target, flags);
+    nbk = std::min(nbk, P.nbuckets);
+    std::vector<uint32_t> bs((size_t)nbk + 1);
+    RB_HIP(hipMemcpy(bs.data(), static_cast<const char *>(temp) + P.off_bstart, ((size_t)nbk + 1) * 4, hipMemcpyDeviceToHost));
+    uint32_t used = 0, mx = 0;
+    for (uint32_t c = 0; c < nbk; ++c) { const uint32_t n = bs[c + 1] - bs[c]; used += n ? 1u : 0u; mx = std::max(mx, n); }
+    *in_use_out = used; *largest_out = mx;
+}
 size_t group_temp_bytes(size_t N, int group_bits, int bucket_target, int flags) { return group_plan(N, group_bits, bucket_target, flags).total; }
 const uint32_t *group_live_count(const void *temp, size_t N, int group_bits, int bucket_target, int flags) {
     const GroupPlan P = group_plan(N, group_bits, bucket_target, flags);
@@ -917,9 +937,11 @@
     hipLaunchKernelGGL(k_lsd_gather64, dim3((unsigned)((n + 255) / 256)), dim3(256), 0, s, i1, vals_in, vals_out, n);
 }
 
+static bool gr_idx_keyed(const GroupPlan &P, const GrIdx &idx) { return idx.span > (1ull << P.T); }
+static uint32_t gr_buckets(const GroupPlan &P, const GrIdx &idx) { return gr_idx_keyed(P, idx) ? P.nbk : P.nbuckets; }
 static GrIdxDev gr_idx_dev(const GroupPlan &P, const GrIdx &idx) {
-    if (idx.span > (1ull << P.T))
-        return GrIdxDev{idx.mod, idx.lo, (uint64_t)((((unsigned __int128)1 << 64) << P.T) / idx.span), (1u << P.T) - 1u, P.t_lo};
+    if (gr_idx_keyed(P, idx))
+        return GrIdxDev{idx.mod, idx.lo, (uint64_t)((((unsigned __int128)1 << 64) * P.nbk) / idx.span), P.nbk - 1u, P.t_lo};
     return GrIdxDev{Mod{1, 0, 0}, 0, 0, 0, 0};
 }
 template <int TPB>
@@ -952,9 +974,10 @@
             part_pass<TPB>(t2, (size_t)P.ntiles2_max << P.t_lo, P.shift_lo, P.t_lo, kin, vin, keys0, vals0, hist, goffs, scan_tmp, P.scan_bytes, st, prof, nullptr, ix);
             kin = keys0; vin = vals0;
         }
-        hipLaunchKernelGGL(k_bucket_bounds, dim3((P.nbuckets + 256u) / 256u), dim3(256), 0, st, goffs, P.ntiles, segtb, segst, P.t_hi, P.t_lo, P.n, bstart, (const uint32_t *)n_live);
+        const uint32_t nbk = gr_buckets(P, idx);
+        hipLaunchKernelGGL(k_bucket_bounds, dim3((nbk + 256u) / 256u), dim3(256), 0, st, goffs, P.ntiles, segtb, segst, P.t_hi, P.t_lo, nbk, P.n, bstart, (const uint32_t *)n_live);
     } else
-        hipLaunchKernelGGL(k_bucket_bounds, dim3(1), dim3(64), 0, st, (const uint32_t *)nullptr, 0u, (const uint32_t *)nullptr, (const uint32_t *)nullptr, 0u, 0u, P.n, bstart);
+        hipLaunchKernelGGL(k_bucket_bounds, dim3(1), dim3(64), 0, st, (const uint32_t *)nullptr, 0u, (const uint32_t *)nullptr, (const uint32_t *)nullptr, 0u, 0u, 1u, P.n, bstart);
     *kin_out = kin; *vin_out = vin;
     return bstart;
 }
@@ -970,22 +993,23 @@
     uint32_t *bstart = partition_records<TPB>(P, keys0, vals0, keys_tmp, vals_tmp, tp, st, prof, idx, &kin, &vin);
     uint32_t *big_list = reinterpret_cast<uint32_t *>(tp + P.off_big), *n_big = ticket + 2;
     if (prof) prof->prof_begin(st);
-    const uint32_t bucket_grid = std::min(P.nbuckets, (uint32_t)(getenv("RB_GROUP_GRID") ? atoi(getenv("RB_GROUP_GRID")) : 768));
+    const uint32_t nbk = gr_buckets(P, idx);
+    const uint32_t bucket_grid = std::min(nbk, (uint32_t)(getenv("RB_GROUP_GRID") ? atoi(getenv("RB_GROUP_GRID")) : 768));
     const bool ordered = getenv("RB_GROUP_ORDERED") && atoi(getenv("RB_GROUP_ORDERED")) != 0;
     if (!ordered) RB_HIP(hipMemsetAsync(n_runs_dev, 0, 4, st));
     const bool prefetch = !(getenv("RB_GROUP_PREFETCH") && atoi(getenv("RB_GROUP_PREFETCH")) == 0);
     const uint32_t by_class = getenv("RB_GROUP_CLASSES") ? (uint32_t)(atoi(getenv("RB_GROUP_CLASSES")) != 0) : 1u;
     if (ordered || !prefetch)
-        hipLaunchKernelGGL((k_group_buckets<TPB, false>), dim3(bucket_grid), dim3(TPB), 0, st, kin, vin, bstart, P.nbuckets, P.lshift_lo, P.l_lo, P.lshift_hi, P.l_hi,
+        hipLaunchKernelGGL((k_group_buckets<TPB, false>), dim3(bucket_grid), dim3(TPB), 0, st, kin, vin, bstart, nbk, P.lshift_lo, P.l_lo, P.lshift_hi, P.l_hi,
                            rng, P.fix_cap, ticket, ordered ? status : nullptr, big_list, n_big, vals_out, tz_out, uniq, counts, starts, n_runs_dev, 0u, ex.brun, ex.bnr);
     else
-        hipLaunchKernelGGL((k_group_buckets<TPB, true>), dim3(bucket_grid), dim3(TPB), 0, st, kin, vin, bstart, P.nbuckets, P.lshift_lo, P.l_lo, P.lshift_hi, P.l_hi,
+        hipLaunchKernelGGL((k_group_buckets<TPB, true>), dim3(bucket_grid), dim3(TPB), 0, st, kin, vin, bstart, nbk, P.lshift_lo, P.l_lo, P.lshift_hi, P.l_hi,
                            rng, P.fix_cap, ticket, nullptr, big_list, n_big, vals_out, tz_out, uniq, counts, starts, n_runs_dev, by_class, ex.brun, ex.bnr);
     if (ex.n_main) hipLaunchKernelGGL(k_copy_u32, dim3(1), dim3(64), 0, st, ex.n_main, n_runs_dev);
     if (prof) { prof->prof_end("group_buckets", st); prof->prof_begin(st); }
     uint64_t *ka = const_cast<uint64_t *>(kin), *kb = kin == keys0 ? keys_tmp : keys0;
     uint32_t *va = const_cast<uint32_t *>(vin), *vb = vin == vals0 ? vals_tmp : vals0;
-    hipLaunchKernelGGL(k_group_big<512>, dim3(std::min(P.nbuckets, 2048u)), dim3(512), 0, st, ka, va, kb, vb, bstart, big_list, n_big,
+    hipLaunchKernelGGL(k_group_big<512>, dim3(std::min(nbk, 2048u)), dim3(512), 0, st, ka, va, kb, vb, bstart, big_list, n_big,
                        P.lshift_lo, P.l_lo, P.lshift_hi, P.l_hi, rng, vals_out, tz_out, uniq, counts, starts, n_runs_dev);
     if (prof) prof->prof_end("group_big_buckets", st);
     RB_HIP(hipGetLastError());
@@ -1002,14 +1026,17 @@
     if (P.tpb == 512u) group_records_impl<512>(P, keys0, vals0, keys_tmp, vals_tmp, rng, static_cast<char *>(temp), vals_out, tz_out, uniq, counts, starts, n_runs_dev, st, prof, idx, ex);
     else group_records_impl<256>(P, keys0, vals0, keys_tmp, vals_tmp, rng, static_cast<char *>(temp), vals_out, tz_out, uniq, counts, starts, n_runs_dev, st, prof, idx, ex);
 }
-uint32_t group_index_buckets(size_t N, int group_bits, int bucket_target, int flags, GrIdx idx) {
+uint32_t group_index_buckets(size_t N, int group_bits, int bucket_target, int flags, GrIdx idx, uint32_t *nbk_out) {
     const GroupPlan P = group_plan(N, group_bits, bucket_target, flags);
-    return (P.T && idx.span > (1ull << P.T)) ? P.T : 0u;
-}
-void group_debug_plan(size_t N, int group_bits, int bucket_target, int flags, GrIdx idx, uint32_t out[7]) {
+    const bool keyed = P.T && gr_idx_keyed(P, idx);
+    if (nbk_out) *nbk_out = keyed ? P.nbk : 0u;
+    return keyed ? P.T : 0u;
+}
+void group_debug_plan(size_t N, int group_bits, int bucket_target, int flags, GrIdx idx, uint32_t out[8]) {
     const GroupPlan P = group_plan(N, group_bits, bucket_target, flags);
     out[0] = P.T; out[1] = P.t_hi; out[2] = P.t_lo; out[3] = P.l_hi; out[4] = P.l_lo; out[5] = P.fix_cap;
     out[6] = (P.T && gr_idx_dev(P, idx).mul != 0) ? 1u : 0u;
+    out[7] = gr_buckets(P, idx);
 }
 
 constexpr uint32_t SW_WORDS = 16384;
@@ -1017,16 +1044,16 @@
 __device__ __forceinline__ uint32_t sw_digit(uint64_t x, const GrIdxDev &ix) {
     return min((uint32_t)min(__umul64hi(x, ix.mul), (uint64_t)0xFFFFFFFFull), ix.top);
 }
-__device__ __forceinline__ uint64_t sw_first(uint32_t c, const GrIdxDev &ix, uint64_t span, uint32_t T) {
+__device__ __forceinline__ uint64_t sw_first(uint32_t c, const GrIdxDev &ix, uint64_t span) {
     if (c == 0u) return 0ull;
     if (c > ix.top) return span;
-    uint64_t e = ((uint64_t)c * span) >> T;
+    uint64_t e = ((uint64_t)c * span) / (uint64_t)(ix.top + 1u);
     while (e > 0ull && sw_digit(e - 1ull, ix) >= c) --e;
     while (e < span && sw_digit(e, ix) < c) ++e;
     return e;
 }
 template <int TPB>
-__global__ void __launch_bounds__(TPB, 4) k_sweep_bits(uint32_t *words, GrIdxDev ix, uint64_t span, uint32_t T, const uint64_t *__restrict__ uniq,
+__global__ void __launch_bounds__(TPB, 4) k_sweep_bits(uint32_t *words, GrIdxDev ix, uint64_t span, const uint64_t *__restrict__ uniq,
                                                     const uint32_t *__restrict__ brun, const uint32_t *__restrict__ bnr,
                                                     const uint64_t *__restrict__ k1, const uint32_t *__restrict__ v1, const uint32_t *__restrict__ bstart1,
                                                     uint8_t *st0, uint8_t *st1, uint32_t SWW ) {
@@ -1036,7 +1063,7 @@
     const uint32_t c = blockIdx.x;
     const uint32_t r0 = brun[c], nr = bnr[c], p0 = bstart1[c], p1 = bstart1[c + 1u];
     if (nr == 0u && p0 == p1) return;
-    const uint64_t x_lo = sw_first(c, ix, span, T), x_hi = sw_first(c + 1u, ix, span, T);
+    const uint64_t x_lo = sw_first(c, ix, span), x_hi = sw_first(c + 1u, ix, span);
     const uint64_t w_lo = (x_lo >> 5) & ~3ull, w_hi = (x_hi + 31ull) >> 5;
     const uint64_t in_lo = (x_lo + 31ull) >> 5, in_hi = x_hi >> 5;
     constexpr uint32_t KEEP = GR_TILE / TPB;
@@ -1140,13 +1167,14 @@
     const uint32_t m = 1u << (uint32_t)(i0 & 31ull);
     if (atomicOr(&words[i0 >> 5], m) & m) st0[d] = 2;
 }
-size_t sweep_temp_bytes(size_t D, uint32_t T) { return group_plan(D, 64, 0, 0, (int)T).total; }
-void sweep_bits_device(uint32_t *words, GrIdx idx, uint32_t T, uint64_t kmul, const uint64_t *uniq, uint32_t D, uint32_t n_main, const uint32_t *brun,
+size_t sweep_temp_bytes(size_t D, uint32_t T, uint32_t nbk) { return group_plan(D, 64, 0, 0, (int)T, nbk).total; }
+void sweep_bits_device(uint32_t *words, GrIdx idx, uint32_t T, uint32_t nbk, uint64_t kmul, const uint64_t *uniq, uint32_t D, uint32_t n_main, const uint32_t *brun,
                        const uint32_t *bnr, uint64_t *keys_a, uint32_t *vals_a, uint64_t *keys_b, uint32_t *vals_b, void *temp, size_t temp_bytes,
                        uint8_t *st0, uint8_t *st1, hipStream_t st) {
-    RB_REQUIRE(D > 0 && T > 0 && idx.span > (1ull << T) && (idx.span >> T) < (1ull << 31), "sweep_bits_device: nothing to sweep by / ranges of 2^31 bits and more");
-    const GroupPlan P = group_plan(D, 64, 0, 0, (int)T);
-    RB_REQUIRE(P.T == T && temp_bytes >= P.total, "sweep_bits_device: plan / temp mismatch");
+    RB_REQUIRE(D > 0 && T > 0 && nbk > 0 && nbk <= (1u << T) && idx.span > (1ull << T) && idx.span / nbk < (1ull << 31),
+               "sweep_bits_device: nothing to sweep by / ranges of 2^31 bits and more");
+    const GroupPlan P = group_plan(D, 64, 0, 0, (int)T, nbk);
+    RB_REQUIRE(P.T == T && P.nbk == nbk && temp_bytes >= P.total, "sweep_bits_device: plan / temp mismatch");
     RB_HIP(hipMemsetAsync(st1, 0, D, st));
     RB_REQUIRE(kmul != 0, "sweep_bits_device: kmul");
     const uint64_t *k1 = nullptr;
@@ -1156,10 +1184,10 @@
     GrIdxDev ix = gr_idx_dev(P, idx);
     const uint32_t n_big = D - std::min(n_main, D);
     if (n_big) hipLaunchKernelGGL(k_sw_big_pre, dim3((n_big + 255u) / 256u), dim3(256), 0, st, (const uint32_t *)words, idx.mod, idx.lo, uniq, n_main, D, st0);
-    const uint64_t range_words = (idx.span >> T) / 32 + 16;
+    const uint64_t range_words = (idx.span / nbk) / 32 + 16;
     const uint32_t sww = (uint32_t)std::min<uint64_t>(SW_WORDS, (range_words + 1023) / 1024 * 1024);
     RB_HIP(hipFuncSetAttribute(reinterpret_cast<const void *>(k_sweep_bits<512>), hipFuncAttributeMaxDynamicSharedMemorySize, (int)((SW_WORDS + 2 * SW_MARKS) * 4)));
-    hipLaunchKernelGGL(k_sweep_bits<512>, dim3(P.nbuckets), dim3(512), (sww + 2 * SW_MARKS) * 4, st, words, ix, idx.span, T, uniq, brun, bnr, k1, v1, bstart1, st0, st1, sww);
+    hipLaunchKernelGGL(k_sweep_bits<512>, dim3(nbk), dim3(512), (sww + 2 * SW_MARKS) * 4, st, words, ix, idx.span, uniq, brun, bnr, k1, v1, bstart1, st0, st1, sww);
     if (n_big) hipLaunchKernelGGL(k_sw_big_set, dim3((n_big + 255u) / 256u), dim3(256), 0, st, words, idx.mod, idx.lo, uniq, n_main, D, st0);
     RB_HIP(hipGetLastError());
 }
diff --git a/rna-bloom_amd/csrc/rb_internal.hpp b/rna-bloom_amd/csrc/rb_internal.hpp
--- a/rna-bloom_amd/csrc/rb_internal.hpp
+++ b/rna-bloom_amd/csrc/rb_internal.hpp
@@ -276,12 +276,14 @@
                      uint32_t mask_b, uint32_t *out_b, uint32_t *count_dev, hipStream_t s);
 
 constexpr int GR_FLAG_DEAD = 1;
+constexpr int GR_FLAG_POW2 = 2;
 struct GrIdx {
     Mod mod;
     uint64_t lo = 0, span = 0;
 };
 struct GroupExport { uint32_t *brun = nullptr, *bnr = nullptr, *n_main = nullptr; };
 void group_debug_big(const void *temp, size_t N, int group_bits, int bucket_target, uint32_t *n_big_out, uint64_t *records_out, uint32_t *largest_out, int flags = 0);
+void group_debug_fill(const void *temp, size_t N, int group_bits, int bucket_target, int flags, uint32_t nbk, uint32_t *in_use_out, uint32_t *largest_out);
 size_t group_temp_bytes(size_t N, int group_bits, int bucket_target = 0, int flags = 0);
 const uint32_t *group_live_count(const void *temp, size_t N, int group_bits, int bucket_target, int flags);
 void group_records_device(uint64_t *keys0, uint32_t *vals0, uint64_t *keys_tmp, uint32_t *vals_tmp, size_t N, int group_bits,
@@ -291,10 +293,10 @@
                           int bucket_target = 0 , int flags = 0 ,
                           GrIdx idx = GrIdx{Mod{1, 0, 0}, 0, 0} ,
                           GroupExport ex = GroupExport{});
-uint32_t group_index_buckets(size_t N, int group_bits, int bucket_target, int flags, GrIdx idx);
-void group_debug_plan(size_t N, int group_bits, int bucket_target, int flags, GrIdx idx, uint32_t out[7]);
-size_t sweep_temp_bytes(size_t D, uint32_t T);
-void sweep_bits_device(uint32_t *words, GrIdx idx, uint32_t T, uint64_t kmul, const uint64_t *uniq, uint32_t D, uint32_t n_main, const uint32_t *brun,
+uint32_t group_index_buckets(size_t N, int group_bits, int bucket_target, int flags, GrIdx idx, uint32_t *nbk_out = nullptr);
+void group_debug_plan(size_t N, int group_bits, int bucket_target, int flags, GrIdx idx, uint32_t out[8]);
+size_t sweep_temp_bytes(size_t D, uint32_t T, uint32_t nbk);
+void sweep_bits_device(uint32_t *words, GrIdx idx, uint32_t T, uint32_t nbk, uint64_t kmul, const uint64_t *uniq, uint32_t D, uint32_t n_main, const uint32_t *brun,
                        const uint32_t *bnr, uint64_t *keys_a, uint32_t *vals_a, uint64_t *keys_b, uint32_t *vals_b, void *temp, size_t temp_bytes,
                        uint8_t *st0, uint8_t *st1, hipStream_t st);
 
diff --git a/rna-bloom_amd/csrc/rb_pipeline.hpp b/rna-bloom_amd/csrc/rb_pipeline.hpp
--- a/rna-bloom_amd/csrc/rb_pipeline.hpp
+++ b/rna-bloom_amd/csrc/rb_pipeline.hpp
@@ -321,7 +321,7 @@
     rb::Stream pk_stream;
     rb::Event ev0, ev1, ev2, ev3;
     DevPool ingest_pool;
-    struct GroupSlot { DevBuf keys1, valsT, vals1, tz, uniq, counts, starts, brun, bnr ; uint32_t sweep_T = 0, n_main = 0; size_t N = 0; uint32_t D = 0; int flags = 0; uint32_t live = 0; int bucket_target = 0;  };
+    struct GroupSlot { DevBuf keys1, valsT, vals1, tz, uniq, counts, starts, brun, bnr ; uint32_t sweep_T = 0, sweep_nbk = 0 , nbk = 0 , n_main = 0; size_t N = 0; uint32_t D = 0; int flags = 0; uint32_t live = 0; int bucket_target = 0;  };
     GroupSlot slots[2];
     int cur = 0;
     DevBuf &keys1() { return slots[cur].keys1; }
```

Result: no change. 43.63 billion (median of 3 runs) (+0.1%).
